# esa/auromat

Hardware: AMD Instinct MI355X
Metric: Mpixels/s georef+resample, 4240x2832 frame (higher is better)
Workload: dtype f64

## Files before the change

### auromat_amd/_native.py

```python
import ctypes as C
import os
import threading
import weakref

import numpy as np

from ._build import LIB_PATH

c_double_p = C.POINTER(C.c_double)
c_void_pp = C.POINTER(C.c_void_p)


class FrameParams(C.Structure):
    _fields_ = [('width', C.c_int32), ('height', C.c_int32), ('fast_center', C.c_int32), ('reserved', C.c_int32),
                ('cd', C.c_double * 4), ('crpix', C.c_double * 2), ('rot', C.c_double * 9),
                ('cam', C.c_double * 3), ('a', C.c_double), ('b', C.c_double),
                ('a0', C.c_double), ('b0', C.c_double), ('m_geo', C.c_double * 9), ('m_sm', C.c_double * 9)]


class AllSkyParams(C.Structure):
    _fields_ = [('size', C.c_int32), ('reserved', C.c_int32), ('xc', C.c_double), ('yc', C.c_double),
                ('k', C.c_double), ('rotation', C.c_double), ('center_offset', C.c_double),
                ('to_geo', C.c_double * 9), ('station', C.c_double * 3), ('a', C.c_double), ('b', C.c_double),
                ('a0', C.c_double), ('b0', C.c_double)]
# ... 13 lines not shown

class ZenithalWcs(C.Structure):
    _fields_ = [(k, C.c_int32) for k in ('width', 'height', 'corner', 'projection')] + \
               [('cd', C.c_double * 4), ('crpix', C.c_double * 2), ('rot', C.c_double * 9), ('start_x', C.c_double),
                ('start_y', C.c_double), ('sip_order_a', C.c_int32), ('sip_order_b', C.c_int32),
                ('sip_a', (C.c_double * SIP_MAX) * SIP_MAX), ('sip_b', (C.c_double * SIP_MAX) * SIP_MAX)]


class Axis(C.Structure):
    _fields_ = [('edges', C.c_void_p), ('nbin', C.c_int32), ('uniform', C.c_int32),
                ('first', C.c_double), ('last', C.c_double), ('step', C.c_double), ('scale', C.c_double),
                ('last_rounded', C.c_double)]


class Grid(C.Structure):
    _fields_ = [('nx', C.c_int32), ('ny', C.c_int32), ('n_lat_nodes', C.c_int32), ('n_lon_nodes', C.c_int32)] + \
               [(k, C.c_double) for k in ('lat_lo', 'lat_hi', 'lon_lo', 'lon_hi', 'lat_step', 'lon_step',
                                          'lat_center_first', 'lat_center_last', 'lon_center_first',
                                          'lon_center_last')] + [('xaxis', Axis), ('yaxis', Axis)]


class SeqFrame(C.Structure):
    _fields_ = [('ny', C.c_int32), ('nx', C.c_int32), ('nc', C.c_int32), ('index', C.c_int32),
                ('lat0', C.c_double), ('lon0', C.c_double), ('dlat', C.c_double), ('dlon', C.c_double),
                ('contains_pole', C.c_int32), ('contains_discontinuity', C.c_int32), ('magnetic', C.c_int32),
                ('reserved', C.c_int32), ('altitude', C.c_double), ('mean', C.c_void_p), ('count', C.c_void_p)]


class MosaicMember(C.Structure):
    _fields_ = [(k, C.c_void_p) for k in ('lat_c', 'lon_c', 'elev', 'img', 'center_mask')] + \
               [(k, C.c_int32) for k in ('height', 'width', 'win_x0', 'win_y0', 'win_nx', 'win_ny')]


class AreaMosaicMember(C.Structure):
    _fields_ = [(k, C.c_void_p) for k in ('lat', 'lon', 'lat_c', 'elev', 'img', 'center_mask')] + \
               [(k, C.c_int32) for k in ('height', 'width', 'win_x0', 'win_y0', 'win_nx', 'win_ny')]


class ScanLineStrip(C.Structure):
    _fields_ = [(k, C.c_void_p) for k in ('row', 'col', 'planes', 'img')] + \
               [('count', C.c_int64), ('frame', C.c_int32), ('reserved', C.c_int32)]


class Projection(C.Structure):
    _fields_ = [('kind', C.c_int32), ('mode', C.c_int32)] + \
               [(k, C.c_double) for k in ('lat0', 'lon0', 'a', 'e', 'sin_chi1', 'cos_chi1', 'm1', 'k')] + \
               [('reserved', C.c_double * 4)]


class PipeResult(C.Structure):
    _fields_ = [('status', C.c_int32), ('fused', C.c_int32), ('lon_wrapped', C.c_int32), ('edge_pixels', C.c_int32),
                ('bbox', C.c_double * 8), ('grid', Grid)]


class RunConfig(C.Structure):
    _fields_ = [(k, C.c_int32) for k in ('width', 'height', 'img_dtype', 'fast_center', 'magnetic', 'batch', 'use_hints',
                                         'n_slots', 'two_pass', 'statistic')] + \
               [(k, C.c_double) for k in ('altitude', 'min_elevation', 'lat_px_per_deg', 'lon_px_per_deg')] + \
               [('slots', C.POINTER(GeorefOut)), ('arcsec_per_px', C.c_double)]


class RunFrame(C.Structure):
    _fields_ = [('crval', C.c_double * 2), ('crpix', C.c_double * 2), ('cd', C.c_double * 4), ('lonpole', C.c_double),
                ('cam', C.c_double * 3), ('jd', C.c_double), ('altitude', C.c_double), ('img', C.c_void_p),
                ('img_host', C.c_void_p)]


class RunResult(C.Structure):
    _fields_ = [(k, C.c_int32) for k in ('status', 'slot', 'ny', 'nx', 'contains_pole', 'lon_wrapped', 'hinted',
                                         'edge_pixels', 'two_pass', 'reserved_')] + \
               [('grid_offset', C.c_int64), ('image_offset', C.c_int64), ('bbox', C.c_double * 8), ('altitude', C.c_double),
                ('grid', Grid), ('params', FrameParams), ('lat_px_per_deg', C.c_double), ('lon_px_per_deg', C.c_double),
                ('retried', C.c_int32), ('reserved2_', C.c_int32), ('uploaded_bytes', C.c_int64)]


class LensModel(C.Structure):
    _fields_ = [(k, C.c_int32) for k in ('kind', 'width', 'height', 'crop_x', 'crop_y', 'crop_width', 'crop_height', 'reserved')] + \
               [('k', C.c_double * 3)]


class LensDebug(C.Structure):
    _fields_ = [('force_path', C.c_int32), ('reserved', C.c_int32), ('tile_path', C.c_void_p)]


ABI_VERSION = 10
QUANTILES_MAX = 8
PIPE_MAX_EDGE_PIXELS = 16384
_I, _L, _D, _P = C.c_int, C.c_int64, C.c_double, C.c_void_p
_SIGNATURES = {
    'amt_abi_version': ([], _I),
    'amt_ctx_create': ([_I, _P, _I, c_void_pp], _I),
    'amt_ctx_destroy': ([_P], _I),
    'amt_ctx_set_stream': ([_P, _P], _I),
    'amt_ctx_get_stream': ([_P], _P),
    'amt_ctx_synchronize': ([_P], _I),
    'amt_last_error': ([_P], C.c_char_p),
    'amt_device_info': ([_P, C.c_char_p, C.c_size_t, C.POINTER(_I), C.POINTER(_I), C.POINTER(C.c_size_t)], _I),
    'amt_malloc': ([_P, C.c_size_t, c_void_pp], _I),
    'amt_free': ([_P, _P], _I),
    'amt_host_threads': ([_I, C.POINTER(_I), C.POINTER(_I)], _I),
    'amt_malloc_host': ([_P, C.c_size_t, c_void_pp], _I),
    'amt_free_host': ([_P, _P], _I),
    'amt_memcpy_h2d': ([_P, _P, _P, C.c_size_t], _I),
    'amt_memcpy_d2h': ([_P, _P, _P, C.c_size_t], _I),
    'amt_memset': ([_P, _P, _I, C.c_size_t], _I),
    'amt_event_create': ([_P, c_void_pp], _I),
    'amt_event_destroy': ([_P, _P], _I),
    'amt_event_record': ([_P, _P], _I),
    'amt_event_elapsed_ms': ([_P, _P, _P, C.POINTER(C.c_float)], _I),
    'amt_timing_enable': ([_P, _I], _I),
    'amt_timing_read': ([_P, _I, C.POINTER(C.c_double), C.POINTER(_I)], _I),
    'amt_pipe_launch_box': ([_P, C.POINTER(FrameParams), _D, _I], _I),
    'amt_pipe_launch_box_many': ([c_void_pp, C.c_int32, c_void_pp, _D, _I], _I),
    'amt_pipe_launch_many_res': ([c_void_pp, C.c_int32, c_void_pp, c_void_pp, c_void_pp, C.c_int32, _D, c_double_p, c_double_p, _I, _I], _I),
    'amt_plate_carree_resolution': ([_D, _D, _D, _D, _D, c_double_p, c_double_p], _I),
    'amt_upload_staged': ([_P, _P, _P, C.c_size_t], _I),
    'amt_padded_pitch': ([C.c_int32], C.c_int64),
    'amt_unpad_rows': ([_P, _P, C.c_int32, C.c_int32, C.c_int32, _P], _I),
    'amt_download_staged': ([_P, _P, _P, C.c_size_t], _I),
    'amt_georef_last_variant': ([_P, C.POINTER(C.c_int32), C.POINTER(C.c_int32), C.POINTER(C.c_int32)], _I),
    'amt_directions_tan': ([_P, C.POINTER(FrameParams), _I, _P], _I),
    'amt_directions_zenithal': ([_P, C.POINTER(ZenithalWcs), _P], _I),
    'amt_directions_tan_points': ([_P, C.POINTER(FrameParams), _P, _P, _L, _I, _P], _I),
    'amt_lens_coords': ([_P, C.POINTER(LensModel)] + [C.c_int32] * 4 + [_I, _P, _P], _I),
    'amt_lens_undistort': ([_P, C.POINTER(LensModel)] + [C.c_int32] * 4 + [_I, _P], _I),
    'amt_lens_remap': ([_P, C.POINTER(LensModel), _P, C.c_int32, C.c_int32, C.c_int32, _P, _P, C.POINTER(LensDebug)], _I),
    'amt_remap_coords': ([_P, _P] + [C.c_int32] * 4 + [_P] + [C.c_int32] * 3 + [_P, _P, C.POINTER(LensDebug)], _I),
    'amt_world_to_pixel': ([_P, C.POINTER(FrameParams), C.POINTER(ZenithalWcs), C.c_int32, _P, _P, _L, _P, _P, _P], _I),
    'amt_grid_to_pixel': ([_P, C.POINTER(FrameParams), C.POINTER(ZenithalWcs), C.c_int32, _P, C.c_int32, _P, C.c_int32, _P, _P, _P,
                           _P], _I),
    'amt_intersect_ellipsoid': ([_P, _D, _D, c_double_p, _P, _L, _I, _P], _I),
    'amt_intersects_ellipsoid': ([_P, _D, _D, c_double_p, _P, _L, _I, _P], _I),
    'amt_intersect_sphere': ([_P, _D, c_double_p, _P, _L, _I, _P], _I),
    'amt_ecef_to_geodetic': ([_P, _P, _P, _P, _L, _D, _D, _P, _P], _I),
    'amt_geodetic_to_ecef': ([_P, _P, _P, _D, _L, _D, _D, _P, _P, _P], _I),
    'amt_rotate_to_latlon': ([_P, c_double_p, _P, _L, _D, _D, _P, _P], _I),
    'amt_rotate_to_mlat_mlt': ([_P, c_double_p, _P, _L, _P, _P], _I),
    'amt_rotate_vectors': ([_P, c_double_p, _P, _L, _P], _I),
    'amt_latlon_to_mlat_mlt': ([_P, c_double_p, _P, _P, _D, _L, _D, _D, _P, _P], _I),
    'amt_sm_to_latlon': ([_P, c_double_p, _P, _P, _L, _D, _D, _P, _P], _I),
    'amt_projection_stereographic': ([_D, _D, _D, _D, C.POINTER(Projection)], _I),
    'amt_projection_polar_aeqd': ([_I, _D, _D, C.POINTER(Projection)], _I),
    'amt_project_forward': ([_P, C.POINTER(Projection), _P, _P, _L, _P, _P], _I),
    'amt_project_inverse': ([_P, C.POINTER(Projection), _P, _P, _L, _P, _P], _I),
    'amt_rotate_pole': ([_P, c_double_p, _P, _P, _D, _L, _D, _D, _P, _P], _I),
    'amt_rotate_pole_deg': ([_P, c_double_p, _P, _P, _D, _L, _D, _D, _P, _P], _I),
    'amt_cartesian_to_spherical': ([_P, _P, _P, _P, _L, _P, _P, _P], _I),
    'amt_spherical_to_cartesian': ([_P, _P, _P, _P, _L, _P, _P, _P], _I),
    'amt_georef_allsky': ([_P, C.POINTER(AllSkyParams), _I, _P, _P, _P, _P, _P], _I),
    'amt_reproject_altitude': ([_P, _D, _D, _P, _P, _L, _D, _D, _D, _D, _P, _P], _I),
    'amt_georef_frame': ([_P, C.POINTER(FrameParams), C.POINTER(GeorefOut)], _I),
    'amt_georef_frame_dirs': ([_P, C.POINTER(FrameParams), _P, C.POINTER(GeorefOut)], _I),
    'amt_georef_coarse_bbox': ([_P, C.POINTER(FrameParams), C.c_int32, _D, _I, _P], _I),
    'amt_delaunay_create': ([_P, C.c_int64, C.POINTER(C.c_void_p)], _I),
    'amt_delaunay_destroy': ([_P], _I),
    'amt_delaunay_sizes': ([_P, C.POINTER(C.c_int64), C.POINTER(C.c_int64), C.POINTER(C.c_int64)], _I),
    'amt_delaunay_stats': ([_P, _P], _I),
    'amt_delaunay_slots': ([_P, c_void_pp, c_void_pp, C.POINTER(C.c_int64)], _I),
    'amt_delaunay_create_threads': ([_P, C.c_int64, C.c_int32, C.c_int64, C.POINTER(C.c_void_p)], _I),
    'amt_delaunay_build_info': ([_P, _P], _I),
    'amt_delaunay_triangles': ([_P, _P, _P], _I),
    'amt_delaunay_vertex_neighbours': ([_P, _P, _P], _I),
    'amt_delaunay_locate': ([_P, _P, C.c_int64, _P, _P, _P], _I),
    'amt_cubic_gradients_csr': ([_P, _P, C.c_int64, _P, _P, _P, C.c_int32, _P, C.c_int32, _D, C.c_int32, _P, _P], _I),
    'amt_cubic_eval': ([_P, C.c_int64, _P, _P, _P, _P, _P, _P, _P, C.c_int32, _P], _I),
    'amt_georef_coarse_bbox_dirs': ([_P, C.POINTER(FrameParams), _P, C.c_int32, _D, _I, _P], _I),
    'amt_pipe_coarse_dirs': ([_P, C.POINTER(FrameParams), _P, _D, _I], _I),
    'amt_pipe_launch_dirs': ([_P, C.POINTER(FrameParams), _P, C.POINTER(GeorefOut), _P, C.c_int32, _D, _D, _D, _I, _I], _I),
    'amt_georef_sky_rows': ([C.POINTER(FrameParams)] + [C.POINTER(C.c_int32)] * 4, _I),
    'amt_georef_image_rows': ([C.POINTER(FrameParams), _D] + [C.POINTER(C.c_int32)] * 2, _I),
    'amt_mask_by_elevation': ([_P, _P, _P, C.c_int32, C.c_int32, _D, _P, _P, _P], _I),
    'amt_sanitize_masks': ([_P, _P, _P, _P, C.c_int32, C.c_int32, _I], _I),
    'amt_bbox_corners': ([_P, _P, _P, _P, _P, C.c_int32, C.c_int32, _P], _I),
    'amt_mask_outline_links': ([_P, _P, C.c_int32, C.c_int32, _P, _L, _P], _I),
    'amt_pixel_polygons': ([_P, _P, _P, _P, C.c_int32, C.c_int32, C.c_int32, C.c_int32, _P, _L, _P, _P, _P], _I),
    'amt_hist2d_accumulate': ([_P, _P, _P, _L, c_void_pp, C.c_int32, C.POINTER(Axis), C.POINTER(Axis), _I, _P,
                               c_void_pp], _I),
    'amt_hist2d_finalize_mean': ([_P, _P, c_void_pp, C.c_int32, C.c_int32, C.c_int32, _P], _I),
    'amt_bin_frame': ([_P, _P, _P, _P, _P, C.c_int32, C.c_int32, _P, C.c_int32, C.c_int32, _D, C.POINTER(Axis),
                       C.POINTER(Axis), _I, _P], _I),
    'amt_bin_frame_finalize': ([_P, _P, C.c_int32, C.c_int32, C.c_int32, C.c_int32, _P, _P, _P, _P], _I),
    'amt_bin_frame_finalize_window': ([_P, _P] + [C.c_int32] * 8 + [_P, _P, _P, _P], _I),
    'amt_area_frame': ([_P, _P, _P, _P, _P, _P, C.c_int32, C.c_int32, _P, C.c_int32, C.c_int32, _D, C.POINTER(Axis),
                        C.POINTER(Axis), _I, _P], _I),
    'amt_area_plane_frame': ([_P, _P, _P, _P, _P, _P, C.c_int32, C.c_int32, _P, C.c_int32, C.c_int32, _D, C.POINTER(Axis),
                              C.POINTER(Axis), _P], _I),
    'amt_area_frame_finalize': ([_P, _P, C.c_int32, C.c_int32, C.c_int32, C.c_int32, C.c_uint64, _P, _P, _P, _P], _I),
    'amt_area_frame_async': ([_P, _P, _P, _P, _P, _P, C.c_int32, C.c_int32, _P, C.c_int32, C.c_int32, _D, C.POINTER(Axis),
                              C.POINTER(Axis), _I, _I, C.c_int32, C.c_int32, C.c_uint64, _P, _P, _P, _P, _P], _I),
    'amt_median_frame': ([_P, _P, _P, _P, _P, C.c_int32, C.c_int32, _P, C.c_int32, C.c_int32, _D, C.POINTER(Axis),
                          C.POINTER(Axis), _I, _P, _P, _P, _P], _I),
    'amt_median_frame_async': ([_P, _P, _P, _P, _P, C.c_int32, C.c_int32, _P, C.c_int32, C.c_int32, _D, C.POINTER(Axis),
                                C.POINTER(Axis), _I, _I, _P, _P, _P, _P], _I),
    'amt_quantile_frame': ([_P, _P, _P, _P, _P, C.c_int32, C.c_int32, _P, C.c_int32, C.c_int32, _D, C.POINTER(Axis),
                            C.POINTER(Axis), _I, c_double_p, _I, _P, _P, _P, _P], _I),
    'amt_quantile_frame_async': ([_P, _P, _P, _P, _P, C.c_int32, C.c_int32, _P, C.c_int32, C.c_int32, _D, C.POINTER(Axis),
                                  C.POINTER(Axis), _I, _I, c_double_p, _I, _P, _P, _P, _P], _I),
    'amt_quantile_rank': ([_L, _D, C.POINTER(_L), C.POINTER(_L), c_double_p], _I),
    'amt_mosaic_frames': ([_P, C.POINTER(MosaicMember), C.c_int32, C.c_int32, C.c_int32, _D, C.POINTER(Axis), C.POINTER(Axis),
                           _I, C.c_int32, _P, _P, _P, _P, _P], _I),
    'amt_mosaic_median_frames': ([_P, C.POINTER(MosaicMember), C.c_int32, C.c_int32, C.c_int32, _D, C.POINTER(Axis),
                                  C.POINTER(Axis), _I, C.c_int32, _P, _P, _P, _P, _P], _I),
    'amt_mosaic_quantile_frames': ([_P, C.POINTER(MosaicMember), C.c_int32, C.c_int32, C.c_int32, _D, C.POINTER(Axis),
                                    C.POINTER(Axis), _I, C.c_int32, c_double_p, _I, _P, _P, _P, _P, _P], _I),
    'amt_area_mosaic_frames': ([_P, C.POINTER(AreaMosaicMember), C.c_int32, C.c_int32, C.c_int32, _D, C.POINTER(Axis),
                                C.POINTER(Axis), _I, C.c_int32, C.c_uint64, _P, _P, _P, _P, _P], _I),
    'amt_scanline_select': ([_P, _P, _P, C.c_int32, C.c_int32, _P, C.c_int32, _P, C.c_int32, C.c_int32, C.c_int32, C.c_int32, _P,
                             _P], _I),
    'amt_scanline_pack': ([_P, _P] + [C.c_int32] * 4 + [_P, C.c_int32, _P] + [C.c_int32] * 6 + [_L, _P, _P, _P, _P], _I),
    'amt_scanline_compose': ([_P, C.POINTER(ScanLineStrip)] + [C.c_int32] * 8 + [_P, _P, _P, _P], _I),
    'amt_nearest_frame': ([_P, _P, _P, _P, _P, C.c_int32, C.c_int32, _D, C.POINTER(Axis), C.POINTER(Axis), _I, _P, _P, _P,
                           _P], _I),
    'amt_nearest_gather': ([_P, _P, _L, _P, C.c_int32, C.c_int32, _P, _P, _P, _P], _I),
    'amt_points_in_polygon': ([_P, _P, _P, _L, _P, C.c_int32, _P], _I),
    'amt_grid_layout': ([_D, _D, _D, _D, _D, _D, C.POINTER(Grid)], _I),
    'amt_pipe_create': ([_P, c_void_pp], _I),
    'amt_pipe_destroy': ([_P], _I),
    'amt_pipe_coarse': ([_P, C.POINTER(FrameParams), _D, _I], _I),
    'amt_pipe_coarse_hint': ([_P, c_double_p, _I], _I),
    'amt_pipe_launch': ([_P, C.POINTER(FrameParams), C.POINTER(GeorefOut), _P, C.c_int32, _D, _D, _D, _I, _I], _I),
    'amt_pipe_launch_many': ([c_void_pp, C.c_int32, c_void_pp, c_void_pp, c_void_pp, C.c_int32, _D, _D, _D, _I, _I], _I),
    'amt_pipe_launch_dirs_many': ([c_void_pp, C.c_int32, c_void_pp, c_void_pp, c_void_pp, c_void_pp, C.c_int32, _D, _D, _D, _I, _I], _I),
    'amt_pipe_wait': ([_P, C.POINTER(PipeResult)], _I),
    'amt_pipe_finalize': ([_P, _P, _P, _P, _P], _I),
    'amt_pipe_finalize_stream': ([_P, _P], _I),
    'amt_pipe_finalize_many': ([_P, C.c_int32, _P, _P, _P, _P], _I),
    'amt_pipe_join': ([_P], _I),
    'amt_pipe_set_plan': ([_P, _I], _I),
    'amt_pipe_general_layout': ([_P, C.POINTER(PipeResult)], _I),
    'amt_pipe_general_finalize': ([_P, _P, _P, _P, _P], _I),
    'amt_frame_params_from_wcs': ([C.POINTER(RunFrame), C.c_int32, C.c_int32, C.c_int32, _D, C.c_int32,
                                   C.POINTER(FrameParams)], _I),
    'amt_pole_in_view': ([C.POINTER(FrameParams), _D, _I], _I),
    'amt_frames_close': ([C.POINTER(FrameParams), C.POINTER(FrameParams)], _I),
    'amt_box_hint': ([c_double_p, C.POINTER(FrameParams), _L, c_double_p, C.POINTER(FrameParams), _L, _L, C.POINTER(FrameParams),
                      c_double_p], _I),
    'amt_run_create': ([_P, C.POINTER(RunConfig), c_void_pp], _I),
    'amt_run_destroy': ([_P], _I),
    'amt_run_process': ([_P, C.POINTER(RunFrame), C.c_int32, _P, _L, _P, _L, C.POINTER(RunResult), C.POINTER(C.c_int32)], _I),
    'amt_run_begin': ([_P, _P, _L, _P, _L, C.POINTER(RunResult), C.c_int32], _I),
    'amt_run_push': ([_P, C.POINTER(RunFrame)], _I),
    'amt_run_end': ([_P, C.POINTER(C.c_int32)], _I),
    'amt_run_reset_hints': ([_P], _I),
    'amt_run_fill_stats': ([_P, C.POINTER(C.c_int64), C.POINTER(C.c_int64)], _I),
    'amt_run_set_quantile': ([_P, _D], _I),
    'amt_run_set_min_coverage': ([_P, C.c_uint64], _I),
    'amt_run_area_overflow': ([_P, C.POINTER(C.c_int32), C.c_int32], _I),
    'amt_seq_payload_size': ([C.POINTER(SeqFrame), C.c_int32, C.POINTER(_L)], _I),
    'amt_seq_pack': ([_P, C.POINTER(SeqFrame), C.c_int32, C.c_int32, _P, _L], _I),
    'amt_seq_unpack': ([_P, _L, C.c_int32, C.c_int32, C.POINTER(SeqFrame), C.c_int32, C.POINTER(C.c_int32)], _I),
}

_lib = None
_lib_lock = threading.Lock()


class NativeError(RuntimeError):
    pass


def host_threads(wanted):
    try:
        cores = len(os.sched_getaffinity(0))
    except (AttributeError, OSError):
        cores = os.cpu_count() or 1
    ranks = 1
    for name in ('AMT_LOCAL_RANKS', 'LOCAL_WORLD_SIZE'):
        try:
            v = int(os.environ.get(name, '0'))
        except ValueError:
            v = 0
        if v > 0:
            ranks = v
            break
    return max(1, min(int(wanted), max(1, cores // ranks)))


def host_threads_report():
    cores, ranks = C.c_int(0), C.c_int(0)
    share = lib().amt_host_threads(1 << 20, C.byref(cores), C.byref(ranks))
    copy = int(os.environ.get('AMT_COPY_THREADS', '8'))
    return dict(cores_available=cores.value, local_ranks=ranks.value, share=share,
                copy_threads=max(1, min(copy, (share + 1) // 2, 16)),
                triangulator_threads=int(os.environ.get('AMT_DELAUNAY_THREADS', '0')) or lib().amt_host_threads(16, None, None),
                io_threads=host_threads(16), omp_num_threads=os.environ.get('OMP_NUM_THREADS'))


def lib():
    global _lib
    if _lib is not None:
        return _lib
    with _lib_lock:
        if _lib is None:
            if not os.path.exists(LIB_PATH):
                raise NativeError('libauromat_hip.so is not built (%s missing); run `python -c "import '
                                  '__graft_entry__ as g; g.build()"` or `python -m auromat_amd._build`. '
                                  'There is no CPU fallback.' % LIB_PATH)
            import torch
            handle = C.CDLL(LIB_PATH, mode=C.RTLD_GLOBAL)
            for name, (argtypes, restype) in _SIGNATURES.items():
                fn = getattr(handle, name)
                fn.argtypes = argtypes
                fn.restype = restype
            if handle.amt_abi_version() != ABI_VERSION:
                raise NativeError('ABI version mismatch: the library is %d, this package expects %d (rebuild: '
                                  'python -c "import __graft_entry__ as g; g.build()")' % (handle.amt_abi_version(), ABI_VERSION))
            _lib = handle
    return _lib


def exported_symbols():
    return sorted(_SIGNATURES)


class Context(object):
    _cache = {}
    _cache_lock = threading.Lock()

    def __init__(self, device_index):
        import torch
        self._lib = lib()
        if not torch.cuda.is_available():
            raise NativeError('no HIP device is visible; auromat_amd has no CPU fallback')
        self.device = torch.device('cuda', device_index)
        self.stream_handle = torch.cuda.current_stream(self.device).cuda_stream
        h = C.c_void_p()
        rc = self._lib.amt_ctx_create(device_index, C.c_void_p(self.stream_handle), 0, C.byref(h))
        if rc != 0:
            raise NativeError('amt_ctx_create failed (%d)' % rc)
        self.handle = h
        self._staging = None

    @classmethod
    def current(cls, device=None):
        import torch
        if not torch.cuda.is_available():
            raise NativeError('no HIP device is visible; auromat_amd has no CPU fallback')
        if device is None:
            idx = torch.cuda.current_device()
        else:
            idx = torch.device(device).index
            if idx is None:
                idx = torch.cuda.current_device()
        key = (os.getpid(), threading.get_ident(), idx)
        with cls._cache_lock:
            ctx = cls._cache.get(key)
            if ctx is None:
                ctx = cls._cache[key] = cls(idx)
        stream = torch.cuda.current_stream(ctx.device).cuda_stream
        if stream != ctx.stream_handle:
            ctx.check(ctx._lib.amt_ctx_set_stream(ctx.handle, C.c_void_p(stream)))
            ctx.stream_handle = stream
        return ctx

    def check(self, rc):
        if rc != 0:
            msg = self._lib.amt_last_error(self.handle)
            raise NativeError('libauromat_hip: %s (code %d)' % (msg.decode() if msg else '?', rc))

    def call(self, name, *args):
        self.check(getattr(self._lib, name)(self.handle, *args))

    def synchronize(self):
        self.call('amt_ctx_synchronize')

    def device_info(self):
        name = C.create_string_buffer(256)
        cus, khz, mem = C.c_int(), C.c_int(), C.c_size_t()
        self.call('amt_device_info', name, 256, C.byref(cus), C.byref(khz), C.byref(mem))
        return dict(name=name.value.decode(), compute_units=cus.value, clock_khz=khz.value, total_mem=mem.value)

    def empty(self, shape, dtype=None):
        import torch
        return torch.empty(shape, dtype=dtype or torch.float64, device=self.device)

    def zeros(self, shape, dtype=None):
        import torch
        return torch.zeros(shape, dtype=dtype or torch.float64, device=self.device)

    def to_device(self, array, dtype=np.float64):
        import torch
        if isinstance(array, torch.Tensor):
            t = array.to(self.device)
            want = _torch_dtype(dtype)
            if t.dtype != want:
                t = t.to(want)
            return t.contiguous()
        a = np.ascontiguousarray(array, dtype=dtype)
        if a.dtype == np.uint16:
            a = a.view(np.int16)
        if a.nbytes >= _PIN_MIN_BYTES and np.dtype(a.dtype) in _TORCH_DTYPES:
            out = torch.empty(a.shape, dtype=_torch_dtype(a.dtype), device=self.device)
            self.upload(a, out)
            return out.view(torch.bool) if a.dtype == np.bool_ else out
        if not a.flags.writeable:
            a = a.copy()
        return torch.from_numpy(a).to(self.device)
# ... 107 lines not shown
```

### auromat_amd/csrc/amt_common.h

```cpp
#pragma once

#include <hip/hip_runtime.h>
#include <hip/hip_ext.h>

#include <cmath>
#include <cstdint>
#include <cstdio>
#include <cstring>
#include <string>
#include <vector>

#include "../../include/auromat_hip.h"

struct amt_copier;
void amt_copier_destroy(amt_copier* c);

struct amt_ctx {
    int device;
    amt_copier* copier;
    hipStream_t stream;
    bool owns_stream;
    double* scratch;
    struct workspace {
        hipStream_t stream;
        void* ptr;
        size_t bytes;
        unsigned long long last_use;
    };
    std::vector<workspace> workspaces;
    unsigned long long workspace_clock;
    std::string last_error;
    hipStream_t aux_pre, aux_tail, aux_fin;
    int last_second, last_bin, last_frames;
    int timing;
    size_t tlaunch[2];
    int tframes[2];
    std::vector<hipEvent_t> tev[2];
    size_t tused[2];
};

constexpr int kTimingMaxLaunches = 4096;

static inline void amt_timing_pair(amt_ctx* ctx, int kind, int frames, hipEvent_t* start, hipEvent_t* stop) {
    *start = *stop = nullptr;
    if (!ctx->timing) return;
    if ((ctx->tlaunch[kind]++ % (size_t)ctx->timing) != 0) return;
    if (ctx->tused[kind] + 2 > (size_t)2 * kTimingMaxLaunches) return;
    while (ctx->tused[kind] + 2 > ctx->tev[kind].size()) {
        hipEvent_t e;
        if (hipEventCreate(&e) != hipSuccess) return;
        ctx->tev[kind].push_back(e);
    }
    *start = ctx->tev[kind][ctx->tused[kind]];
    *stop = ctx->tev[kind][ctx->tused[kind] + 1];
    ctx->tused[kind] += 2;
    ctx->tframes[kind] += frames;
}

struct amt_georef_tail {
    hipStream_t stream;
    hipEvent_t kernel_done;
    double* partials;
    size_t partials_bytes;
    int band_x = 0x7fffffff, band_y = 0x7fffffff;
};
constexpr int kNoBand = 0x7fffffff;
size_t amt_georef_partials_bytes(const amt_frame_params* p);
#define AMT_MAX_BATCH 3
struct amt_sky_state {
    int known_top_end, known_bottom_begin;
    int bands_filled, bands_skipped;
};
int amt_georef_launch_many(amt_ctx* ctx, int n, const amt_frame_params* const* p, const double* const* dirs,
                           const amt_georef_out* const* out, const amt_georef_tail* const* tail, amt_sky_state* sky);
int amt_pipe_launch_many_sky(amt_pipe* const* pipes, int32_t n, const amt_frame_params* const* p, const amt_georef_out* const* out,
                             const void* const* img, int32_t img_dtype, double min_elevation, const double* lat_px_per_deg,
                             const double* lon_px_per_deg, int pole_in_view, int magnetic, amt_sky_state* sky);
int amt_bin_apply_events_on(amt_ctx* ctx, hipStream_t stream, const void* events, uint32_t* count, uint64_t* acc,
                            int32_t acc_nx, int32_t acc_ny, int32_t off_x, int32_t off_y, int32_t nx, int32_t ny,
                            uint32_t xmask, uint32_t ymask);
int amt_bin_finalize_on(amt_ctx* ctx, hipStream_t stream, uint64_t* acc, int32_t acc_nx, int32_t acc_ny, int32_t off_x,
                        int32_t off_y, int32_t nx, int32_t ny, int32_t nchan, int32_t img_dtype, double* mean,
                        void* out_img, uint8_t* out_mask, double* out_count, int clear);

int amt_mosaic_run(amt_ctx* ctx, const amt_mosaic_member* members, int32_t n_members, int32_t img_dtype, int32_t nchan,
                   double min_elevation, const amt_axis* xaxis, const amt_axis* yaxis, int lon_wrap, int32_t rule, double* mean,
                   void* out_img, uint8_t* out_mask, double* out_count, int32_t* out_source, size_t tail_bytes, char** tail);

struct finish_frame {
    const void* events;
    unsigned int* count;
    unsigned long long* acc;
    int acc_nx, acc_ny, off_x, off_y, nx, ny;
    unsigned int n_events;
    unsigned int masks;
    double* mean;
    void* img;
    uint8_t* mask;
    double* out_count;
};
struct finish_batch {
    finish_frame f[3];
    int n, pad_;
};
int amt_pipe_finish_on(amt_ctx* ctx, hipStream_t stream, const finish_batch& B, int32_t img_dtype);

constexpr size_t kMaxWorkspaces = 16;
static inline void* amt_workspace(amt_ctx* ctx, size_t bytes) {
    amt_ctx::workspace* w = nullptr;
    for (auto& e : ctx->workspaces)
        if (e.stream == ctx->stream) w = &e;
    if (w == nullptr) {
        if (ctx->workspaces.size() >= kMaxWorkspaces) {
            size_t lru = 0;
            for (size_t i = 1; i < ctx->workspaces.size(); ++i)
                if (ctx->workspaces[i].last_use < ctx->workspaces[lru].last_use) lru = i;
            amt_ctx::workspace& old = ctx->workspaces[lru];
            if (old.ptr) {
                (void)hipStreamSynchronize(old.stream);
                (void)hipGetLastError();
                (void)hipFree(old.ptr);
            }
            ctx->workspaces.erase(ctx->workspaces.begin() + (long)lru);
        }
        ctx->workspaces.push_back({ctx->stream, nullptr, 0, 0});
        w = &ctx->workspaces.back();
    }
    w->last_use = ++ctx->workspace_clock;
    if (bytes <= w->bytes) return w->ptr;
    if (w->ptr) {
        (void)hipStreamSynchronize(ctx->stream);
        (void)hipFree(w->ptr);
        w->ptr = nullptr;
        w->bytes = 0;
    }
    const size_t cap = bytes < (1u << 20) ? (1u << 20) : bytes;
    if (hipMalloc(&w->ptr, cap) != hipSuccess) {
        w->ptr = nullptr;
        return nullptr;
    }
    w->bytes = cap;
    return w->ptr;
}

#define AMT_CHECK_CTX(ctx) \
    if ((ctx) == nullptr) return AMT_EINVAL

#define AMT_REQUIRE(ctx, cond, msg)                           \
    do {                                                      \
        if (!(cond)) {                                        \
            (ctx)->last_error = std::string(__func__) + ": " + (msg); \
            return AMT_EINVAL;                                \
        }                                                     \
    } while (0)

#define AMT_HIP(ctx, call)                                                              \
    do {                                                                                \
        hipError_t err__ = (call);                                                      \
        if (err__ != hipSuccess) {                                                      \
            (ctx)->last_error = std::string(__func__) + ": " #call " -> " + hipGetErrorString(err__); \
            return AMT_EHIP;                                                            \
        }                                                                               \
    } while (0)

#define AMT_LAUNCH_CHECK(ctx) AMT_HIP(ctx, hipGetLastError())

static inline int amt_set_device(amt_ctx* ctx) {
    AMT_HIP(ctx, hipSetDevice(ctx->device));
    return AMT_OK;
}

namespace amt {

constexpr int kBlock = 256;

inline dim3 grid_for(int64_t n) {
    int64_t blocks = (n + kBlock - 1) / kBlock;
    if (blocks > 256 * 16) blocks = 256 * 16;
    if (blocks < 1) blocks = 1;
    return dim3(static_cast<unsigned>(blocks));
}

#define AMT_GRID_STRIDE(i, n) \
    for (int64_t i = blockIdx.x * (int64_t)blockDim.x + threadIdx.x; i < (n); i += (int64_t)gridDim.x * blockDim.x)

__device__ __forceinline__ bool finite(double v) { return fabs(v) < INFINITY; }

constexpr double kRad2Deg = 57.29577951308232;
constexpr double kDeg2Rad = 0.017453292519943295;
constexpr double kMltPerDeg = (24.0 / 360.0);

struct vec3 {
    double x, y, z;
};

struct mat3 {
    double m[9];
};

__host__ __device__ inline mat3 make_mat3(const double* p) {
    mat3 r;
    for (int i = 0; i < 9; ++i) r.m[i] = p[i];
    return r;
}

__device__ __forceinline__ vec3 mul(const mat3& a, const vec3& v) {
    vec3 r;
    r.x = a.m[0] * v.x + a.m[1] * v.y + a.m[2] * v.z;
    r.y = a.m[3] * v.x + a.m[4] * v.y + a.m[5] * v.z;
    r.z = a.m[6] * v.x + a.m[7] * v.y + a.m[8] * v.z;
    return r;
}

__device__ __forceinline__ double dot(const vec3& a, const vec3& b) { return a.x * b.x + a.y * b.y + a.z * b.z; }

struct ellipsoid_ray {
    double ia, ib;
    double osx, osy, osz;
    double oo;
    double ox, oy, oz;
    int inside;
    int directed;
};

// ... 614 lines not shown
```

### auromat_amd/csrc/amt_context.hip

```cpp
#include <sched.h>

#include <cstdlib>
#include <thread>

#include "amt_common.h"

extern "C" {

int amt_abi_version(void) { return AMT_ABI_VERSION; }

int amt_ctx_create(int device_id, void* stream, int own_stream, amt_ctx** out_ctx) {
    if (out_ctx == nullptr) return AMT_EINVAL;
    *out_ctx = nullptr;
    int count = 0;
    if (hipGetDeviceCount(&count) != hipSuccess || device_id < 0 || device_id >= count) return AMT_EHIP;
    amt_ctx* ctx = new (std::nothrow) amt_ctx();
    if (ctx == nullptr) return AMT_ENOMEM;
    ctx->device = device_id;
    ctx->stream = nullptr;
    ctx->owns_stream = false;
    ctx->scratch = nullptr;
    ctx->timing = 0;
    ctx->copier = nullptr;
    ctx->last_second = ctx->last_bin = ctx->last_frames = -1;
    ctx->aux_pre = ctx->aux_tail = ctx->aux_fin = nullptr;
    ctx->tlaunch[0] = ctx->tlaunch[1] = 0;
    ctx->tframes[0] = ctx->tframes[1] = 0;
    ctx->tused[0] = ctx->tused[1] = 0;
    if (hipSetDevice(device_id) != hipSuccess) {
        delete ctx;
        return AMT_EHIP;
    }
    if (!own_stream) {
        ctx->stream = reinterpret_cast<hipStream_t>(stream);
    } else {
        if (hipStreamCreateWithFlags(&ctx->stream, hipStreamNonBlocking) != hipSuccess) {
            delete ctx;
            return AMT_EHIP;
        }
        ctx->owns_stream = true;
    }
    if (hipMalloc(reinterpret_cast<void**>(&ctx->scratch), 256) != hipSuccess) {
        if (ctx->owns_stream) (void)hipStreamDestroy(ctx->stream);
        delete ctx;
        return AMT_ENOMEM;
    }
    *out_ctx = ctx;
    return AMT_OK;
}

int amt_ctx_destroy(amt_ctx* ctx) {
    AMT_CHECK_CTX(ctx);
    (void)hipSetDevice(ctx->device);
    amt_copier_destroy(ctx->copier);
    if (ctx->scratch) (void)hipFree(ctx->scratch);
    for (auto& w : ctx->workspaces)
        if (w.ptr) (void)hipFree(w.ptr);
    for (int k = 0; k < 2; ++k)
        for (hipEvent_t e : ctx->tev[k]) (void)hipEventDestroy(e);
    for (hipStream_t st : {ctx->aux_pre, ctx->aux_tail, ctx->aux_fin})
        if (st) {
            (void)hipStreamSynchronize(st);
            (void)hipStreamDestroy(st);
        }
    if (ctx->owns_stream) {
        (void)hipStreamSynchronize(ctx->stream);
        (void)hipStreamDestroy(ctx->stream);
    }
    delete ctx;
    return AMT_OK;
}

int amt_ctx_set_stream(amt_ctx* ctx, void* stream) {
    AMT_CHECK_CTX(ctx);
    if (ctx->owns_stream) {
        AMT_HIP(ctx, hipStreamSynchronize(ctx->stream));
        AMT_HIP(ctx, hipStreamDestroy(ctx->stream));
        ctx->owns_stream = false;
    }
    ctx->stream = reinterpret_cast<hipStream_t>(stream);
    return AMT_OK;
}

void* amt_ctx_get_stream(amt_ctx* ctx) { return ctx ? reinterpret_cast<void*>(ctx->stream) : nullptr; }

int amt_ctx_synchronize(amt_ctx* ctx) {
    AMT_CHECK_CTX(ctx);
    AMT_HIP(ctx, hipStreamSynchronize(ctx->stream));
    return AMT_OK;
}

const char* amt_last_error(amt_ctx* ctx) { return ctx ? ctx->last_error.c_str() : "null context"; }

int amt_device_info(amt_ctx* ctx, char* name, size_t name_len, int* compute_units, int* clock_khz,
                    size_t* total_mem) {
    AMT_CHECK_CTX(ctx);
    hipDeviceProp_t prop;
    AMT_HIP(ctx, hipGetDeviceProperties(&prop, ctx->device));
    if (name && name_len > 0) {
        std::string s = std::string(prop.name) + " (" + prop.gcnArchName + ")";
        std::strncpy(name, s.c_str(), name_len - 1);
        name[name_len - 1] = 0;
    }
    if (compute_units) *compute_units = prop.multiProcessorCount;
    if (clock_khz) *clock_khz = prop.clockRate;
    if (total_mem) *total_mem = prop.totalGlobalMem;
    return AMT_OK;
}

int amt_malloc(amt_ctx* ctx, size_t bytes, void** out_dptr) {
    AMT_CHECK_CTX(ctx);
    AMT_REQUIRE(ctx, out_dptr != nullptr, "out_dptr is NULL");
    if (amt_set_device(ctx)) return AMT_EHIP;
    hipError_t e = hipMalloc(out_dptr, bytes ? bytes : 1);
    if (e != hipSuccess) {
        ctx->last_error = std::string("amt_malloc: ") + hipGetErrorString(e);
        return e == hipErrorOutOfMemory ? AMT_ENOMEM : AMT_EHIP;
    }
    return AMT_OK;
}

int amt_free(amt_ctx* ctx, void* dptr) {
    AMT_CHECK_CTX(ctx);
    if (dptr == nullptr) return AMT_OK;
    if (amt_set_device(ctx)) return AMT_EHIP;
    AMT_HIP(ctx, hipFree(dptr));
    return AMT_OK;
}

int amt_host_threads(int wanted, int* cores, int* local_ranks) {
    int n_cores = 0;
    cpu_set_t set;
    CPU_ZERO(&set);
    if (sched_getaffinity(0, sizeof(set), &set) == 0) n_cores = CPU_COUNT(&set);
    if (n_cores <= 0) n_cores = (int)std::thread::hardware_concurrency();
    if (n_cores <= 0) n_cores = 1;
    int ranks = 1;
    for (const char* name : {"AMT_LOCAL_RANKS", "LOCAL_WORLD_SIZE"}) {
        const char* e = std::getenv(name);
        const int v = e ? std::atoi(e) : 0;
        if (v > 0) {
            ranks = v;
            break;
        }
    }
    if (cores) *cores = n_cores;
    if (local_ranks) *local_ranks = ranks;
    int share = n_cores / ranks;
    if (share < 1) share = 1;
    if (wanted < 1) wanted = 1;
    return wanted < share ? wanted : share;
}

int amt_malloc_host(amt_ctx* ctx, size_t bytes, void** out_hptr) {
    AMT_CHECK_CTX(ctx);
    AMT_REQUIRE(ctx, out_hptr != nullptr, "out_hptr is NULL");
    if (amt_set_device(ctx)) return AMT_EHIP;
    hipError_t e = hipHostMalloc(out_hptr, bytes ? bytes : 1, hipHostMallocDefault);
    if (e != hipSuccess) {
        (void)hipGetLastError();
        *out_hptr = nullptr;
        ctx->last_error = std::string("amt_malloc_host: ") + hipGetErrorString(e);
        return e == hipErrorOutOfMemory ? AMT_ENOMEM : AMT_EHIP;
    }
    return AMT_OK;
}

int amt_free_host(amt_ctx* ctx, void* hptr) {
    AMT_CHECK_CTX(ctx);
    if (hptr == nullptr) return AMT_OK;
    if (amt_set_device(ctx)) return AMT_EHIP;
    AMT_HIP(ctx, hipHostFree(hptr));
    return AMT_OK;
}

int amt_memcpy_h2d(amt_ctx* ctx, void* dst, const void* src, size_t bytes) {
    AMT_CHECK_CTX(ctx);
    AMT_REQUIRE(ctx, dst && src, "NULL pointer");
    AMT_HIP(ctx, hipMemcpyAsync(dst, src, bytes, hipMemcpyHostToDevice, ctx->stream));
    return AMT_OK;
}

int amt_memcpy_d2h(amt_ctx* ctx, void* dst, const void* src, size_t bytes) {
    AMT_CHECK_CTX(ctx);
    AMT_REQUIRE(ctx, dst && src, "NULL pointer");
    AMT_HIP(ctx, hipMemcpyAsync(dst, src, bytes, hipMemcpyDeviceToHost, ctx->stream));
    AMT_HIP(ctx, hipStreamSynchronize(ctx->stream));
    return AMT_OK;
}

int amt_memset(amt_ctx* ctx, void* dst, int value, size_t bytes) {
    AMT_CHECK_CTX(ctx);
    AMT_REQUIRE(ctx, dst != nullptr, "NULL pointer");
    AMT_HIP(ctx, hipMemsetAsync(dst, value, bytes, ctx->stream));
    return AMT_OK;
}

int amt_event_create(amt_ctx* ctx, void** out_event) {
    AMT_CHECK_CTX(ctx);
    AMT_REQUIRE(ctx, out_event != nullptr, "out_event is NULL");
    hipEvent_t ev;
    AMT_HIP(ctx, hipEventCreate(&ev));
    *out_event = reinterpret_cast<void*>(ev);
    return AMT_OK;
}

int amt_event_destroy(amt_ctx* ctx, void* event) {
    AMT_CHECK_CTX(ctx);
    if (event) AMT_HIP(ctx, hipEventDestroy(reinterpret_cast<hipEvent_t>(event)));
    return AMT_OK;
}

int amt_event_record(amt_ctx* ctx, void* event) {
    AMT_CHECK_CTX(ctx);
    AMT_REQUIRE(ctx, event != nullptr, "event is NULL");
    AMT_HIP(ctx, hipEventRecord(reinterpret_cast<hipEvent_t>(event), ctx->stream));
    return AMT_OK;
}

int amt_event_elapsed_ms(amt_ctx* ctx, void* start, void* stop, float* out_ms) {
    AMT_CHECK_CTX(ctx);
    AMT_REQUIRE(ctx, start && stop && out_ms, "NULL argument");
    AMT_HIP(ctx, hipEventSynchronize(reinterpret_cast<hipEvent_t>(stop)));
    AMT_HIP(ctx, hipEventElapsedTime(out_ms, reinterpret_cast<hipEvent_t>(start), reinterpret_cast<hipEvent_t>(stop)));
    return AMT_OK;
}

int amt_timing_enable(amt_ctx* ctx, int enable) {
    AMT_CHECK_CTX(ctx);
    ctx->timing = enable > 0 ? enable : 0;
    ctx->tused[0] = ctx->tused[1] = 0;
    ctx->tlaunch[0] = ctx->tlaunch[1] = 0;
    ctx->tframes[0] = ctx->tframes[1] = 0;
    return AMT_OK;
}

int amt_timing_read(amt_ctx* ctx, int kernel, double* total_ms, int* launches) {
    AMT_CHECK_CTX(ctx);
    AMT_REQUIRE(ctx, (kernel == AMT_KERNEL_GEOREF || kernel == AMT_KERNEL_BIN) && total_ms && launches, "bad argument");
    const size_t n = ctx->tused[kernel] / 2;
    double sum = 0;
    for (size_t i = 0; i < n; ++i) {
        float ms = 0;
        AMT_HIP(ctx, hipEventSynchronize(ctx->tev[kernel][2 * i + 1]));
        AMT_HIP(ctx, hipEventElapsedTime(&ms, ctx->tev[kernel][2 * i], ctx->tev[kernel][2 * i + 1]));
        sum += ms;
    }
    *total_ms = sum;
    *launches = ctx->tframes[kernel];
    return AMT_OK;
}

int amt_georef_last_variant(amt_ctx* ctx, int32_t* second, int32_t* bin, int32_t* frames) {
    AMT_CHECK_CTX(ctx);
    AMT_REQUIRE(ctx, second && bin && frames, "NULL argument");
    *second = ctx->last_second, *bin = ctx->last_bin, *frames = ctx->last_frames;
    return AMT_OK;
}

}
```

### auromat_amd/csrc/amt_georef.hip

```cpp
#include "amt_common.h"
#include "amt_params.h"

namespace {

using namespace amt;

struct shell_ray {
    double qa, qd;
    double kx, ky, kz;
    double qd_ko;
    double c0;
    double ox, oy, oz;
    double root_sign;
    double pad_;
};

__host__ inline void mat_mul3(const double* a, const double* b, double* out) {
    for (int i = 0; i < 3; ++i)
        for (int j = 0; j < 3; ++j) out[3 * i + j] = a[3 * i] * b[j] + a[3 * i + 1] * b[3 + j] + a[3 * i + 2] * b[6 + j];
}

__host__ inline shell_ray make_shell_ray(double a, double b, const double* cam, const double* m) {
    shell_ray r;
    r.qa = 1 / (a * a);
    r.qd = 1 / (b * b) - 1 / (a * a);
    r.kx = m[2], r.ky = m[5], r.kz = m[8];
    r.ox = m[0] * cam[0] + m[1] * cam[1] + m[2] * cam[2];
    r.oy = m[3] * cam[0] + m[4] * cam[1] + m[5] * cam[2];
    r.oz = m[6] * cam[0] + m[7] * cam[1] + m[8] * cam[2];
    r.qd_ko = r.qd * cam[2];
    const double qx = cam[0] / a, qy = cam[1] / a, qz = cam[2] / b;
    const double oo = qx * qx + qy * qy + qz * qz;
    r.c0 = oo - 1;
    r.root_sign = oo < 1 ? 1.0 : -1.0;
    r.pad_ = 0;
    return r;
}

struct affine_cam {
    double u0[3], ux[3], uy[3];
    double cx, cy;
    double pad_;
};

__host__ inline affine_cam make_affine_cam(const tan_wcs& w) {
    affine_cam c;
    const double* r = w.rot.m;
    for (int i = 0; i < 3; ++i) {
        const double r0 = r[3 * i], r1 = r[3 * i + 1], r2 = r[3 * i + 2];
        c.u0[i] = kRad2Deg * r2;
        c.ux[i] = w.cd[0] * r1 - w.cd[2] * r0;
        c.uy[i] = w.cd[1] * r1 - w.cd[3] * r0;
    }
    c.cx = 0.5 - w.crpix[0];
    c.cy = 0.5 - w.crpix[1];
    c.pad_ = 0;
    return c;
}

struct georef_args {
    tan_wcs wcs;
    ellipsoid_ray ray;
    mat3 m_geo;
    mat3 m_sm;
    bowring_fast bw;
    affine_cam cam;
    shell_ray sray;
    mat3 m_geo_sm;
    int width, height;
    const double* dirs_in;
    double* lat;
    double* lon;
    double* lat_c;
    double* lon_c;
    double* elev;
    double* mlat;
    double* mlt;
    double* mlat_c;
    double* mlt_c;
    double* bbox_partials;
    double bbox_min_elev;
    axis_dev bax, bay;
    axis_lin bxl, byl;
    const void* bin_img;
    unsigned long long* bin_acc;
    int bin_lon_wrap, bin_magnetic;
    int item_order;
    int sky_top_end, sky_bottom_begin;
    int fill_top_begin, fill_bottom_end;
    int bin_pole;
    int row_layout;
    pole_consts pole;
    bin_event* bin_events;
    unsigned int* bin_event_count;
    long long bin_event_cap;
};

constexpr int kMaxBatch = 3;
struct georef_batch {
    georef_args f[kMaxBatch];
    fx::math_table math;
};
static_assert(sizeof(georef_args) % 8 == 0 && sizeof(georef_batch) <= 4096, "kernel-argument segment");

constexpr int kThreads = 256;
#ifndef AMT_ROWS_THREADS
#define AMT_ROWS_THREADS 256
#endif
constexpr int kRowsThreads = AMT_ROWS_THREADS;
constexpr double kInf = __builtin_huge_val();

__device__ __forceinline__ double ray_param_fast(const ellipsoid_ray& e, const vec3& d) {
    const double dsx = d.x * e.ia, dsy = d.y * e.ia, dsz = d.z * e.ib;
    const double d_o = dsx * e.osx + dsy * e.osy + dsz * e.osz;
    const double d_d = dsx * dsx + dsy * dsy + dsz * dsz;
    const double disc = d_o * d_o - e.oo * d_d + d_d;
    const double root = fm::sqrt_pos(disc);
    double t = e.inside ? d_o + root : d_o - root;
    if (t < 0) t = NAN;
    return t * fm::rcp(d_d);
}

__device__ __forceinline__ void sm_to_mlat_mlt_fast(const vec3& s, double& mlat, double& mlt) {
    const double q = s.x * s.x + s.y * s.y;
    mlat = fm::atan_pos_deg(s.z, q > 0 ? fm::sqrt_pos(q) : 0.0);
    mlt = fm::atan2_deg(s.y, s.x) * (24.0 / 360.0) + 12.0;
}

template <int NT>
__device__ __forceinline__ void block_reduce8(double (&v)[8], double* __restrict__ out, double (*sRed)[NT / 64]) {
    for (int o = 32; o > 0; o >>= 1) {
        v[0] = fmin(v[0], __shfl_xor(v[0], o));
        v[1] = fmax(v[1], __shfl_xor(v[1], o));
        v[2] = fmin(v[2], __shfl_xor(v[2], o));
        v[3] = fmax(v[3], __shfl_xor(v[3], o));
        v[4] = fmin(v[4], __shfl_xor(v[4], o));
        v[5] = fmax(v[5], __shfl_xor(v[5], o));
        v[6] += __shfl_xor(v[6], o);
        v[7] += __shfl_xor(v[7], o);
    }
    const int wave = threadIdx.x >> 6, lane = threadIdx.x & 63;
    if (lane == 0)
        for (int k = 0; k < 8; ++k) sRed[k][wave] = v[k];
    __syncthreads();
    if (threadIdx.x < 8) {
        const int k = threadIdx.x;
        double r = sRed[k][0];
        for (int w = 1; w < NT / 64; ++w) {
            const double o = sRed[k][w];
            r = (k >= 6) ? r + o : ((k & 1) ? fmax(r, o) : fmin(r, o));
        }
        out[k] = r;
    }
}

constexpr int kDppWaveShl1 = 0x130;
constexpr int kDppWaveShr1 = 0x138;

__device__ __forceinline__ double from_next_lane(double v) {
    const long long b = __double_as_longlong(v);
    const int lo = __builtin_amdgcn_mov_dpp((int)(b & 0xffffffffll), kDppWaveShl1, 0xf, 0xf, true);
    const int hi = __builtin_amdgcn_mov_dpp((int)(b >> 32), kDppWaveShl1, 0xf, 0xf, true);
    return __longlong_as_double(((long long)hi << 32) | (unsigned int)lo);
}
__device__ __forceinline__ int from_next_lane(int v) {
    return __builtin_amdgcn_mov_dpp(v, kDppWaveShl1, 0xf, 0xf, true);
}
__device__ __forceinline__ int from_prev_lane(int v) {
    return __builtin_amdgcn_update_dpp(0, v, kDppWaveShr1, 0xf, 0xf, false);
}

__device__ __forceinline__ double nan_unless(bool keep, double v) {
    const unsigned long long b = (unsigned long long)__double_as_longlong(v);
    const unsigned int hi = keep ? (unsigned int)(b >> 32) : 0x7ff80000u;
    return __longlong_as_double((long long)(((unsigned long long)hi << 32) | (b & 0xffffffffull)));
}

__device__ __forceinline__ double opaque_nan() {
    double n = __builtin_nan("");
    asm volatile("" : "+v"(n));
    return n;
}

typedef const __attribute__((address_space(4))) unsigned long long* karg_ptr;

__device__ __forceinline__ karg_ptr karg_fresh(int word_offset = 0) {
    karg_ptr p = (karg_ptr)__builtin_amdgcn_kernarg_segment_ptr() + word_offset;
    asm volatile("" : "+s"(p));
    return p;
}

template <typename T>
__device__ __forceinline__ T karg_load(karg_ptr base, size_t byte_offset) {
    static_assert(sizeof(T) % 8 == 0, "constant blocks are multiples of 8 bytes");
    union {
        T value;
        unsigned long long words[sizeof(T) / 8];
    } u;
    karg_ptr q = base + byte_offset / 8;
#pragma unroll
    for (size_t i = 0; i < sizeof(T) / 8; ++i) u.words[i] = q[i];
    return u.value;
}

__device__ __forceinline__ vec3 affine_ray(double ubx, double uby, double ubz, double uyx, double uyy, double uyz, double py) {
#pragma clang fp contract(off)
    vec3 u = {__builtin_fma(py, uyx, ubx), __builtin_fma(py, uyy, uby), __builtin_fma(py, uyz, ubz)};
    return u;
}

__device__ __forceinline__ double shell_t(const shell_ray& e, const vec3& u, double uu) {
#pragma clang fp contract(off)
    const double ku = fx::dot3(u.x, u.y, u.z, e.kx, e.ky, e.kz);
    const double uo = fx::dot3(u.x, u.y, u.z, e.ox, e.oy, e.oz);
    const double a2 = __builtin_fma(e.qd * ku, ku, e.qa * uu);
    const double nb = -__builtin_fma(e.qa, uo, e.qd_ko * ku);
    const double disc = __builtin_fma(nb, nb, -(a2 * e.c0));
    const double root = fx::sqrt_n(disc);
    const double t = __builtin_fma(e.root_sign, root, nb);
    return t * fx::rcp_n(a2);
}

__device__ __forceinline__ vec3 shell_point(const shell_ray& e, const vec3& u, double t) {
#pragma clang fp contract(off)
    vec3 p = {__builtin_fma(u.x, t, e.ox), __builtin_fma(u.y, t, e.oy), __builtin_fma(u.z, t, e.oz)};
    return p;
}

__device__ __forceinline__ vec3 rotate3(const mat3& a, const vec3& v) {
#pragma clang fp contract(off)
    vec3 r = {__builtin_fma(a.m[2], v.z, __builtin_fma(a.m[1], v.y, a.m[0] * v.x)),
              __builtin_fma(a.m[5], v.z, __builtin_fma(a.m[4], v.y, a.m[3] * v.x)),
              __builtin_fma(a.m[8], v.z, __builtin_fma(a.m[7], v.y, a.m[6] * v.x))};
    return r;
}

constexpr int kBinW = 8, kBinCells = kBinW * kBinW;

#ifndef AMT_ROWS_MIN_WAVES
#define AMT_ROWS_MIN_WAVES 4
#endif
#ifndef AMT_ROWS_MIN_WAVES_BIN
#define AMT_ROWS_MIN_WAVES_BIN 4
#endif
#ifndef AMT_ROWS_MIN_WAVES_MAG
#define AMT_ROWS_MIN_WAVES_MAG 3
#endif
#ifndef AMT_ROWS_MIN_WAVES_POLE
#define AMT_ROWS_MIN_WAVES_POLE 3
#endif
#ifndef AMT_ROWS_MIN_WAVES_MAGONLY
#define AMT_ROWS_MIN_WAVES_MAGONLY 4
#endif
template <bool FAST, bool DIRS_IN, int SECOND, int BIN>
__global__ __launch_bounds__(kRowsThreads, SECOND == 4 ? AMT_ROWS_MIN_WAVES_MAGONLY : (SECOND >= 2 ? AMT_ROWS_MIN_WAVES_POLE : (SECOND == 1 && BIN ? AMT_ROWS_MIN_WAVES_MAG : (BIN ? AMT_ROWS_MIN_WAVES_BIN : AMT_ROWS_MIN_WAVES)))) void k_georef_rows(georef_batch B, int rows_per_chunk, int strips_x,
                                                           int n_items, int n_frames) {
    constexpr bool MAG = SECOND != 0, kPole = SECOND == 2, kMagPole = SECOND == 3, kMagOnly = SECOND == 4;
    static_assert(!(kPole || kMagPole) || (BIN != 0 && !DIRS_IN), "the pole plans exist for fused binning with the camera model only");
    static_assert(!kMagOnly || !DIRS_IN, "the MLat / MLT-only mode exists for the camera model only");
    constexpr int kBinWaves = BIN ? kRowsThreads / 64 : 1, kBinSlots = BIN ? kBinCells : 1;
    __shared__ unsigned int sCnt[kBinWaves][kBinSlots];
    __shared__ unsigned int sCh[kBinWaves][3][kBinSlots];
    __shared__ unsigned long long sEl[kBinWaves][kBinSlots];
    __shared__ double sBox[kRowsThreads / 64][6][64];
    const int lane = threadIdx.x & 63;
    const int wave = __builtin_amdgcn_readfirstlane(threadIdx.x >> 6);
    const int item_all = blockIdx.x * (kRowsThreads / 64) + wave;
    if (item_all >= n_items * n_frames) return;
    const int frame = item_all / n_items;
    const int item = item_all - frame * n_items;
    const georef_args& A = B.f[frame];
    const int koff = frame * (int)(sizeof(georef_args) / 8);
    int bin_ax0 = 0, bin_ay0 = 0;
    bool bin_anchor = false;
    if (BIN) {
#pragma unroll
        for (int i = lane; i < kBinCells; i += 64) {
            sCnt[wave][i] = 0;
            sEl[wave][i] = 0;
            sCh[wave][0][i] = 0;
            sCh[wave][1][i] = 0;
            sCh[wave][2][i] = 0;
        }
    }
    int run_key = 0;
    unsigned int run_cnt = 0, run_c0 = 0, run_c1 = 0, run_c2 = 0;
    long long run_el = 0;
    auto bin_flush = [&](int key, unsigned int cnt, unsigned int c0, unsigned int c1, unsigned int c2, long long el) {
        const int bx = key >> 16, by = key & 0xffff;
        const int dx = bx - bin_ax0, dy = by - bin_ay0;
        if (dx >= 0 && dx < kBinW && dy >= 0 && dy < kBinW) {
            const int slot = dx * kBinW + dy;
            atomicAdd(&sCnt[wave][slot], cnt);
            atomicAdd(&sCh[wave][0][slot], c0);
            atomicAdd(&sCh[wave][1][slot], c1);
            atomicAdd(&sCh[wave][2][slot], c2);
            atomicAdd(&sEl[wave][slot], (unsigned long long)el);
        } else {
            karg_ptr K = karg_fresh(koff);
            const int nby = karg_load<axis_lin>(K, offsetof(georef_args, byl)).nbin;
            const int64_t ncell = (int64_t)karg_load<axis_lin>(K, offsetof(georef_args, bxl)).nbin * nby;
            unsigned long long* acc = karg_load<unsigned long long*>(K, offsetof(georef_args, bin_acc));
            const int64_t cell = (int64_t)(bx - 1) * nby + (by - 1);
            atomicAdd(&acc[cell], (unsigned long long)cnt);
            atomicAdd(&acc[ncell + cell], (unsigned long long)c0);
            atomicAdd(&acc[2 * ncell + cell], (unsigned long long)c1);
            atomicAdd(&acc[3 * ncell + cell], (unsigned long long)c2);
            atomicAdd(&acc[4 * ncell + cell], (unsigned long long)el);
        }
    };
    const int chunks_y = n_items / strips_x;
    int chunk, strip;
    chunk = item / strips_x;
    strip = item - chunk * strips_x;
    if (A.item_order == 2) chunk = chunks_y - 1 - chunk;
    const int x0 = strip * 63, y0 = chunk * rows_per_chunk;
    const int rows = min(rows_per_chunk, A.height - y0);
    const int gx = x0 + lane;
    const int W1 = A.width + 1;
    const bool col_ok = gx <= A.width;
    const bool px_ok = lane < 63 && gx < A.width;
    const bool want_bbox = A.bbox_partials != nullptr;

    if (!DIRS_IN && (chunk < A.sky_top_end || chunk >= A.sky_bottom_begin)) {
        const bool fill = (chunk >= A.fill_top_begin && chunk < A.sky_top_end) || (chunk >= A.sky_bottom_begin && chunk < A.fill_bottom_end);
        const int n_corner_rows = rows + (y0 + rows == A.height ? 1 : 0);
        auto fill_nan = [&](double* base, int64_t first, int64_t count) {
            if (base == nullptr) return;
            int64_t a = first + count * strip / strips_x, b = first + count * (strip + 1) / strips_x;
            if ((reinterpret_cast<uintptr_t>(base + a) & 15) != 0 && a < b) {
                if (lane == 0) base[a] = NAN;
                ++a;
            }
            const double2 two = {NAN, NAN};
            for (int64_t i = a + 2 * lane; i + 1 < b; i += 128) *reinterpret_cast<double2*>(base + i) = two;
            if (((b - a) & 1) && lane == 0 && b > a) base[b - 1] = NAN;
        };
        const bool mag_out = MAG && !kPole;
        const int64_t cpitch = A.row_layout ? (int64_t)strips_x * 64 : W1, ppitch = A.row_layout ? (int64_t)strips_x * 64 : A.width;
        const int64_t c0 = (int64_t)y0 * cpitch, cn = (int64_t)n_corner_rows * cpitch;
        const int64_t p0 = (int64_t)y0 * ppitch, pn = (int64_t)rows * ppitch;
        if (fill) {
            fill_nan(A.lat, c0, cn);
            fill_nan(A.lon, c0, cn);
            fill_nan(A.lat_c, p0, pn);
            fill_nan(A.lon_c, p0, pn);
            fill_nan(A.elev, p0, pn);
        }
        if (fill && mag_out) {
            fill_nan(A.mlat, c0, cn);
            fill_nan(A.mlt, c0, cn);
            fill_nan(A.mlat_c, p0, pn);
            fill_nan(A.mlt_c, p0, pn);
        }
        if (want_bbox && lane < 8)
            A.bbox_partials[(int64_t)item * 8 + lane] = lane >= 6 ? 0.0 : ((lane & 1) ? -kInf : kInf);
        return;
    }

#ifndef AMT_ROWS_PIN
#define AMT_ROWS_PIN 1
#endif
    auto pin = [](auto v) {
        if (AMT_ROWS_PIN >= 1) asm volatile("" : "+s"(v));
        return v;
    };
    auto pin2 = [](auto v) {
        if (AMT_ROWS_PIN >= 2) asm volatile("" : "+s"(v));
        return v;
    };
    affine_cam cm = A.cam;
    cm.uy[0] = pin(cm.uy[0]), cm.uy[1] = pin(cm.uy[1]), cm.uy[2] = pin(cm.uy[2]), cm.cy = pin(cm.cy);
    shell_ray ray = A.sray;
    ray.qa = pin(ray.qa), ray.qd = pin(ray.qd), ray.kx = pin(ray.kx), ray.ky = pin(ray.ky), ray.kz = pin(ray.kz);
    ray.qd_ko = pin(ray.qd_ko), ray.c0 = pin(ray.c0), ray.ox = pin(ray.ox), ray.oy = pin(ray.oy), ray.oz = pin(ray.oz);
    ray.root_sign = pin(ray.root_sign);
    bowring_fast bw = A.bw;
    bw.b_over_a = pin2(bw.b_over_a), bw.d = pin2(bw.d), bw.e2a = pin2(bw.e2a);
    const double min_elev = pin2(A.bbox_min_elev);
    double* const out_lat = pin2(A.lat);
    double* const out_lon = pin2(A.lon);
    double* const out_lat_c = pin2(A.lat_c);
    double* const out_lon_c = pin2(A.lon_c);
    double* const out_elev = pin2(A.elev);
    const unsigned char* const img_base = pin2(static_cast<const unsigned char*>(A.bin_img));
    const double bx_e0 = pin2(A.bxl.e0), bx_inv = pin2(A.bxl.inv_step), bx_margin = pin2(A.bxl.margin), by_e0 = pin2(A.byl.e0),
                 by_inv = pin2(A.byl.inv_step), by_margin = pin2(A.byl.margin);
    const int bx_n = pin2(A.bxl.nbin), by_n = pin2(A.byl.nbin);
    const bool lon_wrap = pin2(A.bin_lon_wrap) != 0;
    const double sm0 = pin2(B.math.small4[0]), sm1 = pin2(B.math.small4[1]), sm2 = pin2(B.math.small4[2]), sm3 = pin2(B.math.small4[3]);
    const int frame_h = pin2(A.height);
    struct row_state {
        vec3 p, d;
        double la, lo;
        double bn, bd;
        double bla, blo;
        vec3 s;
        double sxy, ml, sl;
        vec3 r;
        double rxy, rla, rlo;
        int flag;
    };
    row_state S0 = {{NAN, NAN, NAN}, {NAN, NAN, NAN}, NAN, NAN, NAN, NAN, NAN, NAN, {NAN, NAN, NAN}, NAN, NAN, NAN,
                    {NAN, NAN, NAN}, NAN, NAN, NAN, 0}, S1 = S0;
    constexpr bool kMagBox = (MAG && BIN != 0) || kMagOnly;
    constexpr bool pole_bin = kPole;
    const bool geo_pole = kMagPole && !A.bin_magnetic;
    const bool centre_coords = BIN != 0 || A.lat_c != nullptr || A.lon_c != nullptr || (MAG && A.mlat_c != nullptr);
    int n_valid = 0;
    auto box_add = [&](double la_v, double lo_v) {
        __hip_atomic_fetch_min(&sBox[wave][0][lane], la_v, __ATOMIC_RELAXED, __HIP_MEMORY_SCOPE_WORKGROUP);
        __hip_atomic_fetch_max(&sBox[wave][1][lane], la_v, __ATOMIC_RELAXED, __HIP_MEMORY_SCOPE_WORKGROUP);
        __hip_atomic_fetch_min(&sBox[wave][2][lane], lo_v, __ATOMIC_RELAXED, __HIP_MEMORY_SCOPE_WORKGROUP);
        __hip_atomic_fetch_max(&sBox[wave][3][lane], lo_v, __ATOMIC_RELAXED, __HIP_MEMORY_SCOPE_WORKGROUP);
        if (lo_v > 0)
            __hip_atomic_fetch_min(&sBox[wave][4][lane], lo_v, __ATOMIC_RELAXED, __HIP_MEMORY_SCOPE_WORKGROUP);
        else
            __hip_atomic_fetch_max(&sBox[wave][5][lane], lo_v, __ATOMIC_RELAXED, __HIP_MEMORY_SCOPE_WORKGROUP);
    };
    if (want_bbox) {
#pragma unroll
        for (int k = 0; k < 6; ++k) sBox[wave][k][lane] = (k & 1) ? -kInf : kInf;
    }
    unsigned int rawA0 = 0, rawA1 = 0, rawB0 = 0, rawB1 = 0;
    unsigned int curB0 = 0, curB1 = 0;
    int shiftA = 0, shiftB = 0, curShiftB = 0;
    const unsigned int img_last = (unsigned int)((int64_t)A.width * A.height * (BIN == 1 ? 3 : 6) - 8);
    auto load_pixel = [&](unsigned int byte_offset, unsigned int& w0, unsigned int& w1, int& shift) {
        unsigned int a = byte_offset & ~3u;
        a = a > img_last ? img_last : a;
        shift = (int)(byte_offset - a) * 8;
        uint2 w2;
        __builtin_memcpy(&w2, img_base + a, 8);
        w0 = w2.x;
        w1 = w2.y;
    };
    auto unpack_pixel = [&](unsigned int w0, unsigned int w1, int shift, unsigned int& c0, unsigned int& c1, unsigned int& c2) {
        if (BIN == 1) {
            const unsigned int w = (unsigned int)((((unsigned long long)w1 << 32) | w0) >> shift);
            c0 = w & 0xffu, c1 = (w >> 8) & 0xffu, c2 = (w >> 16) & 0xffu;
        } else {
            const unsigned int lo = __builtin_amdgcn_alignbit(w1, w0, (unsigned int)shift), hi = w1 >> shift;
            c0 = lo & 0xffffu, c1 = lo >> 16, c2 = hi & 0xffffu;
        }
    };

    const bool padded = A.row_layout != 0;
    const unsigned int pitch_corner = padded ? (unsigned int)strips_x * 512u : (unsigned int)W1 * 8u;
    const unsigned int pitch_pixel = padded ? (unsigned int)strips_x * 512u : (unsigned int)A.width * 8u;
    const unsigned int col_bytes = padded ? (unsigned int)(strip * 64 + lane) * 8u : (unsigned int)gx * 8u;
    unsigned int off_corner = (unsigned int)y0 * pitch_corner + col_bytes;
    unsigned int off_pixel = (unsigned int)(y0 - 1) * pitch_pixel + col_bytes;
    const bool st_corner = padded || (col_ok && (lane < 63 || gx == A.width));
    const bool st_pixel = padded || px_ok;
    auto at = [](double* base, unsigned int byte_offset) -> double& {
        return *reinterpret_cast<double*>(reinterpret_cast<char*>(base) + byte_offset);
    };
    const unsigned int img_row = (unsigned int)A.width * (BIN == 1 ? 3u : 6u);
    unsigned int img_off = (unsigned int)((y0 - 1) * A.width + gx) * (BIN == 1 ? 3u : 6u);
    double ubx = 0, uby = 0, ubz = 0;
    if (!DIRS_IN || !FAST) {
#pragma clang fp contract(off)
        const double px = (double)gx + cm.cx;
        ubx = __builtin_fma(px, cm.ux[0], cm.u0[0]), uby = __builtin_fma(px, cm.ux[1], cm.u0[1]);
        ubz = __builtin_fma(px, cm.ux[2], cm.u0[2]);
    }
    const double hcx = 0.5 * (cm.ux[0] - cm.uy[0]), hcy = 0.5 * (cm.ux[1] - cm.uy[1]), hcz = 0.5 * (cm.ux[2] - cm.uy[2]);
    double dj0 = NAN, dj1 = NAN, dj2 = NAN;
    if (DIRS_IN && col_ok) {
        const double* q = A.dirs_in + 3 * ((int64_t)y0 * W1 + gx);
        dj0 = q[0], dj1 = q[1], dj2 = q[2];
    }

    typedef double coef4[4];
    typedef double coef9[9];
    struct c4 { coef4 c; };
    struct c9 { coef9 c; };
    auto small_table = [&]() {
        c4 k = {{sm0, sm1, sm2, sm3}};
        return k;
    };
    auto atan_table = [&]() { return karg_load<c9>(karg_fresh(), offsetof(georef_batch, math) + offsetof(fx::math_table, atan9)); };
    auto full_angles = [&](double n, double d, double x, double y, double& la_v, double& lo_v) {
        const c9 k = atan_table();
        la_v = fx::atan_pos_deg(n, d, k.c);
        lo_v = fx::atan2_deg(y, x, k.c);
    };
    auto sm_point = [&](const vec3& pt, vec3& sv, double& sxy) {
#pragma clang fp contract(off)
        sv = rotate3(karg_load<mat3>(karg_fresh(koff), offsetof(georef_args, m_geo_sm)), pt);
        const double q = __builtin_fma(sv.x, sv.x, sv.y * sv.y);
        sxy = q > 0 ? fx::sqrt_n(q) : 0.0;
    };
    auto pole_point = [&](double n, double d, double x, double y, vec3& sv, double& sxy) {
#pragma clang fp contract(off)
        const pole_consts pc = karg_load<pole_consts>(karg_fresh(koff), offsetof(georef_args, pole));
        const double rs = fx::rsqrt_n(__builtin_fma(n, n, d * d));
        const double sphi = n * rs, cphi = d * rs;
        const double q = __builtin_fma(x, x, y * y);
        const double ip = q > 0 ? fx::rsqrt_n(q) : 0.0;
        const double big_n = pc.w.a * fx::rsqrt_n(__builtin_fma(-(pc.e2 * sphi), sphi, 1.0));
        const double rc = ((big_n + pc.alt) * cphi) * ip;
        const double gx = rc * x, gy = rc * y, gz = __builtin_fma(big_n, pc.one_minus_e2, pc.alt) * sphi;
        double rn, rd, ir;
        fx::bowring_nd(bw, gx, -gz, gy, rn, rd, ir);
        sv.x = gx, sv.y = -gz, sv.z = rn;
        sxy = rd;
    };
    auto sm_angles = [&](const vec3& ref, double ref_sxy, double ref_ml, double ref_sl, const vec3& sv, double sxy, bool live,
                         double& ml, double& sl) {
        double dml, dsl;
        bool ok;
        fx::small_angles(ref_sxy, ref.z, sxy, sv.z, ref.x, ref.y, sv.x, sv.y, small_table().c, dml, dsl, ok);
        ok = ok && fabs(ref_sl) < 178.0;
        ml = ref_ml + dml;
        sl = ref_sl + dsl;
        if (live && !ok) {
            const c9 k = atan_table();
            ml = fx::atan_pos_deg(sv.z, sxy, k.c);
            sl = fx::atan2_deg(sv.y, sv.x, k.c);
        }
    };
    auto corner_ray = [&](int gy, const vec3& dj) -> vec3 {
        if (DIRS_IN) return rotate3(karg_load<mat3>(karg_fresh(koff), offsetof(georef_args, m_geo)), dj);
        return affine_ray(ubx, uby, ubz, cm.uy[0], cm.uy[1], cm.uy[2], (double)gy + cm.cy);
    };
    auto take_pixel = [&](int r, bool even, unsigned int& ch0, unsigned int& ch1, unsigned int& ch2) {
        if (even) {
            asm volatile("" : "+v"(rawA0), "+v"(rawA1), "+v"(rawB0), "+v"(rawB1));
            unpack_pixel(rawA0, rawA1, shiftA, ch0, ch1, ch2);
            curB0 = rawB0, curB1 = rawB1, curShiftB = shiftB;
            if (px_ok && r + 1 < rows) load_pixel(img_off + 2 * img_row, rawA0, rawA1, shiftA);
            if (px_ok && r + 2 < rows) load_pixel(img_off + 3 * img_row, rawB0, rawB1, shiftB);
        } else {
            unpack_pixel(curB0, curB1, curShiftB, ch0, ch1, ch2);
        }
    };
    auto bin_account = [&](int bin_x, int bin_y, unsigned int ch0, unsigned int ch1, unsigned int ch2, long long el_fix) {
        const unsigned long long m = __ballot(bin_x > 0);
        if (m && !bin_anchor) {
            const int src = __builtin_ctzll(m);
            bin_ax0 = __shfl(bin_x, src) - kBinW / 2;
            bin_ay0 = __shfl(bin_y, src) - kBinW / 2;
            bin_anchor = true;
        }
        if (bin_x > 0) {
            const int key = (bin_x << 16) | bin_y;
            if (key != run_key) {
                if (run_key) bin_flush(run_key, run_cnt, run_c0, run_c1, run_c2, run_el);
                run_key = key;
                run_cnt = 0;
                run_c0 = run_c1 = run_c2 = 0;
                run_el = 0;
            }
            run_cnt += 1;
            run_c0 += ch0;
            run_c1 += ch1;
            run_c2 += ch2;
            run_el += el_fix;
        }
    };
    auto bin_common = [&](double bxv, double byv, int& bx, int& by, bool& slow) {
        bool slow_x, slow_y;
        bx = bin_fast(bx_e0, bx_inv, bx_margin, bx_n, bxv, slow_x);
        by = bin_fast(by_e0, by_inv, by_margin, by_n, byv, slow_y);
        slow = slow_x || slow_y;
    };
    auto bin_slow = [&](double bxv, double byv, int& bx, int& by, unsigned int& edge_flags) {
        karg_ptr K = karg_fresh(koff);
        const axis_dev ax = karg_load<axis_dev>(K, offsetof(georef_args, bax));
        bx = bin_index<true>(ax, bxv);
        bx = bx > ax.nbin ? 0 : bx;
        if (bx > 0) {
            const unsigned int f = on_lower_edge_bits(ax, bx, bxv);
            edge_flags |= (f & 1u) | ((f & 2u) << 1) | ((f & 4u) << 2);
        }
        const axis_dev ay = karg_load<axis_dev>(K, offsetof(georef_args, bay));
        by = bin_index<true>(ay, byv);
        by = by > ay.nbin ? 0 : by;
        if (by > 0) {
            const unsigned int f = on_lower_edge_bits(ay, by, byv);
            edge_flags |= ((f & 1u) << 1) | ((f & 2u) << 2) | ((f & 4u) << 3);
        }
    };

    struct corner_vals {
        vec3 p;
        double la, lo, bn, bd, bla, blo;
        vec3 sv;
        double sxy, sml, ssl;
        vec3 rv;
        double rxy, rla, rlo;
    };
    auto step = [&](const int r, const bool even, const vec3& dj, const row_state& prev, row_state& cur) {
        const int gy = y0 + r;
        unsigned int ch0 = 0, ch1 = 0, ch2 = 0;
        const shell_ray& ry = ray;
        const vec3 u = corner_ray(gy, dj);
        const double uu = fx::dot3(u.x, u.y, u.z, u.x, u.y, u.z);
        const double t = shell_t(ry, u, uu);
        const bool hit = col_ok && t >= 0.0;
        vec3 d;
        if (DIRS_IN) {
            d = u;
        } else {
#pragma clang fp contract(off)
            const double rs = fx::rsqrt_n(uu);
            d.x = u.x * rs, d.y = u.y * rs, d.z = u.z * rs;
        }
        corner_vals c;
        const bool magbox = MAG && (kMagOnly || (BIN && !kPole && A.bin_magnetic));
        if (__builtin_amdgcn_ballot_w64(hit) != 0) {
            c.p = shell_point(ry, u, nan_unless(hit, t));
            c.la = c.lo = c.bn = c.bd = NAN;
            if (!kMagOnly) {
                double ir;
                fx::bowring_nd(bw, c.p.x, c.p.y, c.p.z, c.bn, c.bd, ir);
                double dla, dlo;
                bool ok;
                fx::small_angles(prev.bd, prev.bn, c.bd, c.bn, prev.p.x, prev.p.y, c.p.x, c.p.y, small_table().c, dla, dlo, ok);
                ok = ok && fabs(prev.lo) < 178.0;
                c.la = prev.la + dla;
                c.lo = prev.lo + dlo;
                if (hit && !ok) full_angles(c.bn, c.bd, c.p.x, c.p.y, c.la, c.lo);
            }
            c.sv = {NAN, NAN, NAN}, c.sxy = c.sml = c.ssl = NAN;
            c.rv = {NAN, NAN, NAN}, c.rxy = c.rla = c.rlo = NAN;
            if (MAG) {
                if (pole_bin) pole_point(c.bn, c.bd, c.p.x, c.p.y, c.sv, c.sxy); else sm_point(c.p, c.sv, c.sxy);
                sm_angles(prev.s, prev.sxy, prev.ml, prev.sl, c.sv, c.sxy, hit, c.sml, c.ssl);
                if (kMagPole) {
                    if (geo_pole) pole_point(c.bn, c.bd, c.p.x, c.p.y, c.rv, c.rxy); else pole_point(c.sv.z, c.sxy, c.sv.x, c.sv.y, c.rv, c.rxy);
                    sm_angles(prev.r, prev.rxy, prev.rla, prev.rlo, c.rv, c.rxy, hit, c.rla, c.rlo);
                }
            }
        } else {
            const double n = opaque_nan();
            c.p = {n, n, n}, c.la = c.lo = c.bn = c.bd = n;
            c.sv = {n, n, n}, c.sxy = c.sml = c.ssl = n;
            c.rv = {n, n, n}, c.rxy = c.rla = c.rlo = n;
        }
        const double mt_corner = MAG ? c.ssl * (24.0 / 360.0) + 12.0 : NAN;
        c.bla = c.blo = NAN;
        if (MAG) {
            if (magbox) {
                c.bla = c.sml;
                c.blo = (mt_corner - 12.0) / (24.0 / 360.0);
            }
            if (kMagPole) c.bla = c.rla, c.blo = c.rlo;
            if (pole_bin) c.bla = c.sml, c.blo = c.ssl;
            if (kMagBox && !magbox && !pole_bin && !kMagPole) c.bla = c.la, c.blo = c.lo;
        }
        if (BIN) take_pixel(r, even, ch0, ch1, ch2);
        const bool owner = st_corner && (r < rows || gy == frame_h);
        if (owner) {
            if (!kMagOnly) {
                if (out_lat) at(out_lat, off_corner) = c.la;
                if (out_lon) at(out_lon, off_corner) = c.lo;
            }
            if (MAG && !kPole && A.mlat) {
                at(A.mlat, off_corner) = c.sml;
                at(A.mlt, off_corner) = mt_corner;
            }
        }
        int flag_cur = 0;
        if (r > 0) {
            vec3 pc, dsum;
            double dscale;
            bool corners_ok = true;
            if (FAST) {
                const double sx = prev.p.x + c.p.x, sy = prev.p.y + c.p.y, sz = prev.p.z + c.p.z;
                const double tx = prev.d.x + d.x, ty = prev.d.y + d.y, tz = prev.d.z + d.z;
                pc.x = (sx + from_next_lane(sx)) * 0.25;
                pc.y = (sy + from_next_lane(sy)) * 0.25;
                pc.z = (sz + from_next_lane(sz)) * 0.25;
                dsum.x = tx + from_next_lane(tx);
                dsum.y = ty + from_next_lane(ty);
                dsum.z = tz + from_next_lane(tz);
                dscale = 0.25;
            } else {
                vec3 uc;
                double uuc;
                {
#pragma clang fp contract(off)
                    uc.x = u.x + hcx, uc.y = u.y + hcy, uc.z = u.z + hcz;
                    uuc = fx::dot3(uc.x, uc.y, uc.z, uc.x, uc.y, uc.z);
                    const double rs = fx::rsqrt_n(uuc);
                    dsum.x = uc.x * rs, dsum.y = uc.y * rs, dsum.z = uc.z * rs;
                }
                dscale = 1.0;
                const double tc = shell_t(ry, uc, uuc);
                pc = shell_point(ry, uc, nan_unless(tc >= 0.0, tc));
                if (want_bbox) {
                    const int h = (prev.p.x == prev.p.x) && (c.p.x == c.p.x);
                    corners_ok = h && from_next_lane(h);
                }
            }
            const bool live = px_ok && pc.x == pc.x;
            double lac, loc, el, ml = NAN, mt = NAN, slc = NAN, rlac = NAN, rloc = NAN;
            if (__builtin_amdgcn_ballot_w64(live) != 0) {
                double inv_r, cn = NAN, cd = NAN;
                if (kMagOnly || !centre_coords) {
#pragma clang fp contract(off)
                    inv_r = fx::rsqrt_n(__builtin_fma(pc.z, pc.z, __builtin_fma(pc.x, pc.x, pc.y * pc.y)));
                    lac = loc = kMagOnly ? NAN : opaque_nan();
                } else {
                    fx::bowring_nd(bw, pc.x, pc.y, pc.z, cn, cd, inv_r);
                    double dla, dlo;
                    bool ok;
                    fx::small_angles(c.bd, c.bn, cd, cn, c.p.x, c.p.y, pc.x, pc.y, small_table().c, dla, dlo, ok);
                    ok = ok && fabs(c.lo) < 178.0;
                    lac = c.la + dla;
                    loc = c.lo + dlo;
                    if (live && !ok) full_angles(cn, cd, pc.x, pc.y, lac, loc);
                }
                double cs = -(fx::dot3(dsum.x, dsum.y, dsum.z, pc.x, pc.y, pc.z) * dscale) * inv_r;
                cs = nan_unless(live, fmin(1.0, fmax(-1.0, cs)));
                el = fx::asin_deg(cs, atan_table().c);
                if (MAG && centre_coords) {
                    vec3 sc;
                    double sxyc;
                    if (pole_bin) pole_point(cn, cd, pc.x, pc.y, sc, sxyc); else sm_point(pc, sc, sxyc);
                    sm_angles(c.sv, c.sxy, c.sml, c.ssl, sc, sxyc, live, ml, slc);
                    mt = slc * (24.0 / 360.0) + 12.0;
                    if (kMagPole) {
                        vec3 rc;
                        double rxyc;
                        if (geo_pole) pole_point(cn, cd, pc.x, pc.y, rc, rxyc); else pole_point(sc.z, sxyc, sc.x, sc.y, rc, rxyc);
                        sm_angles(c.rv, c.rxy, c.rla, c.rlo, rc, rxyc, live, rlac, rloc);
                    }
                }
            } else {
                const double n = opaque_nan();
                lac = loc = el = ml = mt = slc = rlac = rloc = n;
            }
            if (st_pixel) {
                if (!kMagOnly && out_lat_c) at(out_lat_c, off_pixel) = lac;
                if (!kMagOnly && out_lon_c) at(out_lon_c, off_pixel) = loc;
                if (out_elev) at(out_elev, off_pixel) = el;
                if (MAG && !kPole && A.mlat_c) {
                    at(A.mlat_c, off_pixel) = ml;
                    at(A.mlt_c, off_pixel) = mt;
                }
            }
            const bool valid = px_ok && (el >= min_elev) && corners_ok;
            int bin_x = 0, bin_y = 0;
            long long el_fix = 0;
            if (BIN && valid) {
                const bool bin_mag = kMagOnly || (MAG && !kPole && A.bin_magnetic);
                double bxv = bin_mag ? (mt - 12.0) / (24.0 / 360.0) : loc;
                double byv = bin_mag ? ml : lac;
                if (pole_bin) bxv = slc, byv = ml;
                if (kMagPole) bxv = rloc, byv = rlac;
                if (lon_wrap) bxv = wrap180_shifted(bxv);
                int bx, by;
                bool slow;
                bin_common(bxv, byv, bx, by, slow);
                unsigned int edge_flags = 0;
                if (__ballot(slow)) {
                    if (slow) {
                        if (pole_bin || kMagPole) {
                            const pole_consts pk = karg_load<pole_consts>(karg_fresh(koff), offsetof(georef_args, pole));
                            if (kMagPole && !geo_pole)
                                rotate_pole_deg(pk.w, pk.rot, pk.e2, ml, (mt - 12.0) / (24.0 / 360.0), pk.alt, byv, bxv);
                            else
                                rotate_pole_deg(pk.w, pk.rot, pk.e2, lac, loc, pk.alt, byv, bxv);
                        }
                        bin_slow(bxv, byv, bx, by, edge_flags);
                    }
                }
                if (bx > 0 && by > 0) {
                    el_fix = to_fix32(el);
                    bin_event* events = nullptr;
                    if (edge_flags) events = karg_load<bin_event*>(karg_fresh(koff), offsetof(georef_args, bin_events));
                    if (events != nullptr) {
                        karg_ptr KE = karg_fresh(koff);
                        unsigned int* cnt = karg_load<unsigned int*>(KE, offsetof(georef_args, bin_event_count));
                        const long long cap = karg_load<long long>(KE, offsetof(georef_args, bin_event_cap));
                        const unsigned int slot = atomicAdd(cnt, 1u);
                        if ((long long)slot < cap) {
                            bin_event ev;
                            ev.bx = bx, ev.by = by, ev.flags = edge_flags;
                            ev.c0 = ch0, ev.c1 = ch1, ev.c2 = ch2;
                            ev.el = el_fix;
                            events[slot] = ev;
                        }
                    } else {
                        bin_x = bx;
                        bin_y = by;
                    }
                }
            }
            if (BIN) bin_account(bin_x, bin_y, ch0, ch1, ch2, el_fix);
            if (want_bbox) {
                const int vi = valid ? 1 : 0;
                flag_cur = vi | from_prev_lane(vi);
                n_valid += vi;
                if (kMagBox) {
                    if ((prev.flag | flag_cur) && prev.bla == prev.bla) box_add(prev.bla, prev.blo);
                } else {
                    if ((prev.flag | flag_cur) && prev.la == prev.la) box_add(prev.la, prev.lo);
                }
            }
        }
        cur.p = c.p;
        cur.d = d;
        cur.la = c.la;
        cur.lo = c.lo;
        cur.bn = c.bn;
        cur.bd = c.bd;
        if (kMagBox) {
            cur.bla = c.bla;
            cur.blo = c.blo;
        }
        if (MAG) {
            cur.s = c.sv;
            cur.sxy = c.sxy;
            cur.ml = c.sml;
            cur.sl = c.ssl;
        }
        if (kMagPole) {
            cur.r = c.rv;
            cur.rxy = c.rxy;
            cur.rla = c.rla;
            cur.rlo = c.rlo;
        }
        cur.flag = flag_cur;
    };

    auto advance = [&](const int r, const bool even, const row_state& prev, row_state& cur) {
        vec3 dj = {dj0, dj1, dj2};
        if (DIRS_IN) {
            asm volatile("" : "+v"(dj.x), "+v"(dj.y), "+v"(dj.z));
            if (col_ok && r < rows) {
                const double* q = A.dirs_in + 3 * ((int64_t)(y0 + r + 1) * W1 + gx);
                dj0 = q[0], dj1 = q[1], dj2 = q[2];
            }
        }
        step(r, even, dj, prev, cur);
        off_corner += pitch_corner;
        off_pixel += pitch_pixel;
        img_off += img_row;
    };
    if (BIN && px_ok && rows > 0) load_pixel(img_off + img_row, rawB0, rawB1, shiftB);
    for (int r = 0; r <= rows; r += 2) {
        advance(r, true, S0, S1);
        if (r + 1 <= rows) advance(r + 1, false, S1, S0); else S0 = S1;
    }
    if (BIN && bin_anchor) {
        if (run_key) bin_flush(run_key, run_cnt, run_c0, run_c1, run_c2, run_el);
        __threadfence_block();
        karg_ptr K = karg_fresh(koff);
        const int nby = karg_load<axis_lin>(K, offsetof(georef_args, byl)).nbin;
        const int64_t ncell = (int64_t)karg_load<axis_lin>(K, offsetof(georef_args, bxl)).nbin * nby;
        unsigned long long* acc = karg_load<unsigned long long*>(K, offsetof(georef_args, bin_acc));
#pragma unroll
        for (int i = lane; i < kBinCells; i += 64) {
            const unsigned int cnt = sCnt[wave][i];
            if (cnt == 0) continue;
            const int dx = i / kBinW, dy = i - dx * kBinW;
            const int64_t cell = (int64_t)(bin_ax0 + dx - 1) * nby + (bin_ay0 + dy - 1);
            atomicAdd(&acc[cell], (unsigned long long)cnt);
            atomicAdd(&acc[ncell + cell], (unsigned long long)sCh[wave][0][i]);
            atomicAdd(&acc[2 * ncell + cell], (unsigned long long)sCh[wave][1][i]);
            atomicAdd(&acc[3 * ncell + cell], (unsigned long long)sCh[wave][2][i]);
            atomicAdd(&acc[4 * ncell + cell], sEl[wave][i]);
        }
    }
    if (want_bbox) {
        if (kMagBox) {
            if (S0.flag && S0.bla == S0.bla) box_add(S0.bla, S0.blo);
        } else {
            if (S0.flag && S0.la == S0.la) box_add(S0.la, S0.lo);
        }
        double v[7];
#pragma unroll
        for (int k = 0; k < 6; ++k)
            v[k] = __hip_atomic_load(&sBox[wave][k][lane], __ATOMIC_RELAXED, __HIP_MEMORY_SCOPE_WORKGROUP);
        v[6] = (double)n_valid;
        for (int o = 32; o > 0; o >>= 1) {
            v[0] = fmin(v[0], __shfl_xor(v[0], o));
            v[1] = fmax(v[1], __shfl_xor(v[1], o));
            v[2] = fmin(v[2], __shfl_xor(v[2], o));
            v[3] = fmax(v[3], __shfl_xor(v[3], o));
            v[4] = fmin(v[4], __shfl_xor(v[4], o));
            v[5] = fmax(v[5], __shfl_xor(v[5], o));
            v[6] += __shfl_xor(v[6], o);
        }
        if (lane < 8) A.bbox_partials[(int64_t)item * 8 + lane] = lane == 0 ? v[0] : lane == 1 ? v[1] : lane == 2 ? v[2]
                                                                  : lane == 3 ? v[3] : lane == 4 ? v[4]
                                                                  : lane == 5 ? v[5] : lane == 6 ? v[6] : 0.0;
    }
}

__global__ __launch_bounds__(kThreads) void k_bbox_fold(const double* __restrict__ partials, int n,
                                                         double* __restrict__ out,
                                                         const unsigned int* __restrict__ extra) {
    __shared__ double sRed[8][kThreads / 64];
    double v[8] = {kInf, -kInf, kInf, -kInf, kInf, -kInf, 0, 0};
    for (int i = blockIdx.x * kThreads + threadIdx.x; i < n; i += gridDim.x * kThreads) {
        const double* q = partials + (int64_t)i * 8;
        v[0] = fmin(v[0], q[0]);
        v[1] = fmax(v[1], q[1]);
        v[2] = fmin(v[2], q[2]);
        v[3] = fmax(v[3], q[3]);
        v[4] = fmin(v[4], q[4]);
        v[5] = fmax(v[5], q[5]);
        v[6] += q[6];
        v[7] += q[7];
    }
    if (extra != nullptr) v[7] = threadIdx.x == 0 ? (double)*extra : 0.0;
    block_reduce8<kThreads>(v, out + (int64_t)blockIdx.x * 8, sRed);
}

constexpr int kFoldBlocks = 64;

struct fold_batch {
    const double* in[kMaxBatch];
    double* out[kMaxBatch];
    const unsigned int* extra[kMaxBatch];
};

__global__ __launch_bounds__(kThreads) void k_bbox_fold_batch(fold_batch Bf, int n) {
    __shared__ double sRed[8][kThreads / 64];
    const int f = blockIdx.y;
    const double* partials = Bf.in[f];
    double v[8] = {kInf, -kInf, kInf, -kInf, kInf, -kInf, 0, 0};
    for (int i = blockIdx.x * kThreads + threadIdx.x; i < n; i += gridDim.x * kThreads) {
        const double* q = partials + (int64_t)i * 8;
        v[0] = fmin(v[0], q[0]);
        v[1] = fmax(v[1], q[1]);
        v[2] = fmin(v[2], q[2]);
        v[3] = fmax(v[3], q[3]);
        v[4] = fmin(v[4], q[4]);
        v[5] = fmax(v[5], q[5]);
        v[6] += q[6];
        v[7] += q[7];
    }
    if (Bf.extra[f] != nullptr) v[7] = threadIdx.x == 0 ? (double)*Bf.extra[f] : 0.0;
    block_reduce8<kThreads>(v, Bf.out[f] + (int64_t)blockIdx.x * 8, sRed);
}

struct launch_events {
    hipEvent_t start, stop;
};

template <bool FAST, bool DIRS_IN, int BIN>
void launch_rows_bin(amt_ctx* ctx, const georef_batch& B, int n_frames, dim3 grid, int second, int rows, int strips_x,
                     int n_items, launch_events ev) {
    const dim3 block(kRowsThreads);
    if (second == 4) {
        if constexpr (!DIRS_IN)
            hipExtLaunchKernelGGL((k_georef_rows<FAST, DIRS_IN, 4, BIN>), grid, block, 0, ctx->stream, ev.start, ev.stop, 0, B,
                                  rows, strips_x, n_items, n_frames);
    } else if (second == 3) {
        if constexpr (BIN != 0 && !DIRS_IN)
            hipExtLaunchKernelGGL((k_georef_rows<FAST, DIRS_IN, 3, BIN>), grid, block, 0, ctx->stream, ev.start, ev.stop, 0, B,
                                  rows, strips_x, n_items, n_frames);
    } else if (second == 2) {
        if constexpr (BIN != 0 && !DIRS_IN)
            hipExtLaunchKernelGGL((k_georef_rows<FAST, DIRS_IN, 2, BIN>), grid, block, 0, ctx->stream, ev.start, ev.stop, 0, B,
                                  rows, strips_x, n_items, n_frames);
    } else if (second == 1) {
        hipExtLaunchKernelGGL((k_georef_rows<FAST, DIRS_IN, 1, BIN>), grid, block, 0, ctx->stream, ev.start, ev.stop, 0, B,
                              rows, strips_x, n_items, n_frames);
    } else {
        hipExtLaunchKernelGGL((k_georef_rows<FAST, DIRS_IN, 0, BIN>), grid, block, 0, ctx->stream, ev.start, ev.stop, 0, B,
                              rows, strips_x, n_items, n_frames);
    }
}

template <bool FAST, bool DIRS_IN>
void launch_rows(amt_ctx* ctx, const georef_batch& B, int n_frames, dim3 grid, int second, int bin, int rows, int strips_x,
                 int n_items, launch_events ev) {
    if (bin == 1)
        launch_rows_bin<FAST, DIRS_IN, 1>(ctx, B, n_frames, grid, second, rows, strips_x, n_items, ev);
    else if (bin == 2)
        launch_rows_bin<FAST, DIRS_IN, 2>(ctx, B, n_frames, grid, second, rows, strips_x, n_items, ev);
    else
        launch_rows_bin<FAST, DIRS_IN, 0>(ctx, B, n_frames, grid, second, rows, strips_x, n_items, ev);
}

template <bool DIRS>
__global__ __launch_bounds__(kThreads) void k_coarse_bbox(georef_args A, int stride, int magnetic, double min_elev,
                                                           double* __restrict__ partials) {
    __shared__ double sRed[8][kThreads / 64];
    const int nxl = (A.width + stride - 1) / stride + 1, nyl = (A.height + stride - 1) / stride + 1;
    double v[8] = {kInf, -kInf, kInf, -kInf, kInf, -kInf, 0, 0};
    const int i = blockIdx.x * kThreads + threadIdx.x;
    if (i < nxl * nyl) {
        const int iy = i / nxl, ix = i - iy * nxl;
        const int gx = min(ix * stride, A.width), gy = min(iy * stride, A.height);
        vec3 d;
        if (DIRS) {
            const double* q = A.dirs_in + 3 * ((int64_t)gy * (A.width + 1) + gx);
            d.x = q[0], d.y = q[1], d.z = q[2];
        } else {
            d = tan_direction_fast(A.wcs, gx - 0.5, gy - 0.5);
        }
        const double t = ray_param_fast(A.ray, d);
        if (t == t) {
            v[7] = (double)(((2 * gx > A.width) - (2 * gx < A.width)) * (1 << 20) + ((2 * gy > A.height) - (2 * gy < A.height)));
            const vec3 p = ray_point(A.ray, d, t);
            double c = -(d.x * p.x + d.y * p.y + d.z * p.z) * fm::rsqrt(dot(p, p));
            c = fmin(1.0, fmax(-1.0, c));
            if (fm::asin_deg(c) >= min_elev) {
                double la, lo;
                if (magnetic == 1 || magnetic == 3) {
                    double mt;
                    sm_to_mlat_mlt_fast(mul(A.m_sm, p), la, mt);
                    lo = (mt - 12.0) / (24.0 / 360.0);
                    if (magnetic == 3) rotate_pole_deg(A.pole.w, A.pole.rot, A.pole.e2, la, lo, A.pole.alt, la, lo);
                } else {
                    const vec3 g = mul(A.m_geo, p);
                    ecef_to_geodetic_deg_fast(A.bw, g.x, g.y, g.z, la, lo);
                    if (magnetic == 2) rotate_pole_deg(A.pole.w, A.pole.rot, A.pole.e2, la, lo, A.pole.alt, la, lo);
                }
                v[0] = v[1] = la;
                v[2] = v[3] = lo;
                if (lo > 0) v[4] = lo; else v[5] = lo;
                v[6] = 1;
            }
        }
    }
    block_reduce8<kThreads>(v, partials + (int64_t)blockIdx.x * 8, sRed);
}

int nadir_side(const amt_frame_params* p) {
    const double d[3] = {-p->cam[0], -p->cam[1], -p->cam[2]};
    const double* r = p->rot;
    const double vx = r[0] * d[0] + r[3] * d[1] + r[6] * d[2], vy = r[1] * d[0] + r[4] * d[1] + r[7] * d[2];
    const double bx = vy, by = -vx;
    const double det = p->cd[0] * p->cd[3] - p->cd[1] * p->cd[2];
    if (!(det != 0)) return 1;
    const double px = (bx * p->cd[3] - p->cd[1] * by) / det, py = (p->cd[0] * by - p->cd[2] * bx) / det;
    return (std::fabs(py) >= std::fabs(px) && py > 0) ? 2 : 1;
}

struct launch_shape {
    int rows_per_chunk, strips_x, chunks_y;
    int64_t n_items;
};

launch_shape shape_of(const amt_frame_params* p) {
    launch_shape s;
    s.rows_per_chunk = 16;
    s.strips_x = (p->width + 1 + 62) / 63;
    s.chunks_y = (p->height + s.rows_per_chunk - 1) / s.rows_per_chunk;
    s.n_items = (int64_t)s.strips_x * s.chunks_y;
    return s;
}

template <class Eval>
void conic_bands(double W, double H, int n, int rows_per_chunk, Eval eval, int* top_end, int* bottom_begin) {
    *top_end = 0, *bottom_begin = n;
    struct quad {
        double a, b, c, L;
        double at(double s) const { return (a * s + b) * s + c; }
        double max_on(double s0, double s1) const {
            double m = std::max(at(s0), at(s1));
            if (a < 0) {
                const double v = -b / (2 * a);
                if (v > s0 && v < s1) m = std::max(m, at(v));
            }
            return m;
        }
    };
    auto fit = [](double f0, double f1, double f2, double L) {
        quad q;
        q.L = L;
        q.c = f0;
        q.a = 2 * (f2 - 2 * f1 + f0) / (L * L);
        q.b = (f2 - f0) / L - q.a * L;
        return q;
    };
    const double x0 = -1.0, xL = W + 2.0, y0 = -1.0, yL = H + 2.0;
    double nb00, nb10, nb01, tmp;
    quad col[3];
    double scale = 0;
    for (int k = 0; k < 3; ++k) {
        const double x = x0 + 0.5 * k * xL;
        double f[3];
        for (int j = 0; j < 3; ++j) {
            f[j] = eval(x, y0 + 0.5 * j * yL, &tmp);
            scale = std::max(scale, std::max(std::fabs(f[j]), tmp * tmp));
        }
        col[k] = fit(f[0], f[1], f[2], yL);
    }
    eval(x0, y0, &nb00);
    eval(x0 + xL, y0, &nb10);
    eval(x0, y0 + yL, &nb01);
    const double nbx = (nb10 - nb00) / xL, nby = (nb01 - nb00) / yL;
    const double tol = 1e-9 * scale, nb_tol = 1e-9 * std::sqrt(scale);
    if (!(scale > 0) || !std::isfinite(scale)) return;
    auto segment_free = [&](const quad& q, double n0, double slope, double s0, double s1) {
        double a = s0, b = s1;
        const double na = n0 + slope * s0 + nb_tol, nbv = n0 + slope * s1 + nb_tol;
        if (na < 0 && nbv < 0) return true;
        if (na < 0) a = s0 + (s1 - s0) * (-na) / (nbv - na);
        if (nbv < 0) b = s0 + (s1 - s0) * na / (na - nbv);
        return q.max_on(a, b) < -tol;
    };
    auto line_free = [&](double s) {
        const quad q = fit(col[0].at(s), col[1].at(s), col[2].at(s), xL);
        return segment_free(q, nb00 + nby * s, nbx, 0.0, xL);
    };
    auto side_free = [&](int k, double s0, double s1) {
        return segment_free(col[k], nb00 + (k == 2 ? nbx * xL : 0.0), nby, s0, s1);
    };
    auto band_free = [&](int c) {
        const double s0 = (double)c * rows_per_chunk, s1 = std::min((double)(c + 1) * rows_per_chunk, H) + 2.0;
        return line_free(s0) && line_free(s1) && side_free(0, s0, s1) && side_free(2, s0, s1);
    };
    int t = 0;
    while (t < n && band_free(t)) ++t;
    *top_end = t;
    if (t == n) return;
    int b = n;
    while (b > t && band_free(b - 1)) --b;
    *bottom_begin = b;
}

double pixel_angle(const affine_cam& c) {
    return std::sqrt(std::max(c.uy[0] * c.uy[0] + c.uy[1] * c.uy[1] + c.uy[2] * c.uy[2],
                              c.ux[0] * c.ux[0] + c.ux[1] * c.ux[1] + c.ux[2] * c.ux[2])) / kRad2Deg;
}

void sky_bands(const georef_args& A, const launch_shape& sh, int* top_end, int* bottom_begin) {
    const int n = sh.chunks_y;
    *top_end = 0, *bottom_begin = n;
    const shell_ray& e = A.sray;
    if (!(e.root_sign < 0)) return;
    auto eval = [&](double x, double y, double* nb_out) {
        const affine_cam& c = A.cam;
        const double px = x + c.cx, py = y + c.cy;
        const double ux = c.u0[0] + px * c.ux[0] + py * c.uy[0], uy = c.u0[1] + px * c.ux[1] + py * c.uy[1],
                     uz = c.u0[2] + px * c.ux[2] + py * c.uy[2];
        const double uu = ux * ux + uy * uy + uz * uz;
        const double ku = ux * e.kx + uy * e.ky + uz * e.kz, uo = ux * e.ox + uy * e.oy + uz * e.oz;
        const double a2 = e.qd * ku * ku + e.qa * uu, nb = -(e.qa * uo + e.qd_ko * ku);
        *nb_out = nb;
        return nb * nb - a2 * e.c0;
    };
    {
        const double oo = std::sqrt(e.ox * e.ox + e.oy * e.oy + e.oz * e.oz);
        const double sin_rho = std::min(1.0, 1.0 / (std::sqrt(e.qa) * oo));
        if (!(std::asin(sin_rho) > 8.0 * (sh.rows_per_chunk + 2) * pixel_angle(A.cam))) return;
    }
    conic_bands((double)A.width, (double)A.height, n, sh.rows_per_chunk, eval, top_end, bottom_begin);
}

void elevation_bands(const georef_args& A, const launch_shape& sh, double min_elev_deg, int* top_end, int* bottom_begin) {
    const int n = sh.chunks_y;
    *top_end = 0, *bottom_begin = n;
    const shell_ray& e = A.sray;
    if (!(e.root_sign < 0) || !(min_elev_deg > 0) || !(min_elev_deg < 90)) return;
    const double oo = e.ox * e.ox + e.oy * e.oy + e.oz * e.oz;
    const double r_max = 1.0 / std::sqrt(std::min(e.qa, e.qa + e.qd));
    const double k = r_max / std::sqrt(oo) * std::cos(min_elev_deg * kDeg2Rad);
    if (!(k < 1.0)) return;
    const double cos2 = 1.0 - k * k;
    if (!(std::asin(k) > 8.0 * (sh.rows_per_chunk + 2) * pixel_angle(A.cam))) return;
    auto eval = [&](double x, double y, double* lin_out) {
        const affine_cam& c = A.cam;
        const double px = x + c.cx, py = y + c.cy;
        const double ux = c.u0[0] + px * c.ux[0] + py * c.uy[0], uy = c.u0[1] + px * c.ux[1] + py * c.uy[1],
                     uz = c.u0[2] + px * c.ux[2] + py * c.uy[2];
        const double uu = ux * ux + uy * uy + uz * uz;
        const double uo = ux * e.ox + uy * e.oy + uz * e.oz;
        *lin_out = -uo;
        return uo * uo - cos2 * oo * uu;
    };
    int t = 0, b = n;
    conic_bands((double)A.width, (double)A.height, n, sh.rows_per_chunk, eval, &t, &b);
    *top_end = std::max(0, t - 1), *bottom_begin = std::min(n, b + 1);
    if (t == n) *top_end = n, *bottom_begin = n;
}

void camera_model(const amt_frame_params* p, georef_args* A) {
    double rot_geo[9];
    A->wcs = make_tan_wcs(p);
    mat_mul3(p->m_geo, p->rot, rot_geo);
    tan_wcs wcs_geo = A->wcs;
    wcs_geo.rot = make_mat3(rot_geo);
    A->cam = make_affine_cam(wcs_geo);
    A->sray = make_shell_ray(p->a, p->b, p->cam, p->m_geo);
    A->width = p->width;
    A->height = p->height;
}

struct prepared_frame {
    georef_args A;
    launch_shape sh;
    const amt_frame_params* p;
    const double* dirs;
    const amt_georef_out* out;
    const amt_georef_tail* tail;
    double* fold;
    int second;
    int bin;
};

int prepare_georef(amt_ctx* ctx, const amt_frame_params* p, const double* dirs, const amt_georef_out* out,
                   const amt_georef_tail* tail, prepared_frame* F, amt_sky_state* sky = nullptr) {
    AMT_REQUIRE(ctx, p && out, "NULL argument");
    AMT_REQUIRE(ctx, p->width > 0 && p->height > 0, "empty frame");
    AMT_REQUIRE(ctx, p->a > 0 && p->b > 0 && p->a0 > 0 && p->b0 > 0, "ellipsoid axes must be positive");
    AMT_REQUIRE(ctx, (out->mlat == nullptr) == (out->mlt == nullptr), "mlat and mlt must be given together");
    AMT_REQUIRE(ctx, (out->mlat_c == nullptr) == (out->mlt_c == nullptr), "mlat_c and mlt_c must be given together");
    AMT_REQUIRE(ctx, dirs == nullptr || p->fast_center, "caller-supplied directions need fast_center");
    georef_args& A = F->A;
    camera_model(p, &A);
    A.ray = make_ray(p->a, p->b, p->cam, 1);
    A.m_geo = make_mat3(p->m_geo);
    A.m_sm = make_mat3(p->m_sm);
    {
        double mt[9], geo_sm[9];
        for (int i = 0; i < 3; ++i)
            for (int j = 0; j < 3; ++j) mt[3 * i + j] = p->m_geo[3 * j + i];
        mat_mul3(p->m_sm, mt, geo_sm);
        A.m_geo_sm = make_mat3(geo_sm);
    }
    A.bw = make_bowring_fast(p->a0, p->b0);
    A.dirs_in = dirs;
    A.lat = out->lat;
    A.lon = out->lon;
    A.lat_c = out->lat_c;
    A.lon_c = out->lon_c;
    A.elev = out->elev;
    A.mlat = out->mlat;
    A.mlt = out->mlt;
    A.mlat_c = out->mlat_c;
    A.mlt_c = out->mlt_c;
    A.bbox_min_elev = out->bbox_min_elevation;
    int bin = 0;
    A.bin_img = nullptr;
    A.bin_acc = nullptr;
    A.bin_lon_wrap = A.bin_magnetic = A.bin_pole = 0;
    A.row_layout = out->row_layout == AMT_ROWS_STRIP_PADDED ? 1 : 0;
    A.pole = make_pole_consts(p->a0, p->b0, 0.0);
    A.bin_events = nullptr;
    A.bin_event_count = nullptr;
    A.bin_event_cap = 0;
    A.item_order = out->item_order == 1 || out->item_order == 2 ? out->item_order : (dirs ? 1 : nadir_side(p));
    std::memset(&A.bax, 0, sizeof(A.bax));
    std::memset(&A.bay, 0, sizeof(A.bay));
    std::memset(&A.bxl, 0, sizeof(A.bxl));
    std::memset(&A.byl, 0, sizeof(A.byl));
    if (out->bin_acc != nullptr) {
        AMT_REQUIRE(ctx, out->bin_img && (out->bin_img_dtype == 1 || out->bin_img_dtype == 2),
                    "fused binning needs a uint8 (1) or uint16 (2) RGB image");
        AMT_REQUIRE(ctx, (int64_t)p->width * p->height >= 3, "fused binning needs at least 3 pixels");
        AMT_REQUIRE(ctx, (int64_t)p->width * p->height * 6 < (1ll << 32), "fused binning: image larger than 4 GiB");
        AMT_REQUIRE(ctx, axis_ok(out->bin_xaxis) && axis_ok(out->bin_yaxis) && out->bin_xaxis->uniform &&
                             out->bin_yaxis->uniform, "fused binning needs two uniform axes");
        AMT_REQUIRE(ctx, out->bin_xaxis->nbin < 65535 && out->bin_yaxis->nbin < 65535, "at most 65534 bins per axis");
        make_axis(out->bin_xaxis, &A.bax);
        make_axis(out->bin_yaxis, &A.bay);
        if (tail != nullptr && out->bin_events != nullptr) A.bax.band = tail->band_x, A.bay.band = tail->band_y;
        A.bxl = make_axis_lin(A.bax);
        A.byl = make_axis_lin(A.bay);
        A.bin_img = out->bin_img;
        A.bin_acc = reinterpret_cast<unsigned long long*>(out->bin_acc);
        A.bin_lon_wrap = out->bin_lon_wrap ? 1 : 0;
        A.bin_magnetic = out->bin_magnetic ? 1 : 0;
        if (out->bin_pole) {
            AMT_REQUIRE(ctx, !A.bin_lon_wrap, "bin_pole excludes bin_lon_wrap");
            AMT_REQUIRE(ctx, dirs == nullptr, "bin_pole needs the camera model");
            AMT_REQUIRE(ctx, std::fabs((p->a - p->a0) - out->altitude) < 1e-6 && std::fabs((p->b - p->b0) - out->altitude) < 1e-6,
                        "bin_pole: amt_georef_out.altitude does not match the shell of the frame");
            A.bin_pole = 1;
            A.pole = make_pole_consts(p->a0, p->b0, out->altitude);
        }
        if (out->bin_events != nullptr) {
            AMT_REQUIRE(ctx, out->bin_event_count != nullptr && out->bin_event_capacity > 0, "bin_events needs a counter and a capacity");
            A.bin_events = static_cast<bin_event*>(out->bin_events);
            A.bin_event_count = out->bin_event_count;
            A.bin_event_cap = out->bin_event_capacity;
        }
        bin = out->bin_img_dtype;
    } else if (out->bin_magnetic) {
        AMT_REQUIRE(ctx, dirs == nullptr && !out->lat && !out->lon && !out->lat_c && !out->lon_c,
                    "bin_magnetic without bin_acc (the box in MLat / SM longitude) excludes the geodetic outputs and caller-supplied directions");
        A.bin_magnetic = 1;
    }
    const launch_shape sh = shape_of(p);
    A.sky_top_end = 0, A.sky_bottom_begin = sh.chunks_y;
    if (dirs == nullptr) sky_bands(A, sh, &A.sky_top_end, &A.sky_bottom_begin);
    {
        amt_prm::sky_known known = amt_prm::sky_known_empty();
        if (sky != nullptr) known.top_end = sky->known_top_end, known.bottom_begin = sky->known_bottom_begin;
        known = amt_prm::sky_fill(known, sh.chunks_y, A.sky_top_end, A.sky_bottom_begin, &A.fill_top_begin, &A.fill_bottom_end);
        if (sky != nullptr) {
            sky->known_top_end = known.top_end, sky->known_bottom_begin = known.bottom_begin;
            sky->bands_filled = (A.sky_top_end - A.fill_top_begin) + (A.fill_bottom_end - A.sky_bottom_begin);
            sky->bands_skipped = A.sky_top_end + (sh.chunks_y - A.sky_bottom_begin) - sky->bands_filled;
        }
    }
    const int64_t n_items = sh.n_items;
    AMT_REQUIRE(ctx, n_items < (1ll << 31), "frame too large");
    AMT_REQUIRE(ctx, ((int64_t)p->width + 1) * ((int64_t)p->height + 1) * 8 < (1ll << 32),
                "frame too large (more than 2^29 pixel corners)");
    A.bbox_partials = nullptr;
    double* fold = nullptr;
    if (out->bbox) {
        const size_t need = (size_t)(n_items + kFoldBlocks) * 8 * sizeof(double);
        if (tail) {
            AMT_REQUIRE(ctx, tail->partials != nullptr && tail->partials_bytes >= need, "partials buffer too small");
            A.bbox_partials = tail->partials;
        } else {
            A.bbox_partials = static_cast<double*>(amt_workspace(ctx, need));
        }
        if (A.bbox_partials == nullptr) {
            ctx->last_error = "amt_georef_frame: workspace allocation failed";
            return AMT_ENOMEM;
        }
        fold = A.bbox_partials + n_items * 8;
    }
    AMT_REQUIRE(ctx, out->row_layout == AMT_ROWS_CONTIGUOUS || out->row_layout == AMT_ROWS_STRIP_PADDED, "unknown row_layout");
    AMT_REQUIRE(ctx, !A.row_layout || ((int64_t)p->height + 1) * sh.strips_x * 512 < (1ll << 32),
                "frame too large for strip-padded rows (32-bit byte offsets)");
    F->sh = sh;
    F->p = p;
    F->dirs = dirs;
    F->out = out;
    F->tail = tail;
    F->fold = fold;
    const bool mag = out->mlat != nullptr || out->mlat_c != nullptr || A.bin_magnetic;
    F->second = A.bin_pole ? (mag ? 3 : 2) : (mag ? 1 : 0);
    const bool no_geo_out = !A.lat && !A.lon && !A.lat_c && !A.lon_c;
    if (F->second == 1 && dirs == nullptr && no_geo_out) {
        if (bin ? A.bin_magnetic : (A.bin_magnetic || !out->bbox)) F->second = 4;
    }
    F->bin = bin;
    return AMT_OK;
}

int launch_prepared(amt_ctx* ctx, int n, prepared_frame* F) {
    AMT_REQUIRE(ctx, n >= 1 && n <= kMaxBatch, "bad batch size");
    bool together = n > 1;
    for (int i = 1; i < n && together; ++i)
        together = F[i].p->width == F[0].p->width && F[i].p->height == F[0].p->height &&
                   F[i].p->fast_center == F[0].p->fast_center && F[i].second == F[0].second && F[i].bin == F[0].bin &&
                   (F[i].dirs != nullptr) == (F[0].dirs != nullptr);
    if (n > 1 && !together) {
        for (int i = 0; i < n; ++i)
            if (int rc = launch_prepared(ctx, 1, F + i)) return rc;
        return AMT_OK;
    }
    const amt_frame_params* p = F[0].p;
    const double* dirs = F[0].dirs;
    const launch_shape& sh = F[0].sh;
    const int bin = F[0].bin, rows_per_chunk = sh.rows_per_chunk, strips_x = sh.strips_x;
    const int64_t n_items = sh.n_items;
    const int64_t nblocks = ((int64_t)n * n_items + kRowsThreads / 64 - 1) / (kRowsThreads / 64);
    AMT_REQUIRE(ctx, (int64_t)n * n_items < (1ll << 31), "launch too large");
    const dim3 grid((unsigned)nblocks);
    launch_events ev;
    amt_timing_pair(ctx, AMT_KERNEL_GEOREF, n, &ev.start, &ev.stop);
    for (int i = 0; i < n && ev.stop == nullptr; ++i)
        if (F[i].tail != nullptr && F[i].out->bbox) ev.stop = F[i].tail->kernel_done;
    georef_batch B;
    ctx->last_second = F[0].second, ctx->last_bin = bin, ctx->last_frames = n;
    for (int i = 0; i < kMaxBatch; ++i) B.f[i] = F[i < n ? i : 0].A;
    B.math = fx::make_math_table();
    if (dirs) {
        launch_rows<true, true>(ctx, B, n, grid, F[0].second, bin, rows_per_chunk, strips_x, (int)n_items, ev);
    } else if (p->fast_center) {
        launch_rows<true, false>(ctx, B, n, grid, F[0].second, bin, rows_per_chunk, strips_x, (int)n_items, ev);
    } else {
        launch_rows<false, false>(ctx, B, n, grid, F[0].second, bin, rows_per_chunk, strips_x, (int)n_items, ev);
    }
    AMT_LAUNCH_CHECK(ctx);
    bool folded[kMaxBatch] = {false, false, false};
    for (int i = 0; i < n; ++i) {
        if (!F[i].out->bbox || folded[i]) continue;
        hipStream_t fs = F[i].tail ? F[i].tail->stream : ctx->stream;
        if (F[i].tail) AMT_HIP(ctx, hipStreamWaitEvent(fs, ev.stop, 0));
        fold_batch s0, s1;
        int m = 0;
        for (int k = 0; k < kMaxBatch; ++k) s0.in[k] = s1.in[k] = nullptr, s0.out[k] = s1.out[k] = nullptr, s0.extra[k] = s1.extra[k] = nullptr;
        for (int k = i; k < n; ++k) {
            if (!F[k].out->bbox || folded[k] || (F[k].tail ? F[k].tail->stream : ctx->stream) != fs) continue;
            s0.in[m] = F[k].A.bbox_partials, s0.out[m] = F[k].fold;
            s1.in[m] = F[k].fold, s1.out[m] = F[k].out->bbox, s1.extra[m] = F[k].A.bin_event_count;
            folded[k] = true;
            ++m;
        }
        hipLaunchKernelGGL(k_bbox_fold_batch, dim3(kFoldBlocks, m), dim3(kThreads), 0, fs, s0, (int)n_items);
        hipLaunchKernelGGL(k_bbox_fold_batch, dim3(1, m), dim3(kThreads), 0, fs, s1, kFoldBlocks);
        AMT_LAUNCH_CHECK(ctx);
    }
    return AMT_OK;
}

}

size_t amt_georef_partials_bytes(const amt_frame_params* p) {
    return (size_t)(shape_of(p).n_items + kFoldBlocks) * 8 * sizeof(double);
}

int amt_georef_launch_many(amt_ctx* ctx, int n, const amt_frame_params* const* p, const double* const* dirs,
                           const amt_georef_out* const* out, const amt_georef_tail* const* tail, amt_sky_state* sky) {
    AMT_CHECK_CTX(ctx);
    AMT_REQUIRE(ctx, n >= 1 && n <= kMaxBatch && p && out, "bad batch");
    prepared_frame F[kMaxBatch];
    for (int i = 0; i < n; ++i) {
        AMT_REQUIRE(ctx, dirs == nullptr || dirs[i] != nullptr, "corner_dirs is NULL");
        if (int rc = prepare_georef(ctx, p[i], dirs ? dirs[i] : nullptr, out[i], tail ? tail[i] : nullptr, &F[i], sky ? sky + i : nullptr))
            return rc;
    }
    return launch_prepared(ctx, n, F);
}

extern "C" {

int amt_georef_frame(amt_ctx* ctx, const amt_frame_params* p, const amt_georef_out* out) {
    return amt_georef_launch_many(ctx, 1, &p, nullptr, &out, nullptr, nullptr);
}

namespace {
int coarse_bbox(amt_ctx* ctx, const amt_frame_params* p, const double* dirs, int32_t stride, double min_elevation, int magnetic,
                double* bbox);
}

int amt_georef_coarse_bbox(amt_ctx* ctx, const amt_frame_params* p, int32_t stride, double min_elevation,
                           int magnetic, double* bbox) {
    AMT_CHECK_CTX(ctx);
    return coarse_bbox(ctx, p, nullptr, stride, min_elevation, magnetic, bbox);
}

int amt_georef_coarse_bbox_dirs(amt_ctx* ctx, const amt_frame_params* p, const double* corner_dirs, int32_t stride,
                                double min_elevation, int magnetic, double* bbox) {
    AMT_CHECK_CTX(ctx);
    AMT_REQUIRE(ctx, corner_dirs != nullptr, "corner_dirs is NULL");
    AMT_REQUIRE(ctx, magnetic == 0 || magnetic == 1, "direction arrays have no pole plan: magnetic must be 0 or 1");
    return coarse_bbox(ctx, p, corner_dirs, stride, min_elevation, magnetic, bbox);
}

}

namespace {
int coarse_bbox(amt_ctx* ctx, const amt_frame_params* p, const double* dirs, int32_t stride, double min_elevation, int magnetic,
                double* bbox) {
    AMT_REQUIRE(ctx, p && bbox, "NULL argument");
    AMT_REQUIRE(ctx, p->width > 0 && p->height > 0 && stride > 0, "bad frame or stride");
    georef_args A;
    std::memset(&A, 0, sizeof(A));
    A.wcs = make_tan_wcs(p);
    A.ray = make_ray(p->a, p->b, p->cam, 1);
    A.m_geo = make_mat3(p->m_geo);
    A.m_sm = make_mat3(p->m_sm);
    A.bw = make_bowring_fast(p->a0, p->b0);
    A.pole = make_pole_consts(p->a0, p->b0, p->a - p->a0);
    A.width = p->width;
    A.height = p->height;
    const int nxl = (p->width + stride - 1) / stride + 1, nyl = (p->height + stride - 1) / stride + 1;
    const int nblocks = (nxl * nyl + kThreads - 1) / kThreads;
    double* partials = static_cast<double*>(amt_workspace(ctx, (size_t)nblocks * 8 * sizeof(double)));
    if (partials == nullptr) {
        ctx->last_error = "amt_georef_coarse_bbox: workspace allocation failed";
        return AMT_ENOMEM;
    }
    A.dirs_in = dirs;
    const int mode = (magnetic == 2 || magnetic == 3) ? magnetic : (magnetic ? 1 : 0);
    if (dirs)
        hipLaunchKernelGGL(k_coarse_bbox<true>, dim3(nblocks), dim3(kThreads), 0, ctx->stream, A, stride, mode, min_elevation, partials);
    else
        hipLaunchKernelGGL(k_coarse_bbox<false>, dim3(nblocks), dim3(kThreads), 0, ctx->stream, A, stride, mode, min_elevation, partials);
    AMT_LAUNCH_CHECK(ctx);
    hipLaunchKernelGGL(k_bbox_fold, dim3(1), dim3(kThreads), 0, ctx->stream, partials, nblocks, bbox,
                       (const unsigned int*)nullptr);
    AMT_LAUNCH_CHECK(ctx);
    return AMT_OK;
}
}

extern "C" {

int amt_georef_sky_rows(const amt_frame_params* p, int32_t* rows_per_item, int32_t* n_item_rows, int32_t* top_end,
                        int32_t* bottom_begin) {
    if (p == nullptr || rows_per_item == nullptr || n_item_rows == nullptr || top_end == nullptr || bottom_begin == nullptr)
        return AMT_EINVAL;
    if (p->width <= 0 || p->height <= 0) return AMT_EINVAL;
    georef_args A;
    std::memset(&A, 0, sizeof(A));
    camera_model(p, &A);
    const launch_shape sh = shape_of(p);
    int t = 0, b = sh.chunks_y;
    sky_bands(A, sh, &t, &b);
    *rows_per_item = sh.rows_per_chunk;
    *n_item_rows = sh.chunks_y;
    *top_end = t;
    *bottom_begin = b;
    return AMT_OK;
}

int64_t amt_padded_pitch(int32_t width) {
    if (width <= 0) return 0;
    amt_frame_params p;
    std::memset(&p, 0, sizeof(p));
    p.width = width, p.height = 1;
    return (int64_t)shape_of(&p).strips_x * 64;
}

int amt_georef_image_rows(const amt_frame_params* p, double min_elevation, int32_t* row_begin, int32_t* row_end) {
    if (p == nullptr || row_begin == nullptr || row_end == nullptr) return AMT_EINVAL;
    if (p->width <= 0 || p->height <= 0) return AMT_EINVAL;
    georef_args A;
    std::memset(&A, 0, sizeof(A));
    camera_model(p, &A);
    const launch_shape sh = shape_of(p);
    int t = 0, b = sh.chunks_y, te = 0, be = sh.chunks_y;
    sky_bands(A, sh, &t, &b);
    if (min_elevation > 0) elevation_bands(A, sh, min_elevation, &te, &be);
    t = std::max(t, te), b = std::min(b, be);
    if (t >= b) {
        *row_begin = *row_end = 0;
        return AMT_OK;
    }
    *row_begin = std::max(0, t * sh.rows_per_chunk);
    *row_end = std::min(p->height, b * sh.rows_per_chunk);
    return AMT_OK;
}

int amt_georef_frame_dirs(amt_ctx* ctx, const amt_frame_params* p, const double* corner_dirs,
                          const amt_georef_out* out) {
    return amt_georef_launch_many(ctx, 1, &p, &corner_dirs, &out, nullptr, nullptr);
}

}
```

### auromat_amd/csrc/amt_params.h

```cpp
#pragma once
#include <algorithm>
#include <cmath>
#include <cstring>

#include "../../include/auromat_hip.h"

namespace amt_prm {

constexpr double kDeg2Rad = 0.017453292519943295;
constexpr double kPi = 3.141592653589793;
constexpr double kWgs84A = 6378.137, kWgs84B = 6356.752314245179;

struct m3 {
    double v[9];
};

inline m3 mul(const m3& a, const m3& b) {
    m3 c;
    for (int i = 0; i < 3; ++i)
        for (int j = 0; j < 3; ++j) {
#ifdef AMT_PRM_NOFMA
            c.v[3 * i + j] = a.v[3 * i] * b.v[j] + a.v[3 * i + 1] * b.v[3 + j] + a.v[3 * i + 2] * b.v[6 + j];
#else
            double acc = a.v[3 * i] * b.v[j];
// ... 124 lines not shown
    return m;
}

inline int frame_params(const amt_run_frame* f, int32_t width, int32_t height, int32_t fast_center, double altitude,
                        int want_sm, amt_frame_params* p) {
    std::memset(p, 0, sizeof(*p));
    p->width = width;
    p->height = height;
    p->fast_center = fast_center ? 1 : 0;
    for (int i = 0; i < 4; ++i) p->cd[i] = f->cd[i];
    p->crpix[0] = f->crpix[0];
    p->crpix[1] = f->crpix[1];
    const m3 rot = euler_rzxz((f->crval[0] + 90) * kDeg2Rad, (90 - f->crval[1]) * kDeg2Rad, (-(f->lonpole - 90)) * kDeg2Rad);
    std::memcpy(p->rot, rot.v, sizeof(rot.v));
    for (int i = 0; i < 3; ++i) p->cam[i] = f->cam[i];
    p->a = kWgs84A + altitude;
    p->b = kWgs84B + altitude;
    p->a0 = kWgs84A;
    p->b0 = kWgs84B;
    const double et = (f->jd - 2451545) * 86400;
    const m3 geo = j2000_to_geo(et);
    std::memcpy(p->m_geo, geo.v, sizeof(geo.v));
    if (want_sm) {
        m3 sm;
        if (!j2000_to_sm(et, &sm)) return AMT_EINVAL;
        std::memcpy(p->m_sm, sm.v, sizeof(sm.v));
    }
    return AMT_OK;
}


inline int pole_in_view(const amt_frame_params* p, double min_elevation, int magnetic) {
    const double* m = magnetic ? p->m_sm : p->m_geo;
    const double* r = p->rot;
    const double sc[3] = {1 / p->a, 1 / p->a, 1 / p->b};
    for (int sign = 1; sign >= -1; sign -= 2) {
        double u[3], pole[3], los[3], d[3], n2 = 0;
        for (int i = 0; i < 3; ++i) u[i] = m[6 + i] * sign;
        for (int i = 0; i < 3; ++i) n2 += u[i] * sc[i] * u[i] * sc[i];
        double dist2 = 0;
        for (int i = 0; i < 3; ++i) {
            pole[i] = u[i] / std::sqrt(n2);
            los[i] = pole[i] - p->cam[i];
            dist2 += los[i] * los[i];
        }
        const double dist = std::sqrt(dist2);
        double d_o = 0, d_d = 0, o_o = 0;
        for (int i = 0; i < 3; ++i) {
            d[i] = los[i] / dist;
            const double ds = d[i] * sc[i], os = -p->cam[i] * sc[i];
            d_o += ds * os;
            d_d += ds * ds;
            o_o += os * os;
        }
        const double disc = d_o * d_o - o_o * d_d + d_d;
        if (disc < 0) continue;
        const double t = (o_o < 1 ? d_o + std::sqrt(disc) : d_o - std::sqrt(disc)) / d_d;
        if (std::fabs(t - dist) > 1e-6 * dist) continue;
        double v[3];
        for (int i = 0; i < 3; ++i) v[i] = r[i] * d[0] + r[3 + i] * d[1] + r[6 + i] * d[2];
        if (v[2] <= 0) continue;
        const double k = 180.0 / M_PI, bx = k * v[1] / v[2], by = -k * v[0] / v[2];
        const double det = p->cd[0] * p->cd[3] - p->cd[1] * p->cd[2];
        const double px = (bx * p->cd[3] - p->cd[1] * by) / det, py = (p->cd[0] * by - p->cd[2] * bx) / det;
        const double x = px + p->crpix[0] - 1, y = py + p->crpix[1] - 1;
        if (!(x >= -0.5 && x <= p->width - 0.5 && y >= -0.5 && y <= p->height - 0.5)) continue;
        if (!std::isinf(min_elevation)) {
            double dp = 0, pp = 0;
            for (int i = 0; i < 3; ++i) {
                dp += d[i] * pole[i];
                pp += pole[i] * pole[i];
            }
            double sn = -dp / std::sqrt(pp);
            sn = sn < -1 ? -1 : (sn > 1 ? 1 : sn);
            if (!(std::asin(sn) * k >= min_elevation)) continue;
        }
        return sign;
    }
    return 0;
}

inline bool all_within(const double* a, const double* b, int n, double tol) {
    for (int i = 0; i < n; ++i)
        if (std::fabs(a[i] - b[i]) > tol) return false;
    return true;
}

inline bool close_frames(const amt_frame_params& a, const amt_frame_params& b) {
    if (a.width != b.width || a.height != b.height || a.fast_center != b.fast_center) return false;
    if (std::fabs(a.a - b.a) > 30.0 || std::fabs(a.b - b.b) > 30.0) return false;
    double cd_max = 0;
    for (int i = 0; i < 4; ++i) cd_max = std::max(cd_max, std::fabs(a.cd[i]));
    return all_within(a.cam, b.cam, 3, 100.0) && all_within(a.rot, b.rot, 9, 0.01) && all_within(a.m_geo, b.m_geo, 9, 0.01) &&
           all_within(a.m_sm, b.m_sm, 9, 0.01) && all_within(a.cd, b.cd, 4, 0.01 * cd_max) && all_within(a.crpix, b.crpix, 2, 5.0);
}

inline bool steady_frames(const amt_frame_params& a, const amt_frame_params& b, const amt_frame_params& c, long long n_ab, long long n_bc) {
    if (n_ab <= 0 || n_bc <= 0 || n_bc > 16) return false;
    if (b.width != c.width || b.height != c.height || b.fast_center != c.fast_center) return false;
    if (std::fabs(b.a - c.a) > 30.0 || std::fabs(b.b - c.b) > 30.0) return false;
    if (!(all_within(b.cam, c.cam, 3, 400.0) && all_within(b.rot, c.rot, 9, 0.05) && all_within(b.m_geo, c.m_geo, 9, 0.05) &&
          all_within(b.m_sm, c.m_sm, 9, 0.05) && all_within(b.crpix, c.crpix, 2, 5.0)))
        return false;
    const double scale_b = std::sqrt(std::fabs(b.cd[0] * b.cd[3] - b.cd[1] * b.cd[2]));
    const double scale_c = std::sqrt(std::fabs(c.cd[0] * c.cd[3] - c.cd[1] * c.cd[2]));
    if (!(scale_b > 0 && std::fabs(scale_c - scale_b) <= 0.01 * scale_b)) return false;
    for (int i = 0; i < 4; ++i) {
        const double step = (b.cd[i] - a.cd[i]) / n_ab;
        if (std::fabs((c.cd[i] - b.cd[i]) - step * n_bc) > 0.3 * std::fabs(step * n_bc) + 0.01 * scale_b) return false;
    }
    for (int i = 0; i < 3; ++i) {
        const double step = (b.cam[i] - a.cam[i]) / n_ab;
        if (std::fabs((c.cam[i] - b.cam[i]) - step * n_bc) > 0.2 * std::fabs(step * n_bc) + 5.0) return false;
    }
    for (int i = 0; i < 9; ++i) {
        const double step = (b.rot[i] - a.rot[i]) / n_ab;
        if (std::fabs((c.rot[i] - b.rot[i]) - step * n_bc) > 0.3 * std::fabs(step * n_bc) + 2e-3) return false;
    }
    return true;
}

inline bool box_hint(const double* last_box, const amt_frame_params& last_p, long long last_index, const double* prev_box,
                     const amt_frame_params* prev_p, long long prev_index, long long k, const amt_frame_params& p, double* est) {
    if (close_frames(last_p, p)) {
        std::memcpy(est, last_box, 8 * sizeof(double));
        return true;
    }
    if (prev_box == nullptr || prev_p == nullptr || !close_frames(*prev_p, last_p) ||
        !steady_frames(*prev_p, last_p, p, last_index - prev_index, k - last_index))
        return false;
    if ((prev_box[7] != 0) != (last_box[7] != 0) || (last_box[3] - last_box[2] > 180) != (prev_box[3] - prev_box[2] > 180))
        return false;
    const double f = (double)(k - last_index) / (double)(last_index - prev_index);
    for (int i = 0; i < 6; ++i) est[i] = last_box[i] + f * (last_box[i] - prev_box[i]);
    est[6] = last_box[6], est[7] = last_box[7];
    est[0] = std::max(est[0], -90.0), est[1] = std::min(est[1], 90.0);
    for (int i = 2; i < 6; ++i) est[i] = std::min(std::max(est[i], -180.0), 180.0);
    return true;
}

struct sky_known {
    int top_end, bottom_begin;
};
constexpr int kSkyNoBottom = 0x7fffffff;
inline sky_known sky_known_empty() { return sky_known{0, kSkyNoBottom}; }

inline sky_known sky_fill(const sky_known& known, int n, int t, int b, int* fill_top_begin, int* fill_bottom_end) {
    const int kt = std::min(std::max(known.top_end, 0), n), kb = std::min(std::max(known.bottom_begin, 0), n);
    *fill_top_begin = std::min(kt, t);
    *fill_bottom_end = std::max(kb, b);
    return sky_known{t, b};
}

inline void conformal_sin_cos(double e, double s, double c, double* sin_chi, double* cos_chi) {
    const double es = e * s;
    const double w = std::exp(e * std::log((1.0 - es) / (1.0 + es)));
    const double plus = s >= 0 ? 1.0 + s : c * c / (1.0 - s);
    const double minus = s >= 0 ? c * c / (1.0 + s) : 1.0 - s;
    const double pw = plus * w, den = pw + minus;
    *sin_chi = (pw - minus) / den;
    *cos_chi = 2.0 * c * std::sqrt(w) / den;
}

constexpr double kPolarLimit = 1e-8;

inline int projection_stereographic(double lat0, double lon0, double a, double b, amt_projection* p) {
    if (p == nullptr) return AMT_EINVAL;
    std::memset(p, 0, sizeof(*p));
    if (!(std::isfinite(lat0) && std::isfinite(lon0) && std::isfinite(a) && std::isfinite(b))) return AMT_EINVAL;
    if (!(std::fabs(lat0) <= 90.0) || !(a > 0) || !(b > 0) || b > a) return AMT_EINVAL;
    const double e = std::sqrt((a - b) * (a + b)) / a;
    p->kind = AMT_PROJ_STEREOGRAPHIC;
    p->lat0 = lat0;
    p->lon0 = lon0;
    p->a = a;
    p->e = e;
    if (90.0 - std::fabs(lat0) < kPolarLimit) {
        p->mode = lat0 > 0 ? 1 : -1;
        p->sin_chi1 = p->mode;
        p->cos_chi1 = 0.0;
        p->m1 = 0.0;
        p->k = 2.0 * a / std::sqrt(std::pow(1.0 + e, 1.0 + e) * std::pow(1.0 - e, 1.0 - e));
        return AMT_OK;
    }
    const double colat = (90.0 - std::fabs(lat0)) * kDeg2Rad;
    const double s1 = std::fabs(lat0) > 45.0 ? std::copysign(std::cos(colat), lat0) : std::sin(lat0 * kDeg2Rad);
    const double c1 = std::fabs(lat0) > 45.0 ? std::sin(colat) : std::cos(lat0 * kDeg2Rad);
    conformal_sin_cos(e, s1, c1, &p->sin_chi1, &p->cos_chi1);
    p->mode = 0;
    p->m1 = c1 / std::sqrt(1.0 - (e * s1) * (e * s1));
    p->k = 2.0 * a * p->m1 / p->cos_chi1;
    return AMT_OK;
}

inline int projection_polar_aeqd(int north, double lon0, double radius, amt_projection* p) {
    if (p == nullptr) return AMT_EINVAL;
    std::memset(p, 0, sizeof(*p));
    if (!(std::isfinite(lon0) && std::isfinite(radius)) || !(radius > 0)) return AMT_EINVAL;
    p->kind = AMT_PROJ_POLAR_AEQD;
    p->mode = north ? 1 : -1;
    p->lat0 = north ? 90.0 : -90.0;
    p->lon0 = lon0;
    p->a = radius;
    p->e = 0.0;
    p->sin_chi1 = p->mode;
    p->cos_chi1 = 0.0;
    p->m1 = 0.0;
    p->k = radius;
    return AMT_OK;
}

}
```

### auromat_amd/csrc/amt_run.hip

```cpp
#include <algorithm>
#include <cstring>
#include <new>
#include <vector>

#include "amt_common.h"
#include "amt_grid.h"
#include "amt_params.h"

namespace {

struct slot {
    amt_pipe* pipe = nullptr;
    amt_georef_out out{};
    amt_frame_params prm{};
    double alt = 0;
    int hinted = 0;
    const void* img = nullptr;
    double ppd_lat = 0, ppd_lon = 0;
    int pre_status = 0;
    void* own_img = nullptr;
    hipEvent_t uploaded = nullptr, img_free = nullptr;
    bool upload_pending = false, img_busy = false;
    int64_t uploaded_bytes = 0;
    amt_prm::sky_known known = amt_prm::sky_known_empty();
};

struct batch { int k0, count; };
struct batch_queue {
    batch q[2];
    int n = 0;
    int size() const { return n; }
    const batch& front() const { return q[0]; }
    void push(batch b) { q[n++] = b; }
    void pop() { q[0] = q[1], --n; }
};

}

struct amt_run {
    amt_ctx* ctx = nullptr;
    amt_run_config cfg{};
    std::vector<slot> slots;
    hipEvent_t entry = nullptr;
    struct hint {
        bool valid = false;
        double box[8];
        amt_frame_params p;
        long long index;
    } last, prev;
    long long frames_done = 0;
    bool has_quantile = false;
    double quantile = 0.5;
    uint64_t min_weight = (uint64_t)1 << 31;
    uint32_t* over = nullptr;
    int over_capacity = 0;
    bool active = false, full = false;
    double* grids = nullptr;
    char* images = nullptr;
    int64_t grids_capacity = 0, images_capacity = 0, grid_used = 0, image_used = 0;
    amt_run_result* results = nullptr;
    int max_frames = 0, n_pushed = 0;
    batch collecting = {0, 0};
    batch_queue launched;
    batch_queue boxed;
    hipStream_t copy_stream = nullptr;
    hipStream_t launch_stream = nullptr;
    int64_t bands_filled = 0, bands_skipped = 0;

    slot& slot_of(int k) { return slots[k % cfg.n_slots]; }
};

namespace {

bool box_hint(const amt_run* run, long long k, const amt_frame_params& p, double* est) {
    const amt_run::hint &last = run->last, &prev = run->prev;
    return last.valid && amt_prm::box_hint(last.box, last.p, last.index, prev.valid ? prev.box : nullptr, &prev.p, prev.index, k, p, est);
}

void forget_hints(amt_run* run) { run->last.valid = run->prev.valid = false; }

void remember_hint(amt_run* run, const slot& s, int k, const double* box) {
    run->prev = run->last;
    run->last.valid = true;
    std::memcpy(run->last.box, box, sizeof(run->last.box));
    run->last.p = s.prm;
    run->last.index = run->frames_done + k;
}

void forget_sky(amt_run* run) { for (slot& s : run->slots) s.known = amt_prm::sky_known_empty(); }

int slot_image_create(amt_ctx* ctx, slot& s, size_t bytes) {
    void* buf = nullptr;
    hipEvent_t uploaded = nullptr, img_free = nullptr;
    if (hipMalloc(&buf, bytes) != hipSuccess) {
        (void)hipGetLastError();
        ctx->last_error = "amt_run_push: no device memory for a slot's image buffer";
        return AMT_ENOMEM;
    }
    hipError_t err = hipEventCreateWithFlags(&uploaded, hipEventDisableTiming);
    if (err == hipSuccess) err = hipEventCreateWithFlags(&img_free, hipEventDisableTiming);
    if (err != hipSuccess) {
        if (uploaded != nullptr) (void)hipEventDestroy(uploaded);
        (void)hipFree(buf);
        ctx->last_error = std::string("amt_run_push: event creation for a slot's image buffer -> ") + hipGetErrorString(err);
        return AMT_EHIP;
    }
    s.own_img = buf, s.uploaded = uploaded, s.img_free = img_free;
    return AMT_OK;
}

void slot_image_release(slot& s) {
    if (s.own_img == nullptr) return;
    (void)hipFree(s.own_img);
    (void)hipEventDestroy(s.uploaded);
    (void)hipEventDestroy(s.img_free);
    s.own_img = nullptr, s.uploaded = s.img_free = nullptr;
}

}

extern "C" {

int amt_frame_params_from_wcs(const amt_run_frame* frame, int32_t width, int32_t height, int32_t fast_center,
                              double altitude, int32_t want_sm, amt_frame_params* out) {
    if (frame == nullptr || out == nullptr || width <= 0 || height <= 0) return AMT_EINVAL;
    return amt_prm::frame_params(frame, width, height, fast_center, altitude, want_sm, out);
}

int amt_frames_close(const amt_frame_params* a, const amt_frame_params* b) {
    return a != nullptr && b != nullptr && amt_prm::close_frames(*a, *b) ? 1 : 0;
}

int amt_box_hint(const double* last_box, const amt_frame_params* last_p, int64_t last_index, const double* prev_box,
                 const amt_frame_params* prev_p, int64_t prev_index, int64_t k, const amt_frame_params* p, double* est8) {
    if (last_box == nullptr || last_p == nullptr || p == nullptr || est8 == nullptr) return 0;
    return amt_prm::box_hint(last_box, *last_p, last_index, prev_box, prev_p, prev_index, k, *p, est8) ? 1 : 0;
}

int amt_run_create(amt_ctx* ctx, const amt_run_config* config, amt_run** out_run) {
    AMT_CHECK_CTX(ctx);
    AMT_REQUIRE(ctx, config != nullptr && out_run != nullptr, "NULL argument");
    *out_run = nullptr;
    AMT_REQUIRE(ctx, config->width > 0 && config->height > 0, "empty frame");
    AMT_REQUIRE(ctx, config->img_dtype == 1 || config->img_dtype == 2, "img_dtype must be 1 (uint8) or 2 (uint16)");
    AMT_REQUIRE(ctx, config->batch >= 1 && config->batch <= AMT_PIPE_MAX_BATCH, "batch out of range");
    AMT_REQUIRE(ctx, config->n_slots >= 2 * config->batch && config->slots != nullptr, "n_slots must be at least 2 * batch");
    AMT_REQUIRE(ctx, config->arcsec_per_px > 0 || (config->lat_px_per_deg > 0 && config->lon_px_per_deg > 0), "px per degree must be positive");
    AMT_REQUIRE(ctx, config->statistic >= 0 && config->statistic <= 2, "statistic must be 0 (mean), 1 (median) or 2 (area-weighted)");
    AMT_REQUIRE(ctx, !(config->arcsec_per_px > 0) || ((config->statistic != 0 || !config->two_pass) && config->n_slots >= 3 * config->batch),
                "arcsec_per_px: the box-first plan is a single-pass plan and needs n_slots >= 3 * batch");
    amt_run* run = new (std::nothrow) amt_run();
    if (run == nullptr) return AMT_ENOMEM;
    run->ctx = ctx;
    run->cfg = *config;
    run->cfg.slots = nullptr;
    run->slots.resize(config->n_slots);
    if (amt_set_device(ctx)) {
        delete run;
        return AMT_EHIP;
    }
    for (int i = 0; i < config->n_slots; ++i) {
        slot& s = run->slots[i];
        s.out = config->slots[i];
        s.ppd_lat = config->lat_px_per_deg, s.ppd_lon = config->lon_px_per_deg;
        int rc = amt_pipe_create(ctx, &s.pipe);
        if (rc == AMT_OK) rc = amt_pipe_set_plan(s.pipe, config->statistic != 0 ? 2 : config->two_pass);
        if (rc != AMT_OK) {
            amt_run_destroy(run);
            return rc;
        }
    }
    if (hipEventCreateWithFlags(&run->entry, hipEventDisableTiming) != hipSuccess) {
        ctx->last_error = "amt_run_create: event creation failed";
        amt_run_destroy(run);
        return AMT_EHIP;
    }
    *out_run = run;
    return AMT_OK;
}

int amt_run_destroy(amt_run* run) {
    if (run == nullptr) return AMT_EINVAL;
    for (slot& s : run->slots)
        if (s.pipe != nullptr) amt_pipe_destroy(s.pipe);
    if (run->entry) (void)hipEventDestroy(run->entry);
    if (run->copy_stream) (void)hipStreamSynchronize(run->copy_stream);
    for (slot& s : run->slots) slot_image_release(s);
    if (run->copy_stream) (void)hipStreamDestroy(run->copy_stream);
    if (run->over) (void)hipFree(run->over);
    delete run;
    return AMT_OK;
}

int amt_run_set_quantile(amt_run* run, double q) {
    if (run == nullptr) return AMT_EINVAL;
    amt_ctx* ctx = run->ctx;
    AMT_REQUIRE(ctx, run->cfg.statistic == 1, "the runner was not created with statistic = 1");
    AMT_REQUIRE(ctx, !run->active && run->frames_done == 0, "to be called before the first push");
    AMT_REQUIRE(ctx, q >= 0.0 && q <= 1.0, "the quantile must lie in [0, 1]");
    run->has_quantile = true;
    run->quantile = q;
    return AMT_OK;
}

int amt_run_set_min_coverage(amt_run* run, uint64_t min_weight) {
    if (run == nullptr) return AMT_EINVAL;
    amt_ctx* ctx = run->ctx;
    AMT_REQUIRE(ctx, run->cfg.statistic == 2, "the runner was not created with statistic = 2");
    AMT_REQUIRE(ctx, !run->active && run->frames_done == 0, "to be called before the first push");
    run->min_weight = min_weight;
    return AMT_OK;
}

int amt_run_area_overflow(amt_run* run, int32_t* flags, int32_t n) {
    if (run == nullptr) return AMT_EINVAL;
    amt_ctx* ctx = run->ctx;
    AMT_CHECK_CTX(ctx);
    AMT_REQUIRE(ctx, run->cfg.statistic == 2, "the runner was not created with statistic = 2");
    AMT_REQUIRE(ctx, !run->active, "to be called after amt_run_end");
    AMT_REQUIRE(ctx, n >= 0 && n <= run->max_frames && (n == 0 || flags != nullptr), "n beyond the records of the last call");
    if (n == 0) return AMT_OK;
    if (amt_set_device(ctx)) return AMT_EHIP;
    static_assert(sizeof(int32_t) == sizeof(uint32_t), "one word per record");
    AMT_HIP(ctx, hipMemcpyAsync(flags, run->over, (size_t)n * sizeof(uint32_t), hipMemcpyDeviceToHost, ctx->stream));
    AMT_HIP(ctx, hipStreamSynchronize(ctx->stream));
    return AMT_OK;
}

int amt_run_fill_stats(amt_run* run, int64_t* bands_filled, int64_t* bands_skipped) {
    if (run == nullptr) return AMT_EINVAL;
    if (bands_filled) *bands_filled = run->bands_filled;
    if (bands_skipped) *bands_skipped = run->bands_skipped;
    return AMT_OK;
}

int amt_run_reset_hints(amt_run* run) {
    if (run == nullptr) return AMT_EINVAL;
    forget_hints(run);
    return AMT_OK;
}

}


namespace {

enum class pass { fused, general, ordered, area };

int choose_pass(const amt_run* run, const slot& s, amt_pipe_result* pr, pass* how) {
    const amt_run_config& cfg = run->cfg;
    const amt_georef_out& o = s.out;
    const double* b = pr->bbox;
    *how = pass::fused;
    if (cfg.statistic == 0) {
        if (pr->status != 1) return AMT_OK;
        if (int rc = amt_pipe_general_layout(s.pipe, pr)) return rc;
        if (pr->status == 0) *how = pass::general;
        return AMT_OK;
    }
    const pass second = cfg.statistic == 2 ? pass::area : pass::ordered;
    const bool have = second == pass::area ? (cfg.magnetic ? (o.mlat && o.mlt && o.mlat_c) : (o.lat && o.lon && o.lat_c))
                                           : (cfg.magnetic ? (o.mlat_c && o.mlt_c) : (o.lat_c && o.lon_c));
    if (pr->status == 0) *how = second;
    if (pr->status != 1 || b[7] != 0 || !cfg.fast_center || !have || !o.elev || o.row_layout != 0 || !(b[6] > 0)) return AMT_OK;
    if (!amt_gl::layout_of_box(s.ppd_lat, s.ppd_lon, b, &pr->grid, &pr->lon_wrapped)) return AMT_OK;
    pr->status = 0;
    *how = second;
    return AMT_OK;
}

int launch_slots(amt_run* run, const int* slots, int m, bool nothing_known = false) {
    amt_ctx* ctx = run->ctx;
    const amt_run_config& cfg = run->cfg;
    amt_pipe* pp[AMT_PIPE_MAX_BATCH];
    const amt_frame_params* prm[AMT_PIPE_MAX_BATCH];
    const amt_georef_out* oo[AMT_PIPE_MAX_BATCH];
    const void* ii[AMT_PIPE_MAX_BATCH];
    double la[AMT_PIPE_MAX_BATCH], lo[AMT_PIPE_MAX_BATCH];
    amt_sky_state sky[AMT_PIPE_MAX_BATCH];
    if (ctx->stream != run->launch_stream) forget_sky(run), run->launch_stream = ctx->stream;
    for (int j = 0; j < m; ++j) {
        slot& s = run->slots[slots[j]];
        s.out.altitude = s.alt;
        pp[j] = s.pipe, prm[j] = &s.prm, oo[j] = &s.out, ii[j] = s.img;
        la[j] = s.ppd_lat, lo[j] = s.ppd_lon;
        const amt_prm::sky_known known = nothing_known ? amt_prm::sky_known_empty() : s.known;
        sky[j] = {known.top_end, known.bottom_begin, 0, 0};
        if (s.img == nullptr) {
            ctx->last_error = "amt_run: a frame has no image";
            return AMT_EINVAL;
        }
        if (s.upload_pending) {
            AMT_HIP(ctx, hipStreamWaitEvent(ctx->stream, s.uploaded, 0));
            s.upload_pending = false;
        }
    }
    if (int rc = amt_pipe_launch_many_sky(pp, m, prm, oo, ii, cfg.img_dtype, cfg.min_elevation, la, lo, -1, cfg.magnetic ? 1 : 0, sky))
        return rc;
    for (int j = 0; j < m; ++j) {
        run->slots[slots[j]].known = {sky[j].known_top_end, sky[j].known_bottom_begin};
        run->bands_filled += sky[j].bands_filled, run->bands_skipped += sky[j].bands_skipped;
    }
    return AMT_OK;
}

struct frame_outputs {
    int64_t grid_doubles, image_bytes;
    double *mean, *count;
    void* image;
    uint8_t* mask;
};

bool next_outputs(const amt_run* run, int64_t cells, frame_outputs* f) {
    const int64_t pixel_bytes = cells * 3 * (run->cfg.img_dtype == 2 ? 2 : 1);
    f->grid_doubles = 5 * cells;
    f->image_bytes = (pixel_bytes + cells + 255) & ~(int64_t)255;
    if (run->full || run->grid_used + f->grid_doubles > run->grids_capacity || run->image_used + f->image_bytes > run->images_capacity)
        return false;
    f->mean = run->grids + run->grid_used, f->count = f->mean + 4 * cells;
    f->image = run->images + run->image_used;
    f->mask = reinterpret_cast<uint8_t*>(run->images + run->image_used + pixel_bytes);
    return true;
}

int second_pass(amt_run* run, pass how, int k, const amt_pipe_result& pr, const frame_outputs& f) {
    amt_ctx* ctx = run->ctx;
    const amt_run_config& cfg = run->cfg;
    slot& s = run->slot_of(k);
    const amt_georef_out& o = s.out;
    const bool mag = cfg.magnetic != 0;
    int rc = AMT_OK;
    if (how == pass::ordered) {
        rc = run->has_quantile
                 ? amt_quantile_frame_async(ctx, mag ? o.mlat_c : o.lat_c, mag ? o.mlt_c : o.lon_c, o.elev, s.img, cfg.img_dtype, 3,
                                            nullptr, cfg.height, cfg.width, cfg.min_elevation, &pr.grid.xaxis, &pr.grid.yaxis,
                                            pr.lon_wrapped, mag ? 1 : 0, &run->quantile, 1, f.mean, f.image, f.mask, f.count)
                 : amt_median_frame_async(ctx, mag ? o.mlat_c : o.lat_c, mag ? o.mlt_c : o.lon_c, o.elev, s.img, cfg.img_dtype, 3,
                                          nullptr, cfg.height, cfg.width, cfg.min_elevation, &pr.grid.xaxis, &pr.grid.yaxis,
                                          pr.lon_wrapped, mag ? 1 : 0, f.mean, f.image, f.mask, f.count);
    } else if (how == pass::area) {
        int32_t r0 = 0, r1 = cfg.height;
        if (int rc2 = amt_georef_image_rows(&s.prm, cfg.min_elevation, &r0, &r1)) return rc2;
        r0 = std::min(std::max(r0, 0), cfg.height);
        r1 = std::min(std::max(r1, r0), cfg.height);
        rc = amt_area_frame_async(ctx, mag ? o.mlat : o.lat, mag ? o.mlt : o.lon, mag ? o.mlat_c : o.lat_c, o.elev, s.img,
                                  cfg.img_dtype, 3, nullptr, cfg.height, cfg.width, cfg.min_elevation, &pr.grid.xaxis,
                                  &pr.grid.yaxis, pr.lon_wrapped, mag ? 1 : 0, r0, r1, run->min_weight, f.mean, f.image, f.mask,
                                  f.count, run->over + k);
    } else {
        rc = amt_pipe_general_finalize(s.pipe, f.mean, f.image, f.mask, f.count);
    }
    if (rc) return rc;
    if (s.img == s.own_img && s.own_img != nullptr) {
        AMT_HIP(ctx, hipEventRecord(s.img_free, ctx->stream));
        s.img_busy = true;
    }
    return AMT_OK;
}

int run_finish(amt_run* run, batch b) {
    const amt_run_config& cfg = run->cfg;
    amt_pipe* pp[AMT_PIPE_MAX_BATCH];
    double* mean[AMT_PIPE_MAX_BATCH];
    void* oimg[AMT_PIPE_MAX_BATCH];
    uint8_t* omask[AMT_PIPE_MAX_BATCH];
    double* ocount[AMT_PIPE_MAX_BATCH];
    int m = 0;
    for (int k = b.k0; k < b.k0 + b.count; ++k) {
        slot& s = run->slot_of(k);
        amt_run_result& r = run->results[k];
        std::memset(&r, 0, sizeof(r));
        r.slot = k % cfg.n_slots, r.hinted = s.hinted;
        r.altitude = s.alt, r.params = s.prm;
        r.lat_px_per_deg = s.ppd_lat, r.lon_px_per_deg = s.ppd_lon;
        r.uploaded_bytes = s.uploaded_bytes;
        if (s.pre_status != 0) {
            r.status = s.pre_status;
            forget_hints(run);
            continue;
        }
        amt_pipe_result pr;
        if (int rc = amt_pipe_wait(s.pipe, &pr)) return rc;
        if (pr.status == 1 && pr.fused && !cfg.two_pass && pr.bbox[6] > 0 && pr.edge_pixels <= AMT_PIPE_MAX_EDGE_PIXELS) {
            const int one = r.slot;
            if (int rc = amt_pipe_coarse_hint(s.pipe, pr.bbox, cfg.magnetic ? 1 : 0)) return rc;
            if (int rc = launch_slots(run, &one, 1, true)) return rc;
            if (int rc = amt_pipe_wait(s.pipe, &pr)) return rc;
            r.retried = 1;
        }
        pass how;
        if (int rc = choose_pass(run, s, &pr, &how)) return rc;
        r.status = pr.status;
        r.two_pass = how != pass::fused ? 1 : 0;
        std::memcpy(r.bbox, pr.bbox, sizeof(r.bbox));
        r.edge_pixels = pr.edge_pixels;
        if (pr.status != 0) {
            forget_hints(run);
            continue;
        }
        frame_outputs f;
        if (!next_outputs(run, (int64_t)pr.grid.ny * pr.grid.nx, &f)) {
            run->full = true;
            r.status = 3;
            continue;
        }
        r.ny = pr.grid.ny, r.nx = pr.grid.nx;
        r.contains_pole = pr.bbox[7] != 0 ? 1 : 0;
        r.lon_wrapped = pr.lon_wrapped;
        r.grid = pr.grid;
        r.grid_offset = run->grid_used, r.image_offset = run->image_used;
        if (how == pass::fused) {
            pp[m] = s.pipe;
            mean[m] = f.mean, ocount[m] = f.count, oimg[m] = f.image, omask[m] = f.mask;
            ++m;
        } else if (int rc = second_pass(run, how, k, pr, f)) {
            return rc;
        }
        run->grid_used += f.grid_doubles;
        run->image_used += f.image_bytes;
        remember_hint(run, s, k, pr.bbox);
    }
    if (m > 0)
        if (int rc = amt_pipe_finalize_many(pp, m, mean, oimg, omask, ocount)) return rc;
    return AMT_OK;
}

int run_launch(amt_run* run, batch b) {
    int slots[AMT_PIPE_MAX_BATCH];
    for (int i = 0; i < b.count; ++i) {
        int m = 0;
        for (; i < b.count && run->slot_of(b.k0 + i).pre_status == 0; ++i) slots[m++] = (b.k0 + i) % run->cfg.n_slots;
        if (m > 0)
            if (int rc = launch_slots(run, slots, m)) return rc;
    }
    return AMT_OK;
}

int run_box(amt_run* run, batch b) {
    amt_pipe* pp[AMT_PIPE_MAX_BATCH];
    const amt_frame_params* prm[AMT_PIPE_MAX_BATCH];
    for (int i = 0; i < b.count; ++i) {
        slot& s = run->slot_of(b.k0 + i);
        pp[i] = s.pipe, prm[i] = &s.prm;
        s.pre_status = 0;
    }
    return amt_pipe_launch_box_many(pp, b.count, prm, run->cfg.min_elevation, run->cfg.magnetic ? 1 : 0);
}

int run_resolve(amt_run* run, batch b) {
    const amt_run_config& cfg = run->cfg;
    for (int i = 0; i < b.count; ++i) {
        slot& s = run->slot_of(b.k0 + i);
        amt_pipe_result pr;
        if (int rc = amt_pipe_wait(s.pipe, &pr)) return rc;
// ... 40 lines not shown
    return AMT_OK;
}

int run_batch_ready_box(amt_run* run, batch b) {
    if (run->boxed.size() == 2)
        if (int rc = run_launch_boxed(run)) return rc;
    if (run->full) {
        mark_not_processed(run, b);
        return AMT_OK;
    }
    if (int rc = run_box(run, b)) return rc;
    run->boxed.push(b);
    return AMT_OK;
}

int run_batch_ready(amt_run* run, batch b) {
    if (run->cfg.arcsec_per_px > 0) return run_batch_ready_box(run, b);
    if (run->launched.size() == 2) {
        if (int rc = run_finish(run, run->launched.front())) return rc;
        run->launched.pop();
    }
    if (run->full) {
        mark_not_processed(run, b);
        return AMT_OK;
    }
    if (int rc = run_launch(run, b)) return rc;
    run->launched.push(b);
    return AMT_OK;
}

int run_upload(amt_run* run, slot& s, const void* host) {
    amt_ctx* ctx = run->ctx;
    const amt_run_config& cfg = run->cfg;
    const size_t row_bytes = (size_t)cfg.width * 3 * (cfg.img_dtype == 2 ? 2 : 1);
    if (run->copy_stream == nullptr) AMT_HIP(ctx, hipStreamCreateWithFlags(&run->copy_stream, hipStreamNonBlocking));
    if (s.own_img == nullptr)
        if (int rc = slot_image_create(ctx, s, row_bytes * cfg.height)) return rc;
    int32_t r0 = 0, r1 = cfg.height;
    if (int rc = amt_georef_image_rows(&s.prm, cfg.min_elevation, &r0, &r1)) return rc;
    if (s.img_busy) {
        AMT_HIP(ctx, hipStreamWaitEvent(run->copy_stream, s.img_free, 0));
        s.img_busy = false;
    }
    if (r1 > r0) {
        AMT_HIP(ctx, hipMemcpyAsync(static_cast<char*>(s.own_img) + (size_t)r0 * row_bytes,
                                    static_cast<const char*>(host) + (size_t)r0 * row_bytes, (size_t)(r1 - r0) * row_bytes,
                                    hipMemcpyHostToDevice, run->copy_stream));
        AMT_HIP(ctx, hipEventRecord(s.uploaded, run->copy_stream));
        s.upload_pending = true;
    }
    s.uploaded_bytes = (int64_t)(r1 - r0) * (int64_t)row_bytes;
    s.img = s.own_img;
    return AMT_OK;
}

int run_push_impl(amt_run* run, const amt_run_frame* f) {
    amt_ctx* ctx = run->ctx;
    AMT_CHECK_CTX(ctx);
    AMT_REQUIRE(ctx, run->active, "amt_run_push without amt_run_begin");
    AMT_REQUIRE(ctx, f != nullptr, "NULL frame");
    AMT_REQUIRE(ctx, run->n_pushed < run->max_frames, "more frames than amt_run_begin announced");
    const amt_run_config& cfg = run->cfg;
    const int k = run->n_pushed++;
    mark_not_processed(run, {k, 1});
    if (run->full) return AMT_OK;
    for (;;) {
        if (run->launched.size() > 0 && run->launched.front().k0 <= k - cfg.n_slots) {
            if (int rc = run_finish(run, run->launched.front())) return rc;
            run->launched.pop();
            if (run->full) return AMT_OK;
            continue;
        }
        if (run->boxed.size() > 0 && run->boxed.front().k0 <= k - cfg.n_slots) {
            if (int rc = run_launch_boxed(run)) return rc;
            continue;
        }
        break;
    }
    slot& s = run->slot_of(k);
    const int mag = cfg.magnetic ? 1 : 0;
    const double altitude = f->altitude > 0 ? f->altitude : cfg.altitude;
    const int want_sm = mag || s.out.mlat != nullptr || s.out.mlat_c != nullptr;
    int rc = amt_prm::frame_params(f, cfg.width, cfg.height, cfg.fast_center, altitude, want_sm, &s.prm);
    if (rc != AMT_OK) {
        ctx->last_error = "amt_run_push: the date of a frame is outside the IGRF table";
        return rc;
    }
    s.alt = altitude;
    s.img = f->img;
    s.uploaded_bytes = 0;
    s.upload_pending = false;
    if (f->img == nullptr && f->img_host != nullptr)
        if (int rc2 = run_upload(run, s, f->img_host)) return rc2;
    s.pre_status = 0;
    if (!(cfg.arcsec_per_px > 0)) {
        double est[8];
        const bool hint = cfg.use_hints && box_hint(run, run->frames_done + k, s.prm, est);
        rc = hint ? amt_pipe_coarse_hint(s.pipe, est, mag) : amt_pipe_coarse(s.pipe, &s.prm, cfg.min_elevation, mag);
        if (rc != AMT_OK) return rc;
        s.hinted = hint ? 1 : 0;
    }
    if (run->collecting.count == 0) run->collecting.k0 = k;
    ++run->collecting.count;
    if (run->collecting.count == (k == 0 && !(cfg.arcsec_per_px > 0) ? 1 : cfg.batch)) {
        rc = run_batch_ready(run, run->collecting);
        run->collecting.count = 0;
    }
    return rc;
}

}

extern "C" {

int amt_run_begin(amt_run* run, double* grids, int64_t grids_capacity, void* images, int64_t images_capacity,
                  amt_run_result* results, int32_t max_frames) {
    if (run == nullptr) return AMT_EINVAL;
    amt_ctx* ctx = run->ctx;
    AMT_CHECK_CTX(ctx);
    AMT_REQUIRE(ctx, !run->active, "amt_run_begin: a call is already in progress (amt_run_end it first)");
    AMT_REQUIRE(ctx, max_frames >= 0 && (max_frames == 0 || results != nullptr), "NULL argument");
    AMT_REQUIRE(ctx, max_frames == 0 || (grids != nullptr && images != nullptr), "the arenas are NULL");
    if (amt_set_device(ctx)) return AMT_EHIP;
    void* fin = nullptr;
    if (int rc = amt_pipe_finalize_stream(run->slots[0].pipe, &fin)) return rc;
    AMT_HIP(ctx, hipEventRecord(run->entry, ctx->stream));
    AMT_HIP(ctx, hipStreamWaitEvent(static_cast<hipStream_t>(fin), run->entry, 0));
    if (run->cfg.statistic == 2 && max_frames > 0) {
        if (max_frames > run->over_capacity) {
            if (run->over) (void)hipFree(run->over);
            run->over = nullptr;
            run->over_capacity = 0;
            const int cap = std::max(max_frames, 64);
            if (hipMalloc(reinterpret_cast<void**>(&run->over), (size_t)cap * sizeof(uint32_t)) != hipSuccess) {
                (void)hipGetLastError();
                run->over = nullptr;
                ctx->last_error = "amt_run_begin: no device memory for the overflow flags";
                return AMT_ENOMEM;
            }
            run->over_capacity = cap;
        }
        AMT_HIP(ctx, hipMemsetAsync(run->over, 0, (size_t)max_frames * sizeof(uint32_t), ctx->stream));
    }
    run->grids = grids, run->grids_capacity = grids_capacity;
    run->images = static_cast<char*>(images), run->images_capacity = images_capacity;
    run->results = results, run->max_frames = max_frames;
    run->grid_used = run->image_used = 0;
    run->full = false;
    run->n_pushed = 0;
    run->collecting = {0, 0}, run->launched = {}, run->boxed = {};
    forget_sky(run);
    run->launch_stream = ctx->stream;
    run->bands_filled = run->bands_skipped = 0;
    run->active = true;
    return AMT_OK;
}

int amt_run_push(amt_run* run, const amt_run_frame* f) {
    if (run == nullptr) return AMT_EINVAL;
    const int rc = run_push_impl(run, f);
    if (rc != AMT_OK) forget_hints(run), forget_sky(run);
    return rc;
}

int amt_run_end(amt_run* run, int32_t* frames_done) {
    if (run == nullptr) return AMT_EINVAL;
    amt_ctx* ctx = run->ctx;
    AMT_CHECK_CTX(ctx);
    AMT_REQUIRE(ctx, run->active, "amt_run_end without amt_run_begin");
    run->active = false;
    int rc_all = AMT_OK;
    if (run->collecting.count > 0) {
        rc_all = run_batch_ready(run, run->collecting);
        run->collecting.count = 0;
    }
    while (run->boxed.size() > 0 && rc_all == AMT_OK) rc_all = run_launch_boxed(run);
    for (; run->launched.size() > 0; run->launched.pop()) {
        const int rc = run_finish(run, run->launched.front());
        if (rc_all == AMT_OK) rc_all = rc;
    }
    if (run->copy_stream != nullptr && hipStreamSynchronize(run->copy_stream) != hipSuccess && rc_all == AMT_OK) {
        (void)hipGetLastError();
        ctx->last_error = "amt_run_end: the copy stream failed";
        rc_all = AMT_EHIP;
    }
    for (slot& s : run->slots) {
        s.upload_pending = false;
        const int rc = amt_pipe_join(s.pipe);
        if (rc_all == AMT_OK) rc_all = rc;
    }
    if (rc_all != AMT_OK) {
        forget_hints(run), forget_sky(run);
        if (frames_done) *frames_done = 0;
        return rc_all;
    }
    const int n = run->n_pushed;
    int done = n;
    for (int i = 0; i < n; ++i)
        if (run->results[i].status == 3) {
            done = i;
            break;
        }
    for (int i = done; i < n; ++i) run->results[i].status = 3;
    if (frames_done) *frames_done = done;
    run->frames_done += done;
    if (done < n) forget_hints(run);
    return AMT_OK;
}

int amt_run_process(amt_run* run, const amt_run_frame* frames, int32_t n, double* grids, int64_t grids_capacity,
                    void* images, int64_t images_capacity, amt_run_result* results, int32_t* frames_done) {
    if (run == nullptr) return AMT_EINVAL;
    amt_ctx* ctx = run->ctx;
    AMT_CHECK_CTX(ctx);
    AMT_REQUIRE(ctx, n >= 0 && (n == 0 || frames != nullptr), "NULL argument");
    if (frames_done) *frames_done = 0;
    if (n == 0) return AMT_OK;
    if (int rc = amt_run_begin(run, grids, grids_capacity, images, images_capacity, results, n)) return rc;
    int rc_all = AMT_OK;
    for (int i = 0; i < n && rc_all == AMT_OK; ++i) rc_all = amt_run_push(run, frames + i);
    const int rc = amt_run_end(run, frames_done);
    return rc_all != AMT_OK ? rc_all : rc;
}

}
```

### include/auromat_hip.h

```cpp
#ifndef AUROMAT_HIP_H
#define AUROMAT_HIP_H

#include <stddef.h>
#include <stdint.h>

#ifdef __cplusplus
extern "C" {
#endif

#define AMT_ABI_VERSION 10

#define AMT_OK 0
#define AMT_EINVAL (-1)
#define AMT_EHIP (-2)
#define AMT_ENOMEM (-3)
#define AMT_EEMPTY (-4)
#define AMT_EDOMAIN (-5)

typedef struct amt_ctx amt_ctx;


int amt_abi_version(void);
int amt_ctx_create(int device_id, void* stream, int own_stream, amt_ctx** out_ctx);
int amt_ctx_destroy(amt_ctx* ctx);
int amt_ctx_set_stream(amt_ctx* ctx, void* stream);
void* amt_ctx_get_stream(amt_ctx* ctx);
int amt_ctx_synchronize(amt_ctx* ctx);
const char* amt_last_error(amt_ctx* ctx);
int amt_device_info(amt_ctx* ctx, char* name, size_t name_len, int* compute_units, int* clock_khz,
                    size_t* total_mem);

int amt_malloc(amt_ctx* ctx, size_t bytes, void** out_dptr);
int amt_free(amt_ctx* ctx, void* dptr);
int amt_host_threads(int wanted, int* cores, int* local_ranks);
int amt_malloc_host(amt_ctx* ctx, size_t bytes, void** out_hptr);
int amt_free_host(amt_ctx* ctx, void* hptr);
int amt_memcpy_h2d(amt_ctx* ctx, void* dst, const void* src, size_t bytes);
int amt_memcpy_d2h(amt_ctx* ctx, void* dst, const void* src, size_t bytes);
int amt_memset(amt_ctx* ctx, void* dst, int value, size_t bytes);
int amt_upload_staged(amt_ctx* ctx, void* dst_device, const void* src_host, size_t bytes);
int amt_download_staged(amt_ctx* ctx, void* dst_host, const void* src_device, size_t bytes);
int amt_event_create(amt_ctx* ctx, void** out_event);
int amt_event_destroy(amt_ctx* ctx, void* event);
int amt_event_record(amt_ctx* ctx, void* event);
int amt_event_elapsed_ms(amt_ctx* ctx, void* start, void* stop, float* out_ms);
#define AMT_KERNEL_GEOREF 0
#define AMT_KERNEL_BIN 1
int amt_timing_enable(amt_ctx* ctx, int enable);
int amt_timing_read(amt_ctx* ctx, int kernel, double* total_ms, int* launches);
int amt_georef_last_variant(amt_ctx* ctx, int32_t* second, int32_t* bin, int32_t* frames);

typedef struct amt_frame_params {
    int32_t width;
    int32_t height;
    int32_t fast_center;
    int32_t reserved;
    double cd[4];
    double crpix[2];
    double rot[9];
    double cam[3];
    double a, b;
    double a0, b0;
    double m_geo[9];
    double m_sm[9];
} amt_frame_params;

struct amt_axis;

typedef struct amt_georef_out {
    double* lat;
    double* lon;
    double* lat_c;
    double* lon_c;
    double* elev;
    double* mlat;
    double* mlt;
    double* mlat_c;
    double* mlt_c;
    double* bbox;
    double bbox_min_elevation;
    const struct amt_axis* bin_xaxis;
    const struct amt_axis* bin_yaxis;
    const void* bin_img;
    uint64_t* bin_acc;
    int32_t bin_img_dtype;
    int32_t bin_lon_wrap;
    int32_t bin_magnetic;
    int32_t item_order;
    void* bin_events;
    uint32_t* bin_event_count;
    int64_t bin_event_capacity;
    int32_t bin_pole;
    int32_t row_layout;
    double altitude;
} amt_georef_out;
#define AMT_ROWS_CONTIGUOUS 0
#define AMT_ROWS_STRIP_PADDED 1
int64_t amt_padded_pitch(int32_t width);
int amt_unpad_rows(amt_ctx* ctx, const double* src_padded, int32_t rows, int32_t cols, int32_t width, double* dst);


int amt_directions_tan(amt_ctx* ctx, const amt_frame_params* p, int corner, double* out_dirs);
#define AMT_SIP_MAX 10
typedef struct amt_zenithal_wcs {
    int32_t width, height, corner, projection;
    double cd[4], crpix[2], rot[9];
    double start_x, start_y;
    int32_t sip_order_a, sip_order_b;
    double sip_a[AMT_SIP_MAX][AMT_SIP_MAX], sip_b[AMT_SIP_MAX][AMT_SIP_MAX];
} amt_zenithal_wcs;
int amt_directions_zenithal(amt_ctx* ctx, const amt_zenithal_wcs* w, double* out_dirs);
int amt_directions_tan_points(amt_ctx* ctx, const amt_frame_params* p, const double* px, const double* py,
                              int64_t n, int origin, double* out_dirs);

#define AMT_LENS_NONE 0
#define AMT_LENS_POLY3 1
#define AMT_LENS_POLY5 2
#define AMT_LENS_PTLENS 3
typedef struct amt_lens_model {
    int32_t kind, width, height;
    int32_t crop_x, crop_y, crop_width, crop_height, reserved;
    double k[3];
} amt_lens_model;
int amt_lens_coords(amt_ctx* ctx, const amt_lens_model* model, int32_t x0, int32_t y0, int32_t cols, int32_t rows, int corner,
                    double* out_xy, float* out_xy32);
int amt_lens_undistort(amt_ctx* ctx, const amt_lens_model* model, int32_t x0, int32_t y0, int32_t cols, int32_t rows, int corner,
                       double* out_xy);
#define AMT_INTERP_LINEAR 0
#define AMT_INTERP_LANCZOS4 1
#define AMT_LENS_PATH_AUTO 0
#define AMT_LENS_PATH_STAGED 1
#define AMT_LENS_PATH_GATHER 2
#define AMT_LENS_TILE 32
typedef struct amt_lens_debug {
    int32_t force_path, reserved;
    uint8_t* tile_path;
} amt_lens_debug;
int amt_lens_remap(amt_ctx* ctx, const amt_lens_model* model, const void* src, int32_t sample_bytes, int32_t channels,
                   int32_t interpolation, void* dst, uint8_t* support, const amt_lens_debug* debug);
int amt_remap_coords(amt_ctx* ctx, const void* src, int32_t src_width, int32_t src_height, int32_t sample_bytes, int32_t channels,
                     const float* coords, int32_t dst_width, int32_t dst_height, int32_t interpolation, void* dst, uint8_t* support,
                     const amt_lens_debug* debug);

#define AMT_W2P_GEODETIC 0
#define AMT_W2P_SM 1
#define AMT_W2P_J2000 2
#define AMT_W2P_INVALID 1
#define AMT_W2P_HIDDEN 2
#define AMT_W2P_UNPROJECTABLE 4
#define AMT_W2P_NOT_CONVERGED 8
#define AMT_W2P_OUTSIDE 16
int amt_world_to_pixel(amt_ctx* ctx, const amt_frame_params* params, const amt_zenithal_wcs* zenithal, int32_t frame,
                       const double* c0, const double* c1, int64_t n, double* out_xy, double* out_elev, uint8_t* out_flags);
int amt_grid_to_pixel(amt_ctx* ctx, const amt_frame_params* params, const amt_zenithal_wcs* zenithal, int32_t frame,
                      const double* lat_centres, int32_t ny, const double* lon_centres, int32_t nx, float* out_xy32, double* out_xy,
                      double* out_elev, uint8_t* out_flags);

int amt_intersect_ellipsoid(amt_ctx* ctx, double a, double b, const double* origin, const double* dirs,
                            int64_t n, int directed, double* out_xyz);
int amt_intersects_ellipsoid(amt_ctx* ctx, double a, double b, const double* origin, const double* dirs,
                             int64_t n, int directed, uint8_t* out_hit);
int amt_intersect_sphere(amt_ctx* ctx, double radius, const double* origin, const double* dirs,
                         int64_t n, int directed, double* out_xyz);

int amt_ecef_to_geodetic(amt_ctx* ctx, const double* x, const double* y, const double* z, int64_t n,
                         double a, double b, double* out_lat, double* out_lon);
int amt_geodetic_to_ecef(amt_ctx* ctx, const double* lat, const double* lon, double h, int64_t n,
                         double a, double b, double* out_x, double* out_y, double* out_z);
int amt_rotate_to_latlon(amt_ctx* ctx, const double* m, const double* xyz, int64_t n, double a0, double b0,
                         double* out_lat_deg, double* out_lon_deg);
int amt_rotate_to_mlat_mlt(amt_ctx* ctx, const double* m, const double* xyz, int64_t n,
                           double* out_mlat_deg, double* out_mlt_h);
int amt_rotate_vectors(amt_ctx* ctx, const double* m, const double* xyz, int64_t n, double* out_xyz);
int amt_latlon_to_mlat_mlt(amt_ctx* ctx, const double* m, const double* lat_deg, const double* lon_deg,
                           double h, int64_t n, double a0, double b0, double* out_mlat_deg, double* out_mlt_h);
int amt_sm_to_latlon(amt_ctx* ctx, const double* m_sm_to_geo, const double* smlat_deg, const double* smlon_deg,
                     int64_t n, double a0, double b0, double* out_lat_deg, double* out_lon_deg);

#define AMT_PROJ_STEREOGRAPHIC 1
#define AMT_PROJ_POLAR_AEQD 2
typedef struct amt_projection {
    int32_t kind;
    int32_t mode;
    double lat0, lon0;
    double a, e;
    double sin_chi1, cos_chi1;
    double m1;
    double k;
    double reserved[4];
} amt_projection;
int amt_projection_stereographic(double lat0, double lon0, double a, double b, amt_projection* out);
int amt_projection_polar_aeqd(int north, double lon0, double radius, amt_projection* out);
int amt_project_forward(amt_ctx* ctx, const amt_projection* p, const double* lat_deg, const double* lon_deg, int64_t n,
                        double* out_x, double* out_y);
int amt_project_inverse(amt_ctx* ctx, const amt_projection* p, const double* x, const double* y, int64_t n,
                        double* out_lat_deg, double* out_lon_deg);
int amt_rotate_pole(amt_ctx* ctx, const double* rot, const double* lat, const double* lon, double altitude,
                    int64_t n, double a0, double b0, double* out_lat, double* out_lon);
int amt_rotate_pole_deg(amt_ctx* ctx, const double* rot, const double* lat_deg, const double* lon_deg, double altitude,
                        int64_t n, double a0, double b0, double* out_lat_deg, double* out_lon_deg);
int amt_cartesian_to_spherical(amt_ctx* ctx, const double* x, const double* y, const double* z, int64_t n,
                               double* out_r, double* out_lat, double* out_lon);
int amt_spherical_to_cartesian(amt_ctx* ctx, const double* r, const double* lat, const double* lon, int64_t n,
// ... 157 lines not shown
                         int32_t nplane, int32_t row_base, int32_t col_base, int32_t NY, int32_t NX, double* planes, void* img,
                         uint8_t* mask, int32_t* frame_index);
int amt_hist2d_finalize_mean(amt_ctx* ctx, const double* count, const double* const* sums, int32_t nweights,
                             int32_t nx, int32_t ny, double* mean);


int amt_nearest_frame(amt_ctx* ctx, const double* lat_c, const double* lon_c, const double* elev,
                      const uint8_t* center_mask, int32_t height, int32_t width, double min_elevation,
                      const amt_axis* xaxis, const amt_axis* yaxis, int lon_wrap, const double* target_lat,
                      const double* target_lon, const uint8_t* target_mask, int64_t* out_index);
int amt_nearest_gather(amt_ctx* ctx, const int64_t* index, int64_t n_targets, const void* img, int32_t img_dtype,
                       int32_t nchan, const double* elev, double* mean, void* out_img, uint8_t* out_mask);
typedef struct amt_delaunay amt_delaunay;
int amt_delaunay_create(const double* xy, int64_t n, amt_delaunay** out);
int amt_delaunay_create_threads(const double* xy, int64_t n, int32_t threads, int64_t parallel_min, amt_delaunay** out);
int amt_delaunay_build_info(const amt_delaunay* d, int64_t* info2);
int amt_delaunay_destroy(amt_delaunay* d);
int amt_delaunay_sizes(const amt_delaunay* d, int64_t* n_triangles, int64_t* n_neighbours, int64_t* n_duplicates);
int amt_delaunay_stats(const amt_delaunay* d, int64_t* stats4);
int amt_delaunay_triangles(const amt_delaunay* d, int32_t* simplices, int32_t* neighbours);
int amt_delaunay_slots(const amt_delaunay* d, const int32_t** vertices, const uint8_t** dead, int64_t* n_slots);
int amt_delaunay_vertex_neighbours(const amt_delaunay* d, int64_t* indptr, int32_t* indices);
int amt_delaunay_locate(const amt_delaunay* d, const double* targets, int64_t m, int32_t* vertices, double* centroids,
                        uint8_t* has_neighbour);
int amt_cubic_gradients_csr(amt_ctx* ctx, const double* xy, int64_t n, const int64_t* indptr, const int32_t* indices,
                            const int64_t* row_start, int32_t n_rows, const double* values, int32_t nchan, double tolerance,
                            int32_t max_iterations, double* gradients, int32_t* iterations);
int amt_cubic_eval(amt_ctx* ctx, int64_t m, const double* targets, const int32_t* vertices, const double* centroids,
                   const uint8_t* has_neighbour, const double* xy, const double* values, const double* gradients, int32_t nchan,
                   double* out);
int amt_points_in_polygon(amt_ctx* ctx, const double* px, const double* py, int64_t n, const double* polygon,
                          int32_t n_vertices, uint8_t* out_inside);


typedef struct amt_grid {
    int32_t nx, ny;
    int32_t n_lat_nodes, n_lon_nodes;
    double lat_lo, lat_hi, lon_lo, lon_hi;
    double lat_step, lon_step;
    double lat_center_first, lat_center_last, lon_center_first, lon_center_last;
    amt_axis xaxis, yaxis;
} amt_grid;
int amt_grid_layout(double lat_px_per_deg, double lon_px_per_deg, double lat_min, double lat_max,
                    double lon_min, double lon_max, amt_grid* out);

typedef struct amt_pipe amt_pipe;
#define AMT_PIPE_MAX_EDGE_PIXELS 16384
typedef struct amt_pipe_result {
    int32_t status;
    int32_t fused;
    int32_t lon_wrapped;
    int32_t edge_pixels;
    double bbox[8];
    amt_grid grid;
} amt_pipe_result;
int amt_pipe_create(amt_ctx* ctx, amt_pipe** out_pipe);
int amt_pipe_destroy(amt_pipe* pipe);
int amt_pipe_coarse(amt_pipe* pipe, const amt_frame_params* p, double min_elevation, int magnetic);
int amt_pipe_coarse_hint(amt_pipe* pipe, const double* bbox, int magnetic);
int amt_pipe_launch(amt_pipe* pipe, const amt_frame_params* p, const amt_georef_out* out, const void* img,
                    int32_t img_dtype, double min_elevation, double lat_px_per_deg, double lon_px_per_deg,
                    int pole_in_view, int magnetic);
int amt_pipe_coarse_dirs(amt_pipe* pipe, const amt_frame_params* p, const double* corner_dirs, double min_elevation,
                         int magnetic);
int amt_pipe_launch_dirs(amt_pipe* pipe, const amt_frame_params* p, const double* corner_dirs, const amt_georef_out* out,
                         const void* img, int32_t img_dtype, double min_elevation, double lat_px_per_deg,
                         double lon_px_per_deg, int pole_in_view, int magnetic);
int amt_pipe_launch_dirs_many(amt_pipe* const* pipes, int32_t n, const amt_frame_params* const* p, const double* const* corner_dirs,
                              const amt_georef_out* const* out, const void* const* img, int32_t img_dtype, double min_elevation,
                              double lat_px_per_deg, double lon_px_per_deg, int pole_in_view, int magnetic);
#define AMT_PIPE_MAX_BATCH 3
int amt_pipe_launch_many(amt_pipe* const* pipes, int32_t n, const amt_frame_params* const* p,
                         const amt_georef_out* const* out, const void* const* img, int32_t img_dtype,
                         double min_elevation, double lat_px_per_deg, double lon_px_per_deg, int pole_in_view,
                         int magnetic);
int amt_pipe_launch_many_res(amt_pipe* const* pipes, int32_t n, const amt_frame_params* const* p,
                             const amt_georef_out* const* out, const void* const* img, int32_t img_dtype,
                             double min_elevation, const double* lat_px_per_deg, const double* lon_px_per_deg,
                             int pole_in_view, int magnetic);
int amt_pipe_launch_box(amt_pipe* pipe, const amt_frame_params* p, double min_elevation, int magnetic);
int amt_pipe_launch_box_many(amt_pipe* const* pipes, int32_t n, const amt_frame_params* const* p, double min_elevation,
                             int magnetic);
int amt_plate_carree_resolution(double lat_south, double lon_west, double lat_north, double lon_east, double arcsec_per_px,
                                double* lat_px_per_deg, double* lon_px_per_deg);
int amt_pipe_wait(amt_pipe* pipe, amt_pipe_result* result);
int amt_pipe_finalize(amt_pipe* pipe, double* mean, void* out_img, uint8_t* out_mask, double* out_count);
int amt_pipe_finalize_many(amt_pipe* const* pipes, int32_t n, double* const* mean, void* const* out_img,
                           uint8_t* const* out_mask, double* const* out_count);
int amt_pipe_finalize_stream(amt_pipe* pipe, void** stream);
int amt_pipe_join(amt_pipe* pipe);
int amt_pipe_set_plan(amt_pipe* pipe, int two_pass);
int amt_pipe_general_layout(amt_pipe* pipe, amt_pipe_result* result);
int amt_pipe_general_finalize(amt_pipe* pipe, double* mean, void* out_img, uint8_t* out_mask, double* out_count);

typedef struct amt_run amt_run;
typedef struct amt_run_config {
    int32_t width, height;
    int32_t img_dtype;
    int32_t fast_center;
    int32_t magnetic;
    int32_t batch;
    int32_t use_hints;
    int32_t n_slots;
    int32_t two_pass;
    int32_t statistic;
    double altitude;
    double min_elevation;
    double lat_px_per_deg, lon_px_per_deg;
    const amt_georef_out* slots;
    double arcsec_per_px;
} amt_run_config;
typedef struct amt_run_frame {
    double crval[2], crpix[2], cd[4], lonpole;
    double cam[3];
    double jd;
    double altitude;
    const void* img;
    const void* img_host;
} amt_run_frame;
typedef struct amt_run_result {
    int32_t status, slot;
    int32_t ny, nx;
    int32_t contains_pole;
    int32_t lon_wrapped;
    int32_t hinted;
    int32_t edge_pixels;
    int32_t two_pass;
    int32_t reserved_;
    int64_t grid_offset;
    int64_t image_offset;
    double bbox[8];
    double altitude;
    amt_grid grid;
    amt_frame_params params;
    double lat_px_per_deg, lon_px_per_deg;
    int32_t retried, reserved2_;
    int64_t uploaded_bytes;
} amt_run_result;
int amt_frame_params_from_wcs(const amt_run_frame* frame, int32_t width, int32_t height, int32_t fast_center,
                              double altitude, int32_t want_sm, amt_frame_params* out);
int amt_pole_in_view(const amt_frame_params* p, double min_elevation, int magnetic);
int amt_frames_close(const amt_frame_params* a, const amt_frame_params* b);
int amt_box_hint(const double* last_box, const amt_frame_params* last_p, int64_t last_index, const double* prev_box,
                 const amt_frame_params* prev_p, int64_t prev_index, int64_t k, const amt_frame_params* p, double* est8);
int amt_run_create(amt_ctx* ctx, const amt_run_config* config, amt_run** out_run);
int amt_run_destroy(amt_run* run);
int amt_run_process(amt_run* run, const amt_run_frame* frames, int32_t n, double* grids, int64_t grids_capacity,
                    void* images, int64_t images_capacity, amt_run_result* results, int32_t* frames_done);
int amt_run_begin(amt_run* run, double* grids, int64_t grids_capacity, void* images, int64_t images_capacity,
                  amt_run_result* results, int32_t max_frames);
int amt_run_push(amt_run* run, const amt_run_frame* frame);
int amt_run_end(amt_run* run, int32_t* frames_done);
int amt_run_fill_stats(amt_run* run, int64_t* bands_filled, int64_t* bands_skipped);
int amt_run_reset_hints(amt_run* run);
int amt_run_set_quantile(amt_run* run, double q);
int amt_run_set_min_coverage(amt_run* run, uint64_t min_weight);
int amt_run_area_overflow(amt_run* run, int32_t* flags, int32_t n);

#define AMT_SEQ_DESC_LEN 12
typedef struct amt_seq_frame {
    int32_t ny, nx, nc;
    int32_t index;
    double lat0, lon0, dlat, dlon;
    int32_t contains_pole, contains_discontinuity, magnetic, reserved;
    double altitude;
    const double* mean;
    const double* count;
} amt_seq_frame;
int amt_seq_payload_size(const amt_seq_frame* frames, int32_t n, int64_t* n_doubles);
int amt_seq_pack(amt_ctx* ctx, const amt_seq_frame* frames, int32_t n, int32_t max_frames, double* buffer,
                 int64_t capacity_doubles);
int amt_seq_unpack(const double* host_buffer, int64_t n_doubles, int32_t n_frames, int32_t max_frames,
                   amt_seq_frame* out, int32_t capacity, int32_t* n_out);

#ifdef __cplusplus
}
#endif
#endif
```

Before: 65800.

## Specialize georef row bands into inner, low-elevation and generic roles

Host-side conic tests classify each row band as fully inside the valid shell/elevation region (inner), entirely below the minimum elevation (low), or mixed (generic). The kernel is compiled per role so inner bands skip hit/elevation/corner checks and ballots, and low bands skip pixel loading and binning. The change also adds launch-bound variants for the plain and exact-magnetic kernels and counts valid pixels with a ballot popcount instead of a shuffle reduction. The risks are misclassified bands near the conservative margins, which would give wrong bounding boxes or bins, and more code paths, which raise register pressure.

Measured after the change: 66840, median of 6. +1.6%, better.

```diff
diff --git a/auromat_amd/_native.py b/auromat_amd/_native.py
--- a/auromat_amd/_native.py
+++ b/auromat_amd/_native.py
@@ -189,6 +189,9 @@
     'amt_georef_frame': ([_P, C.POINTER(FrameParams), C.POINTER(GeorefOut)], _I),
     'amt_georef_frame_dirs': ([_P, C.POINTER(FrameParams), _P, C.POINTER(GeorefOut)], _I),
     'amt_georef_coarse_bbox': ([_P, C.POINTER(FrameParams), C.c_int32, _D, _I, _P], _I),
+    'amt_georef_set_roles': ([_P, _I], _I),
+    'amt_georef_last_roles': ([_P, C.POINTER(C.c_int64), C.POINTER(C.c_int64), C.POINTER(C.c_int64)], _I),
+    'amt_georef_band_roles': ([C.POINTER(FrameParams), _D, C.POINTER(C.c_int32), C.POINTER(C.c_int32)], _I),
     'amt_delaunay_create': ([_P, C.c_int64, C.POINTER(C.c_void_p)], _I),
     'amt_delaunay_destroy': ([_P], _I),
     'amt_delaunay_sizes': ([_P, C.POINTER(C.c_int64), C.POINTER(C.c_int64), C.POINTER(C.c_int64)], _I),
@@ -280,6 +283,7 @@
     'amt_run_end': ([_P, C.POINTER(C.c_int32)], _I),
     'amt_run_reset_hints': ([_P], _I),
     'amt_run_fill_stats': ([_P, C.POINTER(C.c_int64), C.POINTER(C.c_int64)], _I),
+    'amt_run_role_stats': ([_P, C.POINTER(C.c_int64), C.POINTER(C.c_int64), C.POINTER(C.c_int64)], _I),
     'amt_run_set_quantile': ([_P, _D], _I),
     'amt_run_set_min_coverage': ([_P, C.c_uint64], _I),
     'amt_run_area_overflow': ([_P, C.POINTER(C.c_int32), C.c_int32], _I),
diff --git a/auromat_amd/csrc/amt_common.h b/auromat_amd/csrc/amt_common.h
--- a/auromat_amd/csrc/amt_common.h
+++ b/auromat_amd/csrc/amt_common.h
@@ -32,6 +32,8 @@
     std::string last_error;
     hipStream_t aux_pre, aux_tail, aux_fin;
     int last_second, last_bin, last_frames;
+    int roles_off;
+    long long last_role_items[3];
     int timing;
     size_t tlaunch[2];
     int tframes[2];
@@ -70,6 +72,7 @@
 struct amt_sky_state {
     int known_top_end, known_bottom_begin;
     int bands_filled, bands_skipped;
+    long long role_items[3];
 };
 int amt_georef_launch_many(amt_ctx* ctx, int n, const amt_frame_params* const* p, const double* const* dirs,
                            const amt_georef_out* const* out, const amt_georef_tail* const* tail, amt_sky_state* sky);
diff --git a/auromat_amd/csrc/amt_context.hip b/auromat_amd/csrc/amt_context.hip
--- a/auromat_amd/csrc/amt_context.hip
+++ b/auromat_amd/csrc/amt_context.hip
@@ -23,6 +23,8 @@
     ctx->timing = 0;
     ctx->copier = nullptr;
     ctx->last_second = ctx->last_bin = ctx->last_frames = -1;
+    ctx->roles_off = 0;
+    ctx->last_role_items[0] = ctx->last_role_items[1] = ctx->last_role_items[2] = -1;
     ctx->aux_pre = ctx->aux_tail = ctx->aux_fin = nullptr;
     ctx->tlaunch[0] = ctx->tlaunch[1] = 0;
     ctx->tframes[0] = ctx->tframes[1] = 0;
@@ -258,4 +260,18 @@
     return AMT_OK;
 }
 
-}
+int amt_georef_set_roles(amt_ctx* ctx, int enable) {
+    AMT_CHECK_CTX(ctx);
+    ctx->roles_off = enable ? 0 : 1;
+    return AMT_OK;
+}
+
+int amt_georef_last_roles(amt_ctx* ctx, int64_t* generic, int64_t* inner, int64_t* low) {
+    AMT_CHECK_CTX(ctx);
+    if (generic) *generic = ctx->last_role_items[0];
+    if (inner) *inner = ctx->last_role_items[1];
+    if (low) *low = ctx->last_role_items[2];
+    return AMT_OK;
+}
+
+}
diff --git a/auromat_amd/csrc/amt_georef.hip b/auromat_amd/csrc/amt_georef.hip
--- a/auromat_amd/csrc/amt_georef.hip
+++ b/auromat_amd/csrc/amt_georef.hip
@@ -88,6 +88,7 @@
     int item_order;
     int sky_top_end, sky_bottom_begin;
     int fill_top_begin, fill_bottom_end;
+    int inner_begin, inner_end, low_top_end, low_bottom_begin;
     int bin_pole;
     int row_layout;
     pole_consts pole;
@@ -153,6 +154,12 @@
         out[k] = r;
     }
 }
+
+constexpr int kRoleGeneric = 0, kRoleInner = 1, kRoleLow = 2;
+template <int ROLE>
+struct role_tag {
+    static constexpr int value = ROLE;
+};
 
 constexpr int kDppWaveShl1 = 0x130;
 constexpr int kDppWaveShr1 = 0x138;
@@ -252,8 +259,14 @@
 #ifndef AMT_ROWS_MIN_WAVES_MAGONLY
 #define AMT_ROWS_MIN_WAVES_MAGONLY 4
 #endif
+#ifndef AMT_ROWS_MIN_WAVES_PLAIN
+#define AMT_ROWS_MIN_WAVES_PLAIN 6
+#endif
+#ifndef AMT_ROWS_MIN_WAVES_MAG_EXACT
+#define AMT_ROWS_MIN_WAVES_MAG_EXACT 4
+#endif
 template <bool FAST, bool DIRS_IN, int SECOND, int BIN>
-__global__ __launch_bounds__(kRowsThreads, SECOND == 4 ? AMT_ROWS_MIN_WAVES_MAGONLY : (SECOND >= 2 ? AMT_ROWS_MIN_WAVES_POLE : (SECOND == 1 && BIN ? AMT_ROWS_MIN_WAVES_MAG : (BIN ? AMT_ROWS_MIN_WAVES_BIN : AMT_ROWS_MIN_WAVES)))) void k_georef_rows(georef_batch B, int rows_per_chunk, int strips_x,
+__global__ __launch_bounds__(kRowsThreads, (!DIRS_IN && SECOND == 0 && BIN == 0) ? AMT_ROWS_MIN_WAVES_PLAIN : (!FAST && SECOND == 1 && BIN != 0) ? AMT_ROWS_MIN_WAVES_MAG_EXACT : SECOND == 4 ? AMT_ROWS_MIN_WAVES_MAGONLY : (SECOND >= 2 ? AMT_ROWS_MIN_WAVES_POLE : (SECOND == 1 && BIN ? AMT_ROWS_MIN_WAVES_MAG : (BIN ? AMT_ROWS_MIN_WAVES_BIN : AMT_ROWS_MIN_WAVES)))) void k_georef_rows(georef_batch B, int rows_per_chunk, int strips_x,
                                                            int n_items, int n_frames) {
     constexpr bool MAG = SECOND != 0, kPole = SECOND == 2, kMagPole = SECOND == 3, kMagOnly = SECOND == 4;
     static_assert(!(kPole || kMagPole) || (BIN != 0 && !DIRS_IN), "the pole plans exist for fused binning with the camera model only");
@@ -408,7 +421,8 @@
     const bool geo_pole = kMagPole && !A.bin_magnetic;
     const bool centre_coords = BIN != 0 || A.lat_c != nullptr || A.lon_c != nullptr || (MAG && A.mlat_c != nullptr);
     int n_valid = 0;
-    auto box_add = [&](double la_v, double lo_v) {
+    const bool box_lane = px_ok || (lane >= 1 && col_ok);
+    auto box_add =[&](double la_v, double lo_v) {
         __hip_atomic_fetch_min(&sBox[wave][0][lane], la_v, __ATOMIC_RELAXED, __HIP_MEMORY_SCOPE_WORKGROUP);
         __hip_atomic_fetch_max(&sBox[wave][1][lane], la_v, __ATOMIC_RELAXED, __HIP_MEMORY_SCOPE_WORKGROUP);
         __hip_atomic_fetch_min(&sBox[wave][2][lane], lo_v, __ATOMIC_RELAXED, __HIP_MEMORY_SCOPE_WORKGROUP);
@@ -592,14 +606,15 @@
         vec3 rv;
         double rxy, rla, rlo;
     };
-    auto step = [&](const int r, const bool even, const vec3& dj, const row_state& prev, row_state& cur) {
+    auto step = [&](auto role, const int r, const bool even, const vec3& dj, const row_state& prev, row_state& cur) __attribute__((always_inline)) {
+        constexpr int ROLE = decltype(role)::value;
         const int gy = y0 + r;
         unsigned int ch0 = 0, ch1 = 0, ch2 = 0;
         const shell_ray& ry = ray;
         const vec3 u = corner_ray(gy, dj);
         const double uu = fx::dot3(u.x, u.y, u.z, u.x, u.y, u.z);
         const double t = shell_t(ry, u, uu);
-        const bool hit = col_ok && t >= 0.0;
+        const bool hit = ROLE == kRoleInner ? col_ok : (col_ok && t >= 0.0);
         vec3 d;
         if (DIRS_IN) {
             d = u;
@@ -610,7 +625,7 @@
         }
         corner_vals c;
         const bool magbox = MAG && (kMagOnly || (BIN && !kPole && A.bin_magnetic));
-        if (__builtin_amdgcn_ballot_w64(hit) != 0) {
+        if (ROLE == kRoleInner || __builtin_amdgcn_ballot_w64(hit) != 0) {
             c.p = shell_point(ry, u, nan_unless(hit, t));
             c.la = c.lo = c.bn = c.bd = NAN;
             if (!kMagOnly) {
@@ -651,7 +666,7 @@
             if (pole_bin) c.bla = c.sml, c.blo = c.ssl;
             if (kMagBox && !magbox && !pole_bin && !kMagPole) c.bla = c.la, c.blo = c.lo;
         }
-        if (BIN) take_pixel(r, even, ch0, ch1, ch2);
+        if (BIN && ROLE != kRoleLow) take_pixel(r, even, ch0, ch1, ch2);
         const bool owner = st_corner && (r < rows || gy == frame_h);
         if (owner) {
             if (!kMagOnly) {
@@ -691,12 +706,12 @@
                 dscale = 1.0;
                 const double tc = shell_t(ry, uc, uuc);
                 pc = shell_point(ry, uc, nan_unless(tc >= 0.0, tc));
-                if (want_bbox) {
+                if (ROLE == kRoleGeneric && want_bbox) {
                     const int h = (prev.p.x == prev.p.x) && (c.p.x == c.p.x);
                     corners_ok = h && from_next_lane(h);
                 }
             }
-            const bool live = px_ok && pc.x == pc.x;
+            const bool live = ROLE == kRoleInner ? px_ok : (px_ok && pc.x == pc.x);
             double lac, loc, el, ml = NAN, mt = NAN, slc = NAN, rlac = NAN, rloc = NAN;
             if (__builtin_amdgcn_ballot_w64(live) != 0) {
                 double inv_r, cn = NAN, cd = NAN;
@@ -743,7 +758,7 @@
                     at(A.mlt_c, off_pixel) = mt;
                 }
             }
-            const bool valid = px_ok && (el >= min_elev) && corners_ok;
+            const bool valid = ROLE == kRoleInner ? px_ok : (ROLE == kRoleLow ? false : (px_ok && (el >= min_elev) && corners_ok));
             int bin_x = 0, bin_y = 0;
             long long el_fix = 0;
             if (BIN && valid) {
@@ -791,11 +806,16 @@
                     }
                 }
             }
-            if (BIN) bin_account(bin_x, bin_y, ch0, ch1, ch2, el_fix);
-            if (want_bbox) {
+            if (BIN && ROLE != kRoleLow) bin_account(bin_x, bin_y, ch0, ch1, ch2, el_fix);
+            if (ROLE == kRoleInner) {
+                flag_cur = box_lane ? 1 : 0;
+                if (want_bbox && box_lane) {
+                    if (kMagBox) box_add(prev.bla, prev.blo); else box_add(prev.la, prev.lo);
+                }
+            } else if (ROLE == kRoleGeneric && want_bbox) {
                 const int vi = valid ? 1 : 0;
                 flag_cur = vi | from_prev_lane(vi);
-                n_valid += vi;
+                n_valid += __builtin_popcountll(__builtin_amdgcn_ballot_w64(valid));
                 if (kMagBox) {
                     if ((prev.flag | flag_cur) && prev.bla == prev.bla) box_add(prev.bla, prev.blo);
                 } else {
@@ -828,7 +848,7 @@
         cur.flag = flag_cur;
     };
 
-    auto advance = [&](const int r, const bool even, const row_state& prev, row_state& cur) {
+    auto advance = [&](auto role, const int r, const bool even, const row_state& prev, row_state& cur) __attribute__((always_inline)) {
         vec3 dj = {dj0, dj1, dj2};
         if (DIRS_IN) {
             asm volatile("" : "+v"(dj.x), "+v"(dj.y), "+v"(dj.z));
@@ -837,15 +857,29 @@
                 dj0 = q[0], dj1 = q[1], dj2 = q[2];
             }
         }
-        step(r, even, dj, prev, cur);
+        step(role, r, even, dj, prev, cur);
         off_corner += pitch_corner;
         off_pixel += pitch_pixel;
         img_off += img_row;
     };
-    if (BIN && px_ok && rows > 0) load_pixel(img_off + img_row, rawB0, rawB1, shiftB);
-    for (int r = 0; r <= rows; r += 2) {
-        advance(r, true, S0, S1);
-        if (r + 1 <= rows) advance(r + 1, false, S1, S0); else S0 = S1;
+    auto march = [&](auto role) __attribute__((always_inline)) {
+        constexpr int ROLE = decltype(role)::value;
+        if (BIN && ROLE != kRoleLow && px_ok && rows > 0) load_pixel(img_off + img_row, rawB0, rawB1, shiftB);
+        if (ROLE == kRoleInner) n_valid = __builtin_popcountll(__builtin_amdgcn_ballot_w64(px_ok)) * rows;
+        for (int r = 0; r <= rows; r += 2) {
+            advance(role, r, true, S0, S1);
+            if (r + 1 <= rows) advance(role, r + 1, false, S1, S0); else S0 = S1;
+        }
+    };
+    if constexpr (DIRS_IN || kPole || kMagPole) {
+        march(role_tag<kRoleGeneric>{});
+    } else {
+        if (chunk >= A.inner_begin && chunk < A.inner_end)
+            march(role_tag<kRoleInner>{});
+        else if (BIN != 0 && (chunk < A.low_top_end || chunk >= A.low_bottom_begin))
+            march(role_tag<kRoleLow>{});
+        else
+            march(role_tag<kRoleGeneric>{});
     }
     if (BIN && bin_anchor) {
         if (run_key) bin_flush(run_key, run_cnt, run_c0, run_c1, run_c2, run_el);
@@ -873,11 +907,10 @@
         } else {
             if (S0.flag && S0.la == S0.la) box_add(S0.la, S0.lo);
         }
-        double v[7];
+        double v[6];
 #pragma unroll
         for (int k = 0; k < 6; ++k)
             v[k] = __hip_atomic_load(&sBox[wave][k][lane], __ATOMIC_RELAXED, __HIP_MEMORY_SCOPE_WORKGROUP);
-        v[6] = (double)n_valid;
         for (int o = 32; o > 0; o >>= 1) {
             v[0] = fmin(v[0], __shfl_xor(v[0], o));
             v[1] = fmax(v[1], __shfl_xor(v[1], o));
@@ -885,11 +918,10 @@
             v[3] = fmax(v[3], __shfl_xor(v[3], o));
             v[4] = fmin(v[4], __shfl_xor(v[4], o));
             v[5] = fmax(v[5], __shfl_xor(v[5], o));
-            v[6] += __shfl_xor(v[6], o);
         }
         if (lane < 8) A.bbox_partials[(int64_t)item * 8 + lane] = lane == 0 ? v[0] : lane == 1 ? v[1] : lane == 2 ? v[2]
                                                                   : lane == 3 ? v[3] : lane == 4 ? v[4]
-                                                                  : lane == 5 ? v[5] : lane == 6 ? v[6] : 0.0;
+                                                                  : lane == 5 ? v[5] : lane == 6 ? (double)n_valid : 0.0;
     }
 }
 
@@ -1052,7 +1084,7 @@
 }
 
 template <class Eval>
-void conic_bands(double W, double H, int n, int rows_per_chunk, Eval eval, int* top_end, int* bottom_begin) {
+void conic_bands(double W, double H, int n, int rows_per_chunk, Eval eval, int* top_end, int* bottom_begin, double margin_px = 1.0) {
     *top_end = 0, *bottom_begin = n;
     struct quad {
         double a, b, c, L;
@@ -1074,7 +1106,7 @@
         q.b = (f2 - f0) / L - q.a * L;
         return q;
     };
-    const double x0 = -1.0, xL = W + 2.0, y0 = -1.0, yL = H + 2.0;
+    const double x0 = -margin_px, xL = W + 2.0 * margin_px, y0 = -margin_px, yL = H + 2.0 * margin_px;
     double nb00, nb10, nb01, tmp;
     quad col[3];
     double scale = 0;
@@ -1109,7 +1141,7 @@
         return segment_free(col[k], nb00 + (k == 2 ? nbx * xL : 0.0), nby, s0, s1);
     };
     auto band_free = [&](int c) {
-        const double s0 = (double)c * rows_per_chunk, s1 = std::min((double)(c + 1) * rows_per_chunk, H) + 2.0;
+        const double s0 = (double)c * rows_per_chunk, s1 = std::min((double)(c + 1) * rows_per_chunk, H) + 2.0 * margin_px;
         return line_free(s0) && line_free(s1) && side_free(0, s0, s1) && side_free(2, s0, s1);
     };
     int t = 0;
@@ -1150,7 +1182,7 @@
     conic_bands((double)A.width, (double)A.height, n, sh.rows_per_chunk, eval, top_end, bottom_begin);
 }
 
-void elevation_bands(const georef_args& A, const launch_shape& sh, double min_elev_deg, int* top_end, int* bottom_begin) {
+void elevation_bands(const georef_args& A, const launch_shape& sh, double min_elev_deg, int* top_end, int* bottom_begin, bool tight = false) {
     const int n = sh.chunks_y;
     *top_end = 0, *bottom_begin = n;
     const shell_ray& e = A.sray;
@@ -1172,9 +1204,51 @@
         return uo * uo - cos2 * oo * uu;
     };
     int t = 0, b = n;
-    conic_bands((double)A.width, (double)A.height, n, sh.rows_per_chunk, eval, &t, &b);
-    *top_end = std::max(0, t - 1), *bottom_begin = std::min(n, b + 1);
+    tight = tight && min_elev_deg >= 5.0;
+    conic_bands((double)A.width, (double)A.height, n, sh.rows_per_chunk, eval, &t, &b, tight ? 3.0 : 1.0);
+    const int extra = tight ? 0 : 1;
+    *top_end = std::max(0, t - extra), *bottom_begin = std::min(n, b + extra);
     if (t == n) *top_end = n, *bottom_begin = n;
+}
+
+void inner_bands(const georef_args& A, const launch_shape& sh, double min_elev_deg, int* begin, int* end) {
+    *begin = *end = 0;
+    const shell_ray& e = A.sray;
+    if (!(e.root_sign < 0) || min_elev_deg != min_elev_deg) return;
+    const double e0 = std::max(min_elev_deg, 0.0) + 0.05;
+    if (!(e0 < 89.0)) return;
+    const double oo = e.ox * e.ox + e.oy * e.oy + e.oz * e.oz;
+    const double r_min = 1.0 / std::sqrt(std::max(e.qa, e.qa + e.qd));
+    const double k = r_min / std::sqrt(oo) * std::cos(e0 * kDeg2Rad);
+    if (!(k > 0.0 && k < 1.0)) return;
+    const double cos2 = 1.0 - k * k;
+    auto inside = [&](double x, double y) {
+        const affine_cam& c = A.cam;
+        const double px = x + c.cx, py = y + c.cy;
+        const double ux = c.u0[0] + px * c.ux[0] + py * c.uy[0], uy = c.u0[1] + px * c.ux[1] + py * c.uy[1],
+                     uz = c.u0[2] + px * c.ux[2] + py * c.uy[2];
+        const double uu = ux * ux + uy * uy + uz * uz;
+        const double uo = ux * e.ox + uy * e.oy + uz * e.oz;
+        return uo < 0 && uo * uo - cos2 * oo * uu > 1e-9 * (oo * uu);
+    };
+    const double margin = 2.0, xa = -margin, xb = (double)A.width + margin;
+    auto band_inside = [&](int c) {
+        const double ya = (double)c * sh.rows_per_chunk - margin;
+        const double yb = std::min((double)(c + 1) * sh.rows_per_chunk, (double)A.height) + margin;
+        return inside(xa, ya) && inside(xb, ya) && inside(xa, yb) && inside(xb, yb);
+    };
+    int b = 0;
+    while (b < sh.chunks_y && !band_inside(b)) ++b;
+    int t = b;
+    while (t < sh.chunks_y && band_inside(t)) ++t;
+    if (b < t) *begin = b, *end = t;
+}
+
+amt_prm::band_role_ranges frame_roles(const georef_args& A, const launch_shape& sh, double min_elev_deg, bool with_low) {
+    int can_top = 0, can_bottom = sh.chunks_y, in_begin = 0, in_end = 0;
+    if (with_low) elevation_bands(A, sh, min_elev_deg, &can_top, &can_bottom, true);
+    inner_bands(A, sh, min_elev_deg, &in_begin, &in_end);
+    return amt_prm::band_roles(sh.chunks_y, A.sky_top_end, A.sky_bottom_begin, can_top, can_bottom, in_begin, in_end);
 }
 
 void camera_model(const amt_frame_params* p, georef_args* A) {
@@ -1199,6 +1273,7 @@
     double* fold;
     int second;
     int bin;
+    int role_bands[3];
 };
 
 int prepare_georef(amt_ctx* ctx, const amt_frame_params* p, const double* dirs, const amt_georef_out* out,
@@ -1333,6 +1408,13 @@
         if (bin ? A.bin_magnetic : (A.bin_magnetic || !out->bbox)) F->second = 4;
     }
     F->bin = bin;
+    amt_prm::band_role_ranges roles = amt_prm::band_roles_none(sh.chunks_y);
+    if (!ctx->roles_off && dirs == nullptr && F->second != 2 && F->second != 3) roles = frame_roles(A, sh, out->bbox_min_elevation, bin != 0);
+    A.inner_begin = roles.inner_begin, A.inner_end = roles.inner_end;
+    A.low_top_end = roles.low_top_end, A.low_bottom_begin = roles.low_bottom_begin;
+    amt_prm::band_role_counts(roles, A.sky_top_end, A.sky_bottom_begin, F->role_bands);
+    if (sky != nullptr)
+        for (int k = 0; k < 3; ++k) sky->role_items[k] = (int64_t)F->role_bands[k] * sh.strips_x;
     return AMT_OK;
 }
 
@@ -1362,6 +1444,10 @@
         if (F[i].tail != nullptr && F[i].out->bbox) ev.stop = F[i].tail->kernel_done;
     georef_batch B;
     ctx->last_second = F[0].second, ctx->last_bin = bin, ctx->last_frames = n;
+    for (int k = 0; k < 3; ++k) {
+        ctx->last_role_items[k] = 0;
+        for (int i = 0; i < n; ++i) ctx->last_role_items[k] += (int64_t)F[i].role_bands[k] * strips_x;
+    }
     for (int i = 0; i < kMaxBatch; ++i) B.f[i] = F[i < n ? i : 0].A;
     B.math = fx::make_math_table();
     if (dirs) {
@@ -1524,6 +1610,24 @@
     return AMT_OK;
 }
 
+int amt_georef_band_roles(const amt_frame_params* p, double min_elevation, int32_t* rows_per_item, int32_t* ranges8) {
+    if (p == nullptr || rows_per_item == nullptr || ranges8 == nullptr) return AMT_EINVAL;
+    if (p->width <= 0 || p->height <= 0) return AMT_EINVAL;
+    georef_args A;
+    std::memset(&A, 0, sizeof(A));
+    camera_model(p, &A);
+    const launch_shape sh = shape_of(p);
+    A.sky_top_end = 0, A.sky_bottom_begin = sh.chunks_y;
+    sky_bands(A, sh, &A.sky_top_end, &A.sky_bottom_begin);
+    const amt_prm::band_role_ranges r = frame_roles(A, sh, min_elevation, true);
+    *rows_per_item = sh.rows_per_chunk;
+    ranges8[0] = sh.chunks_y, ranges8[1] = sh.strips_x;
+    ranges8[2] = A.sky_top_end, ranges8[3] = A.sky_bottom_begin;
+    ranges8[4] = r.low_top_end, ranges8[5] = r.low_bottom_begin;
+    ranges8[6] = r.inner_begin, ranges8[7] = r.inner_end;
+    return AMT_OK;
+}
+
 int amt_georef_frame_dirs(amt_ctx* ctx, const amt_frame_params* p, const double* corner_dirs,
                           const amt_georef_out* out) {
     return amt_georef_launch_many(ctx, 1, &p, &corner_dirs, &out, nullptr, nullptr);
diff --git a/auromat_amd/csrc/amt_params.h b/auromat_amd/csrc/amt_params.h
--- a/auromat_amd/csrc/amt_params.h
+++ b/auromat_amd/csrc/amt_params.h
@@ -300,6 +300,28 @@
     return sky_known{t, b};
 }
 
+struct band_role_ranges {
+    int inner_begin, inner_end;
+    int low_top_end, low_bottom_begin;
+};
+inline band_role_ranges band_roles_none(int n) { return band_role_ranges{0, 0, 0, n}; }
+
+inline band_role_ranges band_roles(int n, int t, int b, int can_top, int can_bottom, int in_begin, int in_end) {
+    band_role_ranges r = band_roles_none(n);
+    t = std::min(std::max(t, 0), n), b = std::min(std::max(b, t), n);
+    r.low_top_end = std::min(std::max(can_top, t), b);
+    r.low_bottom_begin = std::min(std::max(can_bottom, r.low_top_end), b);
+    const int i0 = std::max(in_begin, r.low_top_end), i1 = std::min(in_end, r.low_bottom_begin);
+    if (i0 < i1) r.inner_begin = i0, r.inner_end = i1;
+    return r;
+}
+inline void band_role_counts(const band_role_ranges& r, int t, int b, int* counts) {
+    t = std::max(t, 0), b = std::max(b, t);
+    counts[1] = r.inner_end - r.inner_begin;
+    counts[2] = std::max(0, std::min(r.low_top_end, b) - t) + std::max(0, b - std::max(r.low_bottom_begin, t));
+    counts[0] = (b - t) - counts[1] - counts[2];
+}
+
 inline void conformal_sin_cos(double e, double s, double c, double* sin_chi, double* cos_chi) {
     const double es = e * s;
     const double w = std::exp(e * std::log((1.0 - es) / (1.0 + es)));
diff --git a/auromat_amd/csrc/amt_run.hip b/auromat_amd/csrc/amt_run.hip
--- a/auromat_amd/csrc/amt_run.hip
+++ b/auromat_amd/csrc/amt_run.hip
@@ -66,6 +66,7 @@
     hipStream_t copy_stream = nullptr;
     hipStream_t launch_stream = nullptr;
     int64_t bands_filled = 0, bands_skipped = 0;
+    int64_t role_items[3] = {0, 0, 0};
 
     slot& slot_of(int k) { return slots[k % cfg.n_slots]; }
 };
@@ -234,6 +235,14 @@
     return AMT_OK;
 }
 
+int amt_run_role_stats(amt_run* run, int64_t* generic, int64_t* inner, int64_t* low) {
+    if (run == nullptr) return AMT_EINVAL;
+    if (generic) *generic = run->role_items[0];
+    if (inner) *inner = run->role_items[1];
+    if (low) *low = run->role_items[2];
+    return AMT_OK;
+}
+
 int amt_run_reset_hints(amt_run* run) {
     if (run == nullptr) return AMT_EINVAL;
     forget_hints(run);
@@ -285,7 +294,7 @@
         pp[j] = s.pipe, prm[j] = &s.prm, oo[j] = &s.out, ii[j] = s.img;
         la[j] = s.ppd_lat, lo[j] = s.ppd_lon;
         const amt_prm::sky_known known = nothing_known ? amt_prm::sky_known_empty() : s.known;
-        sky[j] = {known.top_end, known.bottom_begin, 0, 0};
+        sky[j] = {known.top_end, known.bottom_begin, 0, 0, {0, 0, 0}};
         if (s.img == nullptr) {
             ctx->last_error = "amt_run: a frame has no image";
             return AMT_EINVAL;
@@ -300,6 +309,7 @@
     for (int j = 0; j < m; ++j) {
         run->slots[slots[j]].known = {sky[j].known_top_end, sky[j].known_bottom_begin};
         run->bands_filled += sky[j].bands_filled, run->bands_skipped += sky[j].bands_skipped;
+        for (int k = 0; k < 3; ++k) run->role_items[k] += sky[j].role_items[k];
     }
     return AMT_OK;
 }
@@ -646,6 +656,7 @@
     forget_sky(run);
     run->launch_stream = ctx->stream;
     run->bands_filled = run->bands_skipped = 0;
+    run->role_items[0] = run->role_items[1] = run->role_items[2] = 0;
     run->active = true;
     return AMT_OK;
 }
diff --git a/include/auromat_hip.h b/include/auromat_hip.h
--- a/include/auromat_hip.h
+++ b/include/auromat_hip.h
@@ -49,6 +49,10 @@
 int amt_timing_enable(amt_ctx* ctx, int enable);
 int amt_timing_read(amt_ctx* ctx, int kernel, double* total_ms, int* launches);
 int amt_georef_last_variant(amt_ctx* ctx, int32_t* second, int32_t* bin, int32_t* frames);
+int amt_georef_set_roles(amt_ctx* ctx, int enable);
+int amt_georef_last_roles(amt_ctx* ctx, int64_t* generic, int64_t* inner, int64_t* low);
+struct amt_frame_params;
+int amt_georef_band_roles(const struct amt_frame_params* p, double min_elevation, int32_t* rows_per_item, int32_t* ranges8);
 
 typedef struct amt_frame_params {
     int32_t width;
@@ -512,6 +516,7 @@
 int amt_run_push(amt_run* run, const amt_run_frame* frame);
 int amt_run_end(amt_run* run, int32_t* frames_done);
 int amt_run_fill_stats(amt_run* run, int64_t* bands_filled, int64_t* bands_skipped);
+int amt_run_role_stats(amt_run* run, int64_t* generic, int64_t* inner, int64_t* low);
 int amt_run_reset_hints(amt_run* run);
 int amt_run_set_quantile(amt_run* run, double q);
 int amt_run_set_min_coverage(amt_run* run, uint64_t min_weight);
```
